# CSTR-Edinburgh/magphase

Measured on AMD Instinct MI355X. Metric: frames/sec analysis+synthesis @48kHz FFT=4096, higher is better.
Workload: dtype f32

## Files before the change

include/magphase_hip.h:

```cpp
#ifndef MAGPHASE_HIP_H
#define MAGPHASE_HIP_H

#include <stddef.h>
#include <stdint.h>

#ifdef __cplusplus
extern "C" {
#endif

#define MPX_ABI_VERSION 2

#define MPX_OK 0
#define MPX_ERR_ARG (-1)
#define MPX_ERR_HIP (-2)
#define MPX_ERR_HOST (-3)

int mpx_version(void);
const char* mpx_last_error(void);

size_t mpx_tables_bytes(int fft_len);
int mpx_tables_init(void* stream, int fft_len, void* tables);

int mpx_analysis_frames(void* stream, int fft_len, const void* tables, const float* sig,
                        const int64_t* frame_pos, const int32_t* frame_left, const int32_t* frame_right,
                        int64_t n_frames, float* out_mag, float* out_real, float* out_imag, int64_t ld);

size_t mpx_tables_f64_bytes(int fft_len);
int mpx_tables_f64_init(void* stream, int fft_len, void* tables);
int mpx_analysis_frames_f64(void* stream, int fft_len, const void* tables_f64, const float* sig,
                            const int64_t* frame_pos, const int32_t* frame_left, const int32_t* frame_right,
                            int64_t n_frames, float* out_mag, float* out_real, float* out_imag, int64_t ld,
                            const float* rows_in_use);

int mpx_analysis_frames_f64w(void* stream, int fft_len, const void* tables_f64, const float* sig,
                             const int64_t* frame_pos, const int32_t* frame_left, const int32_t* frame_right,
                             int64_t n_frames, float* out_mag, float* out_real, float* out_imag, int64_t ld,
                             const float* rows_in_use, const double* win_tab, int32_t win_cap);

int mpx_analysis_compressed_fused(void* stream, int fft_len, const void* tables_f64, const float* sig,
                                  const int64_t* frame_pos, const int32_t* frame_left, const int32_t* frame_right,
                                  int64_t n_frames, const double* win_tab, int32_t win_cap, const float* wpack,
                                  const float* whalf, int32_t mag_dim, int32_t phase_dim, const float* voiced,
                                  int32_t mag_fbank, float* out_mag, float* out_real, float* out_imag);
int mpx_analysis_compressed_fused_cr(void* stream, int fft_len, const void* tables_f64, const float* sig,
                                     const int64_t* frame_pos, const int32_t* frame_left, const int32_t* frame_right,
                                     int64_t n_frames, const double* win_tab, int32_t win_cap, const float* wpack,
                                     const float* whalf, int32_t mag_dim, int32_t phase_dim, const float* rows_in_use,
                                     const int32_t* row0, const int32_t* row1, const float* row_t, int64_t n_const,
                                     float* out_mag, float* tmp_real, float* tmp_imag, void* work);
int64_t mpx_analysis_compressed_fused_cr_work_bytes(int fft_len, int64_t n_frames);
int mpx_analysis_compressed_fused_tiles(int32_t mag_dim, int32_t phase_dim, int32_t* ntm, int32_t* ntp);
int mpx_analysis_compressed_fused_waves(void);
int mpx_analysis_compressed_fused_layout(void);
int mpx_analysis_compressed_fused_blocks_per_cu(int fft_len, int32_t phase_dim);

int64_t mpx_feat_ld(int fft_len);

int mpx_synthesis_lossless_frames(void* stream, int fft_len, const void* tables, const float* mag,
                                  const float* real, const float* imag, int64_t n_frames, float* frames_out,
                                  int64_t ld);

int mpx_ola_gather(void* stream, int fft_len, const float* frames, int32_t n_utts, const int32_t* utt_frame_off,
                   const int32_t* pm_rel, const int32_t* out_start, const int64_t* out_off, int64_t max_out_len,
                   float* pcm_out);

typedef struct mpx_ola_run {
    int32_t frame_begin, frame_end;
    int32_t x0;
    int32_t head_end;
    int32_t out_lo, out_hi;
    int32_t flush_end;
    int32_t fix_lo, fix_hi;
    int32_t pad;
    int64_t out_base;
    int64_t strip_off;
} mpx_ola_run;

int mpx_synth_ola_slots(void);
int mpx_synth_ola_slot_weights(float* weights_host, int32_t n_slots);
int64_t mpx_ola_strip_floats(int fft_len);
int mpx_synthesis_lossless_ola(void* stream, int fft_len, const void* tables, const float* mag, const float* real,
                               const float* imag, const mpx_ola_run* runs, int32_t n_runs, const int32_t* slot_off,
                               const int32_t* slot_runs, int32_t n_slots, const int32_t* pm_rel, float* strips,
                               float* pcm_out, int64_t ld );
int mpx_ola_fixup(void* stream, int fft_len, const mpx_ola_run* runs, int32_t n_runs, const float* strips,
                  float* pcm_out);
int mpx_ola_fixup_width(void* stream, int fft_len, const mpx_ola_run* runs, int32_t n_runs, const float* strips,
                        float* pcm_out, int32_t max_width);
int mpx_synthesis_lossless_ola_lerp(void* stream, int fft_len, const void* tables, const float* mag, const float* real,
                                    const float* imag, const int32_t* row0, const int32_t* row1, const float* row_t,
                                    const mpx_ola_run* runs, int32_t n_runs, const int32_t* slot_off,
                                    const int32_t* slot_runs, int32_t n_slots, const int32_t* pm_rel, float* strips,
                                    float* pcm_out, int64_t ld);

int mpx_rows_lerp(void* stream, int32_t n_bins, const float* src_mag, const float* src_real, const float* src_imag,
                  int64_t ld_src, const int32_t* row0, const int32_t* row1, const float* row_t, int64_t n_out,
                  float* dst_mag, float* dst_real, float* dst_imag, int64_t ld_dst);

int mpx_synthesis_lossless_backward(void* stream, int fft_len, const void* tables, const float* grad_out,
                                    int64_t total_out, const int64_t* grad_pos, const int32_t* grad_lo,
                                    const int32_t* grad_hi, int64_t n_frames, const float* mag, const float* real,
                                    const float* imag, int64_t ld, const int32_t* row0, const int32_t* row1,
                                    const float* row_t, float* grad_mag, float* grad_real, float* grad_imag,
                                    int64_t ld_grad);

int mpx_synthesis_compressed_backward(void* stream, int fft_len, const void* tables, const float* grad_out,
                                      int64_t total_out, const int64_t* grad_pos, const int32_t* grad_lo,
                                      const int32_t* grad_hi, int64_t n_frames, const float* mag, const float* real,
                                      const float* imag, int64_t ld, const float* noise, const int64_t* noise_pos,
                                      const int32_t* noise_left, const int32_t* noise_right, const int32_t* noise_wtype,
                                      const int32_t* voiced, const float* inv_gain, const int32_t* win_left,
                                      const int32_t* win_right, const float* per_v, const float* ap_v, const float* ap_u,
                                      int32_t n_per, float* grad_mag, float* grad_real, float* grad_imag,
                                      int64_t ld_grad);

int mpx_synthesis_compressed_type2_backward(void* stream, int fft_len, const void* tables, const float* grad_out,
                                            int64_t total_out, const int64_t* grad_pos, const int32_t* grad_lo,
                                            const int32_t* grad_hi, int64_t n_frames, const float* mag, const float* real,
                                            const float* imag, int64_t ld, const float* noise, const int64_t* noise_pos,
                                            const int32_t* noise_left, const int32_t* noise_right,
                                            const int32_t* noise_wtype, const int32_t* voiced, const float* inv_gain,
                                            const int32_t* win_left, const int32_t* win_right, const float* per_v,
                                            const float* ap_v, const float* ap_u, int32_t n_per, float* grad_mag,
                                            float* grad_real, float* grad_imag, int64_t ld_grad);

int mpx_rows_lerp_adjoint(void* stream, int32_t n_bins, const float* src_mag, const float* src_real,
                          const float* src_imag, int64_t ld_src, const int32_t* ranges, const float* row_t,
                          int64_t n_rows, float* dst_mag, float* dst_real, float* dst_imag, int64_t ld_dst);

int mpx_analysis_lossless_backward(void* stream, int fft_len, const void* tables, const float* mag, const float* real,
                                   const float* imag, int64_t ld, const float* grad_mag, const float* grad_real,
                                   const float* grad_imag, int64_t ld_grad, const int64_t* frame_pos,
                                   const int32_t* frame_left, const int32_t* frame_right, const int64_t* scratch_off,
                                   int64_t n_frames, float* scratch, int64_t scratch_floats, float* grad_sig,
                                   int64_t total_smpls);

int mpx_roundtrip_slot_weights(float* weights_host, int32_t n_slots);
int mpx_roundtrip_frame_terms(int fft_len, const int32_t* frame_left, const int32_t* frame_right, int64_t n_frames,
                              int32_t* terms_host);
int mpx_roundtrip_slot_costs(int32_t* coef_host, int32_t n_slots);
int mpx_roundtrip_lossless_ola(void* stream, int fft_len, const void* tables, const float* sig, const int64_t* frame_pos,
                               const int32_t* frame_left, const int32_t* frame_right, int64_t n_frames,
                               const mpx_ola_run* runs, int32_t n_runs, const int32_t* slot_off, const int32_t* slot_runs,
                               int32_t n_slots, const int32_t* pm_rel, float* out_mag, float* out_real, float* out_imag,
                               float* strips, float* pcm_out, int64_t ld);
#define MPX_RT_FULL_SUPPORT 1u
#define MPX_RT_STORE_ROWS 4u
#define MPX_RT_STORE_NT 8u
#define MPX_RT_INVERSE_TRANSFORM 32u
int mpx_roundtrip_store_map(int fft_len, int phase, int32_t* out);
int mpx_roundtrip_lossless_ola_flags(void* stream, int fft_len, const void* tables, const float* sig,
                                     const int64_t* frame_pos, const int32_t* frame_left, const int32_t* frame_right,
                                     int64_t n_frames, const mpx_ola_run* runs, int32_t n_runs, const int32_t* slot_off,
                                     const int32_t* slot_runs, int32_t n_slots, const int32_t* pm_rel, float* out_mag,
                                     float* out_real, float* out_imag, float* strips, float* pcm_out, int64_t ld,
                                     uint32_t flags);
int mpx_roundtrip_support_classes(int fft_len, const int32_t* frame_left, const int32_t* frame_right, int64_t n_frames,
                                  int32_t* class_host);
int mpx_roundtrip_frame_extents(int fft_len, const int32_t* frame_left, const int32_t* frame_right, int64_t n_frames,
                                uint32_t flags, int32_t* extents_host);

int mpx_griffin_lim_ola(void* stream, int fft_len, const void* tables, const float* sig_in, const int64_t* frame_pos,
                        const int32_t* frame_left, const int32_t* frame_right, int64_t n_frames, const float* target_mag,
                        const mpx_ola_run* runs, int32_t n_runs, const int32_t* slot_off, const int32_t* slot_runs,
                        int32_t n_slots, const int32_t* pm_rel, float* phase_out, float* strips, float* sig_out,
                        int64_t ld);


int mpx_mel_unwarp(void* stream, int64_t n_frames, int32_t n_bins, const float* a_mag, int32_t k_mag,
                   const float* u_mag, float* out_mag, const float* a_real, const float* a_imag, int32_t k_phase,
                   const float* u_phase, float* out_real, float* out_imag,
// ... 236 lines not shown
```

magphase_amd/_lib.py:

```python
import ctypes
import threading
import os

_HERE = os.path.dirname(os.path.abspath(__file__))
LIB_PATH = os.path.join(_HERE, "libmagphase_hip.so")

vp, i32, i64, sz, f64 = ctypes.c_void_p, ctypes.c_int32, ctypes.c_int64, ctypes.c_size_t, ctypes.c_double
u32 = ctypes.c_uint32

PROTOTYPES = {
    "mpx_version": (i32, []),
    "mpx_last_error": (ctypes.c_char_p, []),
    "mpx_tables_bytes": (sz, [i32]),
    "mpx_tables_init": (i32, [vp, i32, vp]),
    "mpx_feat_ld": (i64, [i32]),
    "mpx_analysis_frames": (i32, [vp, i32] + [vp] * 5 + [i64, vp, vp, vp, i64]),
    "mpx_tables_f64_bytes": (sz, [i32]),
    "mpx_tables_f64_init": (i32, [vp, i32, vp]),
    "mpx_analysis_frames_f64": (i32, [vp, i32] + [vp] * 5 + [i64, vp, vp, vp, i64, vp]),
    "mpx_analysis_frames_f64w": (i32, [vp, i32] + [vp] * 5 + [i64, vp, vp, vp, i64, vp, vp, i32]),
    "mpx_analysis_compressed_fused": (i32, [vp, i32] + [vp] * 5 + [i64, vp, i32, vp, vp, i32, i32, vp, i32, vp, vp,
                                       vp]),
    "mpx_analysis_compressed_fused_cr": (i32, [vp, i32] + [vp] * 5 + [i64, vp, i32, vp, vp, i32, i32] + [vp] * 4 +
                                          [i64] + [vp] * 4),
    "mpx_analysis_compressed_fused_cr_work_bytes": (i64, [i32, i64]),
    "mpx_analysis_compressed_fused_tiles": (i32, [i32, i32, ctypes.POINTER(i32), ctypes.POINTER(i32)]),
    "mpx_analysis_compressed_fused_waves": (i32, []),
    "mpx_analysis_compressed_fused_layout": (i32, []),
    "mpx_analysis_compressed_fused_blocks_per_cu": (i32, [i32, i32]),
    "mpx_synthesis_lossless_frames": (i32, [vp, i32] + [vp] * 4 + [i64, vp, i64]),
    "mpx_ola_gather": (i32, [vp, i32, vp, i32] + [vp] * 4 + [i64, vp]),
    "mpx_synth_ola_slots": (i32, []),
    "mpx_synth_ola_slot_weights": (i32, [vp, i32]),
    "mpx_ola_strip_floats": (i64, [i32]),
    "mpx_synthesis_lossless_ola": (i32, [vp, i32] + [vp] * 5 + [i32, vp, vp, i32, vp, vp, vp, i64]),
    "mpx_synthesis_lossless_ola_lerp": (i32, [vp, i32] + [vp] * 8 + [i32, vp, vp, i32, vp, vp, vp, i64]),
    "mpx_rows_lerp": (i32, [vp, i32, vp, vp, vp, i64, vp, vp, vp, i64, vp, vp, vp, i64]),
    "mpx_synthesis_lossless_backward": (i32, [vp, i32, vp, vp, i64, vp, vp, vp, i64, vp, vp, vp, i64] + [vp] * 6 + [i64]),
    "mpx_synthesis_compressed_backward": (i32, [vp, i32, vp, vp, i64, vp, vp, vp, i64, vp, vp, vp, i64] + [vp] * 12
                                          + [i32, vp, vp, vp, i64]),
    "mpx_synthesis_compressed_type2_backward": (i32, [vp, i32, vp, vp, i64, vp, vp, vp, i64, vp, vp, vp, i64] + [vp] * 12
                                                + [i32, vp, vp, vp, i64]),
    "mpx_rows_lerp_adjoint": (i32, [vp, i32, vp, vp, vp, i64, vp, vp, i64, vp, vp, vp, i64]),
    "mpx_analysis_lossless_backward": (i32, [vp, i32, vp, vp, vp, vp, i64, vp, vp, vp, i64, vp, vp, vp, vp, i64, vp, i64,
                                             vp, i64]),
    "mpx_ola_fixup": (i32, [vp, i32, vp, i32, vp, vp]),
    "mpx_ola_fixup_width": (i32, [vp, i32, vp, i32, vp, vp, i32]),
    "mpx_roundtrip_lossless_ola": (i32, [vp, i32] + [vp] * 5 + [i64, vp, i32, vp, vp, i32] + [vp] * 6 + [i64]),
    "mpx_roundtrip_lossless_ola_flags": (i32, [vp, i32] + [vp] * 5 + [i64, vp, i32, vp, vp, i32] + [vp] * 6 + [i64, u32]),
    "mpx_roundtrip_support_classes": (i32, [i32, vp, vp, i64, vp]),
    "mpx_roundtrip_frame_extents": (i32, [i32, vp, vp, i64, u32, vp]),
    "mpx_roundtrip_store_map": (i32, [i32, i32, vp]),
    "mpx_roundtrip_slot_weights": (i32, [vp, i32]),
    "mpx_roundtrip_frame_terms": (i32, [i32, vp, vp, i64, vp]),
    "mpx_roundtrip_slot_costs": (i32, [vp, i32]),
    "mpx_griffin_lim_ola": (i32, [vp, i32] + [vp] * 5 + [i64, vp, vp, i32, vp, vp, i32] + [vp] * 4 + [i64]),
    "mpx_mel_unwarp": (i32, [vp, i64, i32, vp, i32] + [vp] * 4 + [i32, vp, vp, vp, i64]),
    "mpx_mel_unwarp_rows": (i32, [vp, i64, i32, vp, i32] + [vp] * 4 + [i32, vp, vp, vp, i64, vp, vp, vp, i64, vp, vp,
                             i32]),
    "mpx_spec_ld": (i64, [i32]),
    "mpx_noise_uniform": (i32, [vp, i32, vp, vp, i64, vp]),
    "mpx_noise_numpy_mt19937": (i32, [vp, vp, i32, i64] + [vp] * 5),
    "mpx_noise_numpy_mt19937_work_words": (i64, []),
    "mpx_host_mt19937_jump_poly": (i32, [i64, i32, vp]),
    "mpx_host_mt19937_jump_polys": (i32, [vp, i32, vp, i32]),
    "mpx_noise_stats": (i32, [vp, i32] + [vp] * 6 + [i64, vp]),
    "mpx_noise_spectra_floats": (i64, [i32, i64]),
    "mpx_noise_stats_spectra": (i32, [vp, i32] + [vp] * 6 + [i64, vp, vp]),
    "mpx_synth_comp_slots": (i32, []),
    "mpx_synth_comp_slot_weights": (i32, [vp, i32]),
    "mpx_synthesis_compressed_ola": (i32, [vp, i32] + [vp] * 21 + [i32, vp, vp, i32, vp, vp, i64, i32]),
    "mpx_synthesis_compressed_type2_ola": (i32, [vp, i32] + [vp] * 21 + [i32, vp, vp, i32, vp, vp, i64, i32]),
    "mpx_synthesis_compressed_ola_spectra": (i32, [vp, i32] + [vp] * 21 + [i32, vp, vp, i32, vp, vp, i64, i32, vp]),
    "mpx_host_const_to_var_scan": (i64, [vp, vp, i64, vp, vp]),
    "mpx_host_const_to_var_scan_cap": (i64, [vp, vp, i64, vp, vp, i64]),
    "mpx_host_plan_analysis": (i64, [i32] + [vp] * 12),
    "mpx_host_plan_analysis_batch": (i64, [i32] + [vp] * 8 + [i32] + [vp] * 9 + [i32, vp, vp, i64, vp, i32]),
    "mpx_host_plan_synthesis": (i64, [i32, vp, vp, f64, i32, i32, i32, i64] + [vp] * 17),
    "mpx_host_plan_synthesis_batch": (i64, [i32] + [vp] * 5 + [i32, i32, vp, vp, f64] + [i32] * 4 + [vp, f64, i32, vp,
                                       i64] + [vp] * 9 + [i64, vp, i32]),
    "mpx_host_plan_lossless_synthesis": (i64, [i32, vp, vp, vp, i32] + [vp] * 4),
    "mpx_host_ola_runs": (i64, [i32] + [vp] * 5 + [i32, vp, i64, vp, i64]),
    "mpx_host_ola_runs_extents": (i64, [i32] + [vp] * 5 + [i32, vp, i64, vp, vp, i64]),
    "mpx_host_deal_cuts": (i64, [vp, i64, i32, vp, i32, vp, vp]),
    "mpx_host_widen_f32": (i32, [vp, vp, i64, i32]),
    "mpx_host_narrow_f64": (i32, [vp, vp, i64, i32]),
    "mpx_host_copy_many": (i32, [i32] + [vp] * 4 + [i32]),
    "mpx_host_file_sizes": (i32, [i32, vp, vp]),
    "mpx_host_read_est_batch": (i32, [i32, vp, i32] + [vp] * 4 + [i32]),
    "mpx_host_write_files": (i32, [i32] + [vp] * 6 + [i32]),
    "mpx_host_read_files": (i32, [i32] + [vp] * 4 + [i32]),
    "mpx_mel_warp": (i32, [vp, i64, i32] + [vp] * 7 + [i32, vp, i32] + [vp] * 4 + [i64]),
    "mpx_mel_warp_fbank": (i32, [vp, i64, i32] + [vp] * 7 + [i32, vp, i32] + [vp] * 4 + [i64]),
    "mpx_mel_warp_rows": (i32, [vp, i64, i32] + [vp] * 7 + [i32, vp, i32] + [vp] * 4 + [i64, i32, i64, vp, vp, vp]),
    "mpx_warp_phase_rows": (i32, [vp, i64, i32] + [vp] * 8),
    "mpx_mel_warp_backward": (i32, [vp, i32, vp, vp, i32, vp, i64] + [vp] * 7 + [i32, vp, vp, i64, vp, vp, vp, i64, i64]),
    "mpx_mel_unwarp_backward": (i32, [vp, i32, vp, i64, vp, i64, vp, i32, i64, vp, vp, vp, i64, i32, vp, i32, i64, vp, vp]),
    "mpx_phase_grad_mask": (i32, [vp, i64, i32] + [vp] * 7),
    "mpx_min_phase": (i32, [vp, i32] + [vp] * 5 + [i64, vp, vp, vp, i64]),
    "mpx_true_envelope": (i32, [vp, i32, vp, vp, vp, i64, i64, i32, f64, i32, vp, i64, vp, vp, vp]),
    "mpx_frame_gain": (i32, [vp, i32] + [vp] * 5 + [i64, vp, i32]),
    "mpx_noise_gains": (i32, [vp] * 4 + [i32, i32, vp, vp]),
    "mpx_noise_power": (i32, [vp, i32] + [vp] * 5 + [i64, vp]),
    "mpx_noise_rms": (i32, [vp, i32, vp, vp, i32, vp, vp]),
    "mpx_post_filter": (i32, [vp, vp, i64, i32, vp, i32, i32, vp, vp]),
    "mpx_epoch_f0_track": (i32, [vp, vp, vp, i32, i32, vp, i64, vp, vp, vp, i64] + [i32] * 4 + [f64, vp, vp, vp]),
    "mpx_epoch_zff": (i32, [vp, vp, vp, i32, i64, vp, i32, vp, vp, vp, i32] + [vp] * 5),
    "mpx_pcm16": (i32, [vp, vp, i32, vp, i32, i64, f64, vp, vp]),
    "mpx_pcm16_to_f32": (i32, [vp, vp, i64, vp]),
    "mpx_hpf_block": (i32, []),
    "mpx_output_hpf": (i32, [vp] * 4 + [i32, i64] + [vp] * 7),
    "mpx_bw_probe": (i32, [vp, i32, vp, vp, i64]),
    "mpx_bw_probe_shapes": (i32, []),
    "mpx_rows_pack": (i32, [vp, vp, vp, i32, i32] + [vp, i32, i64, i64] * 3),
    "mpx_post_filter_merlin": (i32, [vp, vp, i64, i32] + [vp] * 4 + [i32, f64, vp, f64] + [vp] * 5),
}
SYMBOLS = tuple(PROTOTYPES)
RT_STORE_FLAGS = {"rows": 4, "lines": 0, "lines_nt": 8}
RT_INVERSE_FLAGS = {"direct": 0, "transform": 32}
del vp, i32, i64, sz, f64

_lib = None


class MagphaseHipError(RuntimeError):
    pass


_load_lock = threading.Lock()


def load():
    global _lib
    if _lib is not None:
        return _lib
    with _load_lock:
        return _load_locked()


def _load_locked():
    global _lib
    if _lib is not None:
        return _lib
    import torch
    if not os.path.isfile(LIB_PATH):
        raise MagphaseHipError(
            "libmagphase_hip.so not found at %s -- build it with `python -m magphase_amd.build` "
            "(hipcc --offload-arch=gfx950). There is no CPU fallback." % LIB_PATH
        )
    lib = ctypes.CDLL(LIB_PATH)
    for name, (restype, argtypes) in PROTOTYPES.items():
        fn = getattr(lib, name)
        fn.restype, fn.argtypes = restype, argtypes
    _lib = lib
    return lib


def check(rc, what):
    if rc != 0:
        msg = load().mpx_last_error()
        raise MagphaseHipError("%s failed (%d): %s" % (what, rc, msg.decode("utf-8", "replace") if msg else ""))
```

magphase_amd/csrc/magphase_comp.hip:

```cpp
#include <type_traits>

#include "mpx_common.hpp"

#ifndef MPX_COMP_PAIR_WAVES
#define MPX_COMP_PAIR_WAVES 12
#endif
#ifndef MPX_COMP_DIT
#define MPX_COMP_DIT 0
#endif
#ifndef MPX_COMP_CH
#define MPX_COMP_CH 16
#endif

namespace mpx {

template <int P, bool PRESTAGED, bool COMPACT, int W>
__device__ __forceinline__ void noise_window_gather(const FrameGeom& g, int wtype, float* xbuf, unsigned xbuf_byte, int lane,
                                                    float (&re)[P], float (&im)[P]) {
    constexpr int M = 64 * P, N = 2 * M, kTile = noise_tile_len(P, COMPACT);
    MPX_MARK("zero_init");
#pragma unroll
    for (int j = 0; j < P; ++j)
        if (j < W || j >= P - W) re[(COMPACT && MPX_COMP_DIT) ? brev(j, ilog2(P)) : j] = im[(COMPACT && MPX_COMP_DIT) ? brev(j, ilog2(P)) : j] = 0.0f;
    const int ntiles = MPX_NOISE_TILES(g.len, kTile);
    for (int t = 0; t < ntiles; ++t) {
        MPX_MARK("window");
        const int tile0 = t * kTile;
        if (!PRESTAGED || t > 0) {
            stage_samples_async(g, tile0, kTile, xbuf_byte, lane);
            staged_wait<0>();
        }
        const int hi = min(g.len, tile0 + kTile);
        if (wtype == 0) {
            for (int k = tile0 + lane; k < hi; k += 64)
                xbuf[k - tile0] *= half_window(k, g.L, g.LR, g.kadd, g.invL, g.invR, 0);
        } else {
            for (int k = tile0 + lane; k < hi; k += 64)
                xbuf[k - tile0] *= half_window(k, g.L, g.LR, g.kadd, g.invL, g.invR, 1);
        }
        wave_sync();
        MPX_MARK("gather");
        {
            int n_lo = g.len - g.rot, n_hi = N - g.rot;
            asm volatile("" : "+s"(n_lo), "+s"(n_hi));
            const unsigned span = (unsigned)(hi - tile0);
            const unsigned b0 = (unsigned)(2 * lane + g.rot) - (unsigned)tile0;
#pragma unroll
            for (int j = 0; j < P; ++j) {
                constexpr int LBJ = ilog2(P);
                const int m0 = 128 * j;
                if ((j < W || j >= P - W) && MPX_NOISE_ROW_ACTIVE(m0, n_lo, n_hi)) {
                    const int rj = (COMPACT && MPX_COMP_DIT) ? brev(j, LBJ) : j;
                    const unsigned d0 = (b0 + (unsigned)m0) & (unsigned)(N - 1), d1 = (d0 + 1u) & (unsigned)(N - 1);
                    const float v0 = xbuf[min(d0, (unsigned)(kTile - 1))], v1 = xbuf[min(d1, (unsigned)(kTile - 1))];
                    re[rj] = (d0 < span) ? v0 : re[rj];
                    im[rj] = (d1 < span) ? v1 : im[rj];
                }
            }
        }
        wave_sync();
    }
}

struct NoiseFftNoHook {
    template <int P, typename B>
    __device__ __forceinline__ void gathered(float (&)[P], float (&)[P], B) const {}
    __device__ __forceinline__ void exchanged() const {}
};
template <typename GFn, typename XFn>
struct NoiseFftHook {
    GFn on_gathered;
    XFn on_exchanged;
    template <int P, typename B>
    __device__ __forceinline__ void gathered(float (&re)[P], float (&im)[P], B narrow_c) const { on_gathered(re, im, narrow_c); }
    __device__ __forceinline__ void exchanged() const { on_exchanged(); }
};
template <typename GFn, typename XFn>
__device__ __forceinline__ NoiseFftHook<GFn, XFn> noise_fft_hook(GFn g, XFn x) { return NoiseFftHook<GFn, XFn>{g, x}; }

template <int P, bool PRESTAGED = false, bool COMPACT = false, int NW = 0, typename Hook = NoiseFftNoHook>
__device__ __forceinline__ void noise_fft(const FrameGeom& g, int wtype, const float* tw, float* xbuf,
                                          unsigned xbuf_byte, int lane, float (&re)[P], float (&im)[P], float lc = 1.0f,
                                          float ls = 0.0f, bool narrow = false, Hook hook = Hook()) {
    static_assert(NW == 0 || (COMPACT && !MPX_COMP_DIT), "support classes: the compact DIF form only");
    if constexpr (NW > 0) {
        constexpr unsigned kZin = support_zero_rows<P>(NW);
        constexpr int S0 = zin_clear_stride<P>(kZin);
        static_assert(S0 >= 1 && S0 < P / 2, "a class prunes some, not all, stages of the first pass");
        if (narrow) {
            noise_window_gather<P, PRESTAGED, COMPACT, NW>(g, wtype, xbuf, xbuf_byte, lane, re, im);
            mpx_pin_live<~kZin>(re), mpx_pin_live<~kZin>(im);
            hook.gathered(re, im, std::true_type());
            MPX_MARK("fft_forward");
            fft_inreg_pruned_stage<P, -1, P / 2, kZin, kAllRegs, 2 * S0>(re, im);
            MPX_ARM_END_CLASS();
        } else {
            noise_window_gather<P, PRESTAGED, COMPACT, P / 2>(g, wtype, xbuf, xbuf_byte, lane, re, im);
            mpx_pin(re), mpx_pin(im);
            hook.gathered(re, im, std::false_type());
            MPX_MARK("fft_forward");
            fft_inreg_stages<P, -1, P / 2, 2 * S0>(re, im);
            MPX_ARM_END_FULL();
        }
        const float4 pk = tw_half_pad<P>(tw, lane);
        fft_inreg_stages<P, -1, S0>(re, im);
        wave_fft_front_compact_rest<P, -1>(re, im, tw, xbuf, lane, pk.z, pk.w);
        hook.exchanged();
        fft_inreg<P, -1>(re, im);
        (void)lc;
        (void)ls;
        return;
    }
    constexpr int M = 64 * P, N = 2 * M, kTile = noise_tile_len(P, COMPACT);
    MPX_MARK("zero_init");
#pragma unroll
    for (int j = 0; j < P; ++j) re[j] = im[j] = 0.0f;
    const int ntiles = MPX_NOISE_TILES(g.len, kTile);
    for (int t = 0; t < ntiles; ++t) {
        MPX_MARK("window");
        const int tile0 = t * kTile;
        if (!PRESTAGED || t > 0) {
            stage_samples_async(g, tile0, kTile, xbuf_byte, lane);
            staged_wait<0>();
        }
        const int hi = min(g.len, tile0 + kTile);
        if (wtype == 0) {
            for (int k = tile0 + lane; k < hi; k += 64)
                xbuf[k - tile0] *= half_window(k, g.L, g.LR, g.kadd, g.invL, g.invR, 0);
        } else {
            for (int k = tile0 + lane; k < hi; k += 64)
                xbuf[k - tile0] *= half_window(k, g.L, g.LR, g.kadd, g.invL, g.invR, 1);
        }
        wave_sync();
        MPX_MARK("gather");
        {
            int n_lo = g.len - g.rot, n_hi = N - g.rot;
            asm volatile("" : "+s"(n_lo), "+s"(n_hi));
            const unsigned span = (unsigned)(hi - tile0);
            const unsigned b0 = (unsigned)(2 * lane + g.rot) - (unsigned)tile0;
#pragma unroll
            for (int j = 0; j < P; ++j) {
                constexpr int LBJ = ilog2(P);
                const int m0 = 128 * j;
                if (MPX_NOISE_ROW_ACTIVE(m0, n_lo, n_hi)) {
                    const int rj = (COMPACT && MPX_COMP_DIT) ? brev(j, LBJ) : j;
                    const unsigned d0 = (b0 + (unsigned)m0) & (unsigned)(N - 1), d1 = (d0 + 1u) & (unsigned)(N - 1);
                    const float v0 = xbuf[min(d0, (unsigned)(kTile - 1))], v1 = xbuf[min(d1, (unsigned)(kTile - 1))];
                    re[rj] = (d0 < span) ? v0 : re[rj];
                    im[rj] = (d1 < span) ? v1 : im[rj];
                }
            }
        }
        wave_sync();
    }
    mpx_pin(re), mpx_pin(im);
    hook.gathered(re, im, std::false_type());
    MPX_MARK("fft_forward");
    if constexpr (COMPACT) {
        const float4 pk = tw_half_pad<P>(tw, lane);
#if MPX_COMP_DIT
        wave_fft_dit_compact<P, -1>(re, im, tw, xbuf, lane, pk.z, pk.w);
        hook.exchanged();
#else
        wave_fft_front_compact<P, -1>(re, im, tw, xbuf, lane, pk.z, pk.w);
        hook.exchanged();
        fft_inreg<P, -1>(re, im);
#endif
        (void)lc;
        (void)ls;
    } else {
        wave_fft_front<P, -1>(re, im, tw, xbuf, lane);
        hook.exchanged();
        fft_inreg<P, -1>(re, im);
    }
}

template <int P, bool PRESTAGED = false, bool COMPACT = false, int NW = 0, typename Hook = NoiseFftNoHook>
__device__ __forceinline__ void noise_spectrum_paired(const FrameGeom& g, int wtype, const float* tw, float* xbuf,
                                                      unsigned xbuf_byte, int lane, float wl_c, float wl_s,
                                                      float (&no_r)[P / 2], float (&no_i)[P / 2], float (&nm_r)[P / 2],
                                                      float (&nm_i)[P / 2], float& nh_r, float& nh_i, float lc = 1.0f,
                                                      float ls = 0.0f, bool narrow = false, Hook hook = Hook()) {
    constexpr int LB = ilog2(P);
    float re[P], im[P];
    noise_fft<P, PRESTAGED, COMPACT, NW>(g, wtype, tw, xbuf, xbuf_byte, lane, re, im, lc, ls, narrow, hook);
    mpx_pin(re), mpx_pin(im);
    MPX_MARK("split");
    if constexpr (COMPACT) {
        const float4 pk = tw_half_pad<P>(tw, lane);
        wl_c = pk.x;
        wl_s = pk.y;
    }
    const int kap = kappa<P>(lane);
    const int src_lane = kappa<P>((64 - kap) & 63);
    const bool lane0 = (kap == 0);
#ifndef MPX_NOISE_SPLIT_BATCH
#define MPX_NOISE_SPLIT_BATCH (MPX_COMP_PAIR_WAVES > 8 ? 8 : 16)
#endif
    constexpr int SB = (P / 2 < MPX_NOISE_SPLIT_BATCH) ? P / 2 : MPX_NOISE_SPLIT_BATCH;
#pragma unroll
    for (int qb = 0; qb < P / 2; qb += SB) {
        float zpr[SB], zpi[SB];
        constexpr bool NATR = COMPACT && MPX_COMP_DIT;
#pragma unroll
        for (int u = 0; u < SB; ++u) {
            const int i = NATR ? qb + u : brev(qb + u, LB);
            zpr[u] = __shfl(re[P - 1 - i], src_lane);
            zpi[u] = __shfl(im[P - 1 - i], src_lane);
        }
#pragma unroll
        for (int u = 0; u < SB; ++u) {
            const int q = qb + u;
            const int i = NATR ? q : brev(q, LB);
            const int i0 = NATR ? (P - q) % P : brev((P - q) % P, LB);
            const float pr = lane0 ? re[i0] : zpr[u];
            const float pi = lane0 ? im[i0] : zpi[u];
            const float er = 0.5f * (re[i] + pr), ei = 0.5f * (im[i] - pi);
            const float orr = 0.5f * (im[i] + pi), oi = -0.5f * (re[i] - pr);
            const float cq = cos2p<P>(q), sq = -sin2p<P>(q);
            const float wr = wl_c * cq - wl_s * sq, wi = wl_c * sq + wl_s * cq;
            const float tr = wr * orr - wi * oi, ti = wr * oi + wi * orr;
            no_r[q] = er + tr;
            no_i[q] = ei + ti;
            nm_r[q] = er - tr;
            nm_i[q] = ti - ei;
        }
    }
    constexpr int ih = (COMPACT && MPX_COMP_DIT) ? P / 2 : 1;
    nh_r = re[ih];
    nh_i = -im[ih];
}

template <int P, bool PRESTAGED = false, bool COMPACT = false>
__device__ __forceinline__ void noise_spectrum(const FrameGeom& g, int wtype, const float* tw, float* xbuf,
                                               unsigned xbuf_byte, int lane, float wl_c, float wl_s,
                                               float (&nr)[P], float (&ni)[P], float& nM, float lc = 1.0f, float ls = 0.0f) {
    constexpr int LB = ilog2(P);
    float re[P], im[P];
    noise_fft<P, PRESTAGED, COMPACT>(g, wtype, tw, xbuf, xbuf_byte, lane, re, im, lc, ls);
    if constexpr (COMPACT) {
        const float4 pk = tw_half_pad<P>(tw, lane);
        wl_c = pk.x;
        wl_s = pk.y;
    }
    const int kap = kappa<P>(lane);
    const int src_lane = kappa<P>((64 - kap) & 63);
    const bool lane0 = (kap == 0);
#pragma unroll
    for (int ib = 0; ib < P; ib += 8) {
        float prb[8], pib[8];
#pragma unroll
        for (int u = 0; u < 8; ++u) {
            prb[u] = __shfl(re[P - 1 - (ib + u)], src_lane);
            pib[u] = __shfl(im[P - 1 - (ib + u)], src_lane);
        }
#pragma unroll
        for (int u = 0; u < 8; ++u) {
            const int i = ib + u;
            constexpr bool NATR = COMPACT && MPX_COMP_DIT;
            const int q = NATR ? i : brev(i, LB);
            const int i0 = NATR ? (P - q) % P : brev((P - q) % P, LB);
            const float pr = lane0 ? re[i0] : prb[u];
            const float pi = lane0 ? im[i0] : pib[u];
            const float er = 0.5f * (re[i] + pr), ei = 0.5f * (im[i] - pi);
            const float orr = 0.5f * (im[i] + pi), oi = -0.5f * (re[i] - pr);
            const float cq = cos2p<P>(q), sq = -sin2p<P>(q);
            const float wr = wl_c * cq - wl_s * sq, wi = wl_c * sq + wl_s * cq;
            nr[q] = er + (wr * orr - wi * oi);
            ni[q] = ei + (wr * oi + wi * orr);
        }
    }
    nM = re[0] - im[0];
}

constexpr int kSpecFrameFloats = 17 * 64 * 4;
typedef float spec_f32x4 __attribute__((ext_vector_type(4)));

template <int P>
__global__ __launch_bounds__(kAnaThreads) void k_noise_stats(const float* __restrict__ noise,
                                                          const long long* __restrict__ npos,
                                                          const int* __restrict__ nleft,
                                                          const int* __restrict__ nright,
                                                          const int* __restrict__ wtype, long long nframes,
                                                          const float* __restrict__ tw_g,
                                                          float* __restrict__ out_sum,
                                                          float* __restrict__ spec_out) {
    constexpr int M = 64 * P, N = 2 * M;
    extern __shared__ __attribute__((aligned(16))) float smem[];
    float* tw = smem;
    const int lane_id = threadIdx.x & 63;
    const int wave = threadIdx.x >> 6;
    float* xbuf = smem + tw_floats<P>() + wave * (P * kXStride);
    const unsigned xbuf_byte = 4u * (unsigned)(tw_floats<P>() + rfl(wave) * (P * kXStride));
    for (int i = threadIdx.x; i < tw_floats<P>(); i += kAnaThreads) tw[i] = tw_g[i];
    unsigned* queue = reinterpret_cast<unsigned*>(smem + tw_floats<P>() + kAnaWaves * (P * kXStride));
    if (threadIdx.x == 0) *queue = 0u;
    __syncthreads();
    float wl_s0, wl_c0;
    sincospif(-2.0f * (float)kappa<P>(lane_id) / (float)N, &wl_s0, &wl_c0);
    long long fb, fe;
    block_frame_range(nframes, fb, fe);
    for (long long f = queue_pull(queue, fb); f < fe; f = queue_pull(queue, fb)) {
        int lane = lane_id;
        float wl_s = wl_s0, wl_c = wl_c0;
        asm volatile("" : "+v"(lane), "+v"(wl_s), "+v"(wl_c));
        const FrameGeom g = frame_geom(noise, npos[f], nleft[f], nright[f], N);
        float no_r[P / 2], no_i[P / 2], nm_r[P / 2], nm_i[P / 2], nh_r, nh_i;
        noise_spectrum_paired<P>(g, wtype[f], tw, xbuf, xbuf_byte, lane, wl_c, wl_s, no_r, no_i, nm_r, nm_i, nh_r, nh_i);
        if constexpr (P == 32) {
            if (spec_out) {
                spec_f32x4* d = reinterpret_cast<spec_f32x4*>(spec_out + f * (long long)kSpecFrameFloats) + lane_id;
#pragma unroll
                for (int s_ = 0; s_ < 4; ++s_) {
                    __builtin_nontemporal_store(spec_f32x4{no_r[4 * s_], no_r[4 * s_ + 1], no_r[4 * s_ + 2], no_r[4 * s_ + 3]}, d + 64 * s_);
                    __builtin_nontemporal_store(spec_f32x4{no_i[4 * s_], no_i[4 * s_ + 1], no_i[4 * s_ + 2], no_i[4 * s_ + 3]}, d + 64 * (4 + s_));
                    __builtin_nontemporal_store(spec_f32x4{nm_r[4 * s_], nm_r[4 * s_ + 1], nm_r[4 * s_ + 2], nm_r[4 * s_ + 3]}, d + 64 * (8 + s_));
                    __builtin_nontemporal_store(spec_f32x4{nm_i[4 * s_], nm_i[4 * s_ + 1], nm_i[4 * s_ + 2], nm_i[4 * s_ + 3]}, d + 64 * (12 + s_));
                }
                __builtin_nontemporal_store(spec_f32x4{nh_r, nh_i, 0.0f, 0.0f}, d + 64 * 16);
            }
        }
        const bool lane0 = (kappa<P>(lane) == 0);
        float so[P / 2], sm[P / 2];
        const float sh = nh_r * nh_r + nh_i * nh_i;
        float smin = lane0 ? sh : 1.0f;
#pragma unroll
        for (int q = 0; q < P / 2; ++q) {
            so[q] = no_r[q] * no_r[q] + no_i[q] * no_i[q];
            sm[q] = nm_r[q] * nm_r[q] + nm_i[q] * nm_i[q];
            smin = fminf(smin, fminf(so[q], sm[q]));
        }
        float acc;
        if (!__any(smin < 1.1754944e-38f)) {
            auto term = [](float s_) {
                const float lg = 0.34657359027997264f * __builtin_amdgcn_logf(s_);
                return lg * lg;
            };
            acc = lane0 ? term(sh) : 0.0f;
#pragma unroll
            for (int q = 0; q < P / 2; ++q) {
                const float tq = term(so[q]) + term(sm[q]);
                acc += (q == 0 && lane0) ? 0.0f : tq;
            }
        } else {
            auto term = [](float s_) {
                const float lg = (s_ > 0.0f) ? 0.5f * __logf(s_) : -1.0e10f;
                return lg * lg;
            };
            acc = lane0 ? term(sh) : 0.0f;
#pragma unroll
            for (int q = 0; q < P / 2; ++q) {
                const float tq = term(so[q]) + term(sm[q]);
                acc += (q == 0 && lane0) ? 0.0f : tq;
            }
        }
#pragma unroll
        for (int off = 32; off >= 1; off >>= 1) acc += __shfl_xor(acc, off);
        if (lane_id == 0) out_sum[f] = acc;
    }
}

__global__ __launch_bounds__(256) void k_noise_gains(const float* __restrict__ sums, const int* __restrict__ voiced,
                                                     const int* __restrict__ utt_frame_off, int bins_per_frame,
                                                     float* __restrict__ inv_gain, double* __restrict__ gains) {
    __shared__ double s_sum[2][256];
    __shared__ int s_cnt[2][256];
    const int u = blockIdx.x;
    const int f0 = utt_frame_off[u], f1 = utt_frame_off[u + 1];
    double acc[2] = {0.0, 0.0};
    int cnt[2] = {0, 0};
    for (int f = f0 + threadIdx.x; f < f1; f += 256) {
        const int c = voiced[f] ? 0 : 1;
        acc[c] += (double)sums[f];
        cnt[c] += 1;
    }
    for (int c = 0; c < 2; ++c) {
        s_sum[c][threadIdx.x] = acc[c];
        s_cnt[c][threadIdx.x] = cnt[c];
    }
    __syncthreads();
    for (int off = 128; off >= 1; off >>= 1) {
        if (threadIdx.x < off) {
            for (int c = 0; c < 2; ++c) {
                s_sum[c][threadIdx.x] += s_sum[c][threadIdx.x + off];
                s_cnt[c][threadIdx.x] += s_cnt[c][threadIdx.x + off];
            }
        }
        __syncthreads();
    }
    double g[2];
    for (int c = 0; c < 2; ++c)
        g[c] = (s_cnt[c][0] > 0) ? sqrt(exp(s_sum[c][0] / ((double)s_cnt[c][0] * (double)bins_per_frame))) : nan("");
    if (threadIdx.x == 0 && gains) {
        gains[2 * u + 0] = g[0];
        gains[2 * u + 1] = g[1];
    }
    for (int f = f0 + threadIdx.x; f < f1; f += 256) inv_gain[f] = (float)(1.0 / g[voiced[f] ? 0 : 1]);
}

template <int P>
__global__ __launch_bounds__(kThreads) void k_min_phase(const float* __restrict__ mag, const int* __restrict__ row0,
                                                        const int* __restrict__ row1,
                                                        const float* __restrict__ rowt, long long nframes,
                                                        const float* __restrict__ tw_g, float* __restrict__ omag,
                                                        float* __restrict__ oreal, float* __restrict__ oimag,
                                                        long long ld) {
    constexpr int M = 64 * P, N = 2 * M, H = M + 1, LB = ilog2(P);
    extern __shared__ __attribute__((aligned(16))) float smem[];
    float* tw = smem;
    const int lane_id = threadIdx.x & 63;
    const int wave = threadIdx.x >> 6;
    float* xbuf = smem + tw_floats<P>() + wave * (P * kXStride);
    for (int i = threadIdx.x; i < tw_floats<P>(); i += kThreads) tw[i] = tw_g[i];
    __syncthreads();
    float wa_s0, wa_c0, ws_s0, ws_c0;
    sincospif(-2.0f * (float)kappa<P>(lane_id) / (float)N, &wa_s0, &wa_c0);
    sincospif(2.0f * (float)lane_id / (float)N, &ws_s0, &ws_c0);
    const int wave_u = rfl(wave);
    for (long long f = (long long)blockIdx.x * kWavesPerBlock + wave_u; f < nframes;
         f += (long long)gridDim.x * kWavesPerBlock) {
        int lane = lane_id;
        float wa_s = wa_s0, wa_c = wa_c0, ws_s = ws_s0, ws_c = ws_c0;
        asm volatile("" : "+v"(lane), "+v"(wa_s), "+v"(wa_c), "+v"(ws_s), "+v"(ws_c));
        const int r0 = row0[f], r1 = row1[f];
        const float rt = rowt[f];
        const float* m0p = mag + (long long)r0 * ld;
        const float* m1p = mag + (long long)r1 * ld;
        float xr[P], xi[P], mv[P];
        const float scale = 0.5f / (float)M;
#pragma unroll
        for (int j = 0; j < P; ++j) {
            const float a = m0p[lane + 64 * j], b = m1p[lane + 64 * j];
            mv[j] = fmaf(b - a, rt, a);
        }
        float mM = 0.0f;
        if (lane == 0) {
            const float a = m0p[M], b = m1p[M];
            mM = fmaf(b - a, rt, a);
        }
#pragma unroll
        for (int j = 0; j < P; ++j) {
            xr[j] = ((mv[j] > 0.0f) ? logf(mv[j]) : -1.0e10f) * scale;
            xi[j] = 0.0f;
        }
        const float xm = ((mM > 0.0f) ? logf(mM) : -1.0e10f) * scale;
        hermitian_merge<P>(xr, xi, xm, lane, ws_c, ws_s);
        wave_fft<P, +1>(xr, xi, tw, xbuf, lane);
        const int kap = kappa<P>(lane);
#pragma unroll
        for (int i = 0; i < P; ++i) {
            const int n0 = 2 * (kap + 64 * brev(i, LB));
            const float w0 = (n0 == 0) ? 1.0f : ((n0 < M) ? 2.0f : ((n0 == M) ? 1.0f : 0.0f));
            const float w1 = (n0 + 1 < M) ? 2.0f : ((n0 + 1 == M) ? 1.0f : 0.0f);
            xr[i] *= w0;
            xi[i] *= w1;
        }
        float re[P], im[P];
#pragma unroll
        for (int i = 0; i < P; ++i) {
            re[brev(i, LB)] = xr[i];
            im[brev(i, LB)] = xi[i];
// ... 835 lines not shown
                              "the mirror tail's lanes: lane 0 and those that do not store this step's mirror");
                st_mask(mhi + row_mir_base(lane, cu_m, M) + row_mir_off(HP), lane0 ? mH : hm, ~k_cu_m | 1ull);
                st_mask(rhi + row_mir_base(lane, cu_r, M) + row_mir_off(HP), lane0 ? aH : ha, ~k_cu_r | 1ull);
                st_mask(ihi + row_mir_base(lane, cu_i, M) + row_mir_off(HP), lane0 ? bH : hb, ~k_cu_i | 1ull);
            }
            if constexpr (!DIRECT) merge_handover<P>(zr, zi, 2.0f * nh_r, -2.0f * nh_i, xr, xi, lane);
        }
        if constexpr (DIRECT) {
            g = g_next;
        } else {
            pair_inverse_fft_front<P>(w, xr, xi, lane);
            if (nxt.valid) {
                g = frame_geom(sig, fpos[nxt.fi], fleft[nxt.fi], fright[nxt.fi], N);
                pair_stage_next<P>(w, g, lane);
            }
            if constexpr (kCls) pair_inverse_fft_back_class<P, NW>(xr, xi, narrow);
            else pair_inverse_fft_back<P>(xr, xi);
            constexpr float kScale = 0.5f / (float)M;
            auto plain_add = [](float o, float v, int) { return fmaf(v, kScale, o); };
            auto all_rows = [](int) { return true; };
            pair_ordered_ola<P, true, NW>(w, cur, smem, runs, pm_rel, strips, pcm, xr, xi, lane, plain_add, all_rows, narrow);
        }
        cur = nxt;
#ifdef MPX_PROBE_ENDTIME
        ++probe_frames;
#endif
    }
#ifdef MPX_PROBE_ENDTIME
    if (w.lane_id == 0) {
        const int pw = (blockIdx.x * kCompPairWaves + (int)(threadIdx.x >> 6)) % 8192;
        g_rt_endprobe[4 * pw + 0] = probe_t0;
        g_rt_endprobe[4 * pw + 1] = wall_clock64();
        g_rt_endprobe[4 * pw + 2] = (unsigned long long)probe_frames;
        g_rt_endprobe[4 * pw + 3] = clock64() - probe_c0;
    }
#endif
}

template <int P, bool PHASE>
__global__ __launch_bounds__(kCompPairWaves * 64) void k_griffin_lim_pair(const float* __restrict__ sig,
                                                                         const long long* __restrict__ fpos,
                                                                         const int* __restrict__ fleft,
                                                                         const int* __restrict__ fright,
                                                                         const RunDesc* __restrict__ runs,
                                                                         const int* __restrict__ slot_off,
                                                                         const int* __restrict__ slot_runs, int nslots,
                                                                         const int* __restrict__ pm_rel,
                                                                         const float* __restrict__ tw_g,
                                                                         const float* __restrict__ tmag,
                                                                         float* __restrict__ phase_out,
                                                                         float* __restrict__ strips,
                                                                         float* __restrict__ pcm, long long ld) {
    constexpr int M = 64 * P, N = 2 * M, HP = P / 2;
    extern __shared__ __attribute__((aligned(16))) float smem[];
    PairWave w;
    if (!pair_wave_setup<P>(w, smem, tw_g, runs, slot_off, slot_runs, nslots)) return;
    PairCursor cur = w.cur;

    FrameGeom g = frame_geom(sig, fpos[cur.fi], fleft[cur.fi], fright[cur.fi], N);
    pair_stage_frame<P>(w, g, w.lane_id);

    while (cur.valid) {
        int lane;
        float wa_s, wa_c, ws_s, ws_c;
        pair_frame_lane<P>(w, lane, wa_s, wa_c, ws_s, ws_c);
        PairCursor nxt = cur;
        pair_cursor_advance(nxt, w.wi_end, w.half, runs, slot_runs);
        const int fi = cur.fi;

        float xr[P], xi[P];
        {
            float no_r[HP], no_i[HP], nm_r[HP], nm_i[HP], nh_r, nh_i;
            pair_analysis_spectrum<P>(w, g, lane, wa_c, wa_s, no_r, no_i, nm_r, nm_i, nh_r, nh_i);
            MPX_MARK("magnitude_merge");
            const bool lane0 = (lane == 0);
            const float sgn = (lane & 1) ? -1.0f : 1.0f;
            const float* trow = tmag + (long long)fi * ld;
            float* prow = PHASE ? phase_out + (long long)fi * ld : nullptr;
            if constexpr (PHASE) {
                auto ang = [](float x_r, float x_i, float s) {
                    return (x_r == 0.0f && x_i == 0.0f) ? 0.0f : atan2f(s * x_i, s * x_r);
                };
#pragma unroll
                for (int q = 0; q < HP; ++q) {
                    const int k = lane + 64 * q;
                    prow[k] = ang(no_r[q], no_i[q], sgn);
                    prow[M - k] = ang(nm_r[q], nm_i[q], sgn);
                    asm volatile("" ::: "memory");
                }
                if (lane0) prow[M / 2] = ang(nh_r, nh_i, 1.0f);
            }
            auto replace = [](float& x_r, float& x_i, float t, float s) {
                const bool z = (x_r == 0.0f) && (x_i == 0.0f);
                const float sc = (fmaxf(fabsf(x_r), fabsf(x_i)) < 0x1p-60f) ? 0x1p100f : 1.0f;
                const float u_r = x_r * sc, u_i = x_i * sc;
                const float r = __builtin_amdgcn_rsqf(fmaxf(u_r * u_r + u_i * u_i, 1.0e-37f));
                x_r = z ? t * s : t * (u_r * r);
                x_i = z ? 0.0f : t * (u_i * r);
            };
            if constexpr (comp_compact<P>()) {
                const float4 pk = tw_half_pad<P>(w.tw, lane);
                ws_c = pk.x;
                ws_s = -pk.y;
            }
            float zr[HP], zi[HP];
#pragma unroll
            for (int q = 0; q < HP; ++q) {
                const int k = lane + 64 * q;
                float x_r = no_r[q], x_i = no_i[q], p_r = nm_r[q], p_i = nm_i[q];
                replace(x_r, x_i, trow[k], sgn);
                replace(p_r, p_i, trow[M - k], sgn);
                if (q == 0) {
                    x_i = lane0 ? 0.0f : x_i;
                    p_i = lane0 ? 0.0f : p_i;
                }
                merge_pair_step<P>(q, x_r, x_i, p_r, p_i, ws_c, ws_s, xr[q], xi[q], zr[q], zi[q]);
            }
            replace(nh_r, nh_i, trow[M / 2], 1.0f);
            merge_handover<P>(zr, zi, 2.0f * nh_r, -2.0f * nh_i, xr, xi, lane);
        }
        pair_inverse_fft_front<P>(w, xr, xi, lane);
        if (nxt.valid) {
            g = frame_geom(sig, fpos[nxt.fi], fleft[nxt.fi], fright[nxt.fi], N);
            pair_stage_next<P>(w, g, lane);
        }
        pair_inverse_fft_back<P>(xr, xi);
        constexpr float kScale = 0.5f / (float)M;
        auto plain_add = [](float o, float v, int) { return fmaf(v, kScale, o); };
        auto all_rows = [](int) { return true; };
        pair_ordered_ola<P, true>(w, cur, smem, runs, pm_rel, strips, pcm, xr, xi, lane, plain_add, all_rows);
        cur = nxt;
    }
}

}

using namespace mpx;

extern "C" {

int64_t mpx_spec_ld(int32_t n_bins) { return n_bins <= 0 ? 0 : ((int64_t)n_bins + 31) / 32 * 32; }

static int noise_stats_impl(void* stream, int fft_len, const void* tables, const float* noise, const int64_t* frame_pos,
                            const int32_t* frame_left, const int32_t* frame_right, const int32_t* frame_wtype,
                            int64_t n_frames, float* out_sum, float* spectra) {
    const int P = p_of(fft_len);
    if (!P) return fail(MPX_ERR_ARG, "mpx_noise_stats: fft_len must be 1024, 2048 or 4096%s");
    if (n_frames < 0) return fail(MPX_ERR_ARG, "mpx_noise_stats: negative n_frames%s");
    if (n_frames == 0) return MPX_OK;
    if (!tables || !noise || !frame_pos || !frame_left || !frame_right || !frame_wtype || !out_sum)
        return fail(MPX_ERR_ARG, "mpx_noise_stats: null pointer%s");
    const dim3 grid(grid_for(n_frames, kAnaWaves)), block(kAnaThreads);
    hipStream_t s = (hipStream_t)stream;
    if (P == 32) {
        if (int rc = set_lds(k_noise_stats<32>, lds_bytes_ana<32>())) return rc;
        hipLaunchKernelGGL(k_noise_stats<32>, grid, block, lds_bytes_ana<32>(), s, noise, (const long long*)frame_pos,
                           frame_left, frame_right, frame_wtype, (long long)n_frames, (const float*)tables, out_sum, spectra);
    } else if (P == 16) {
        if (int rc = set_lds(k_noise_stats<16>, lds_bytes_ana<16>())) return rc;
        hipLaunchKernelGGL(k_noise_stats<16>, grid, block, lds_bytes_ana<16>(), s, noise, (const long long*)frame_pos,
                           frame_left, frame_right, frame_wtype, (long long)n_frames, (const float*)tables, out_sum, spectra);
    } else {
        if (int rc = set_lds(k_noise_stats<8>, lds_bytes_ana<8>())) return rc;
        hipLaunchKernelGGL(k_noise_stats<8>, grid, block, lds_bytes_ana<8>(), s, noise, (const long long*)frame_pos,
                           frame_left, frame_right, frame_wtype, (long long)n_frames, (const float*)tables, out_sum, spectra);
    }
    MPX_HIP_CHECK(hipGetLastError());
    return MPX_OK;
}

int mpx_noise_stats(void* stream, int fft_len, const void* tables, const float* noise, const int64_t* frame_pos,
                    const int32_t* frame_left, const int32_t* frame_right, const int32_t* frame_wtype,
                    int64_t n_frames, float* out_sum) {
    return noise_stats_impl(stream, fft_len, tables, noise, frame_pos, frame_left, frame_right, frame_wtype, n_frames,
                            out_sum, nullptr);
}

int64_t mpx_noise_spectra_floats(int fft_len, int64_t n_frames) {
    return (fft_len == 4096 && n_frames > 0) ? n_frames * (int64_t)kSpecFrameFloats : 0;
}

int mpx_noise_stats_spectra(void* stream, int fft_len, const void* tables, const float* noise, const int64_t* frame_pos,
                            const int32_t* frame_left, const int32_t* frame_right, const int32_t* frame_wtype,
                            int64_t n_frames, float* out_sum, float* spectra) {
    if (fft_len != 4096) return fail(MPX_ERR_ARG, "mpx_noise_stats_spectra: fft_len must be 4096%s");
    if (!spectra && n_frames > 0) return fail(MPX_ERR_ARG, "mpx_noise_stats_spectra: null pointer%s");
    return noise_stats_impl(stream, fft_len, tables, noise, frame_pos, frame_left, frame_right, frame_wtype, n_frames,
                            out_sum, spectra);
}

int mpx_synth_comp_slots(void) { return device_cus() * kCompPairs; }

#ifndef MPX_COMP_W0
#define MPX_COMP_W0 100
#endif
#ifndef MPX_COMP_W1
#define MPX_COMP_W1 (MPX_COMP_PAIR_WAVES > 8 ? 82 : 80)
#endif
#ifndef MPX_COMP_W2
#define MPX_COMP_W2 66
#endif
int mpx_synth_comp_slot_weights(float* weights_host, int32_t n_slots) {
    if (!weights_host || n_slots < 0) return fail(MPX_ERR_ARG, "mpx_synth_comp_slot_weights: bad arguments%s");
    for (int s = 0; s < n_slots; ++s) {
        const int age = ((s % kCompPairs) * 2) / 4;
        weights_host[s] = (age == 0) ? (float)MPX_COMP_W0 : ((age == 1) ? (float)MPX_COMP_W1 : (float)MPX_COMP_W2);
    }
    return MPX_OK;
}

extern "C++" {
template <bool T2>
static int synthesis_compressed_ola_impl(const char* who, void* stream, int fft_len, const void* tables, const float* mag, const float* real,
                                 const float* imag, const float* noise, const int64_t* noise_pos,
                                 const int32_t* noise_left, const int32_t* noise_right, const int32_t* noise_wtype,
                                 const int32_t* voiced, const float* inv_gain, const int32_t* row0,
                                 const int32_t* row1, const float* row_t, const int32_t* win_left,
                                 const int32_t* win_right, const int32_t* pm_rel, const float* per_v,
                                 const float* ap_v, const float* ap_u, const mpx_ola_run* runs, int32_t n_runs,
                                 const int32_t* slot_off, const int32_t* slot_runs, int32_t n_slots,
                                 float* strips, float* pcm_out, int64_t ld, int32_t n_per_bins,
                                 const float* spectra) {
    const int P = p_of(fft_len);
    if (!P) return fail(MPX_ERR_ARG, "%s: fft_len must be 1024, 2048 or 4096", who);
    const int n_per = (n_per_bins <= 0 || n_per_bins > fft_len / 2 + 1) ? fft_len / 2 + 1 : (int)n_per_bins;
    if (n_runs < 0 || n_slots < 0) return fail(MPX_ERR_ARG, "%s: negative count", who);
    if (n_runs == 0 || n_slots == 0) return MPX_OK;
    if (!tables || !mag || !real || !imag || !noise || !noise_pos || !noise_left || !noise_right || !noise_wtype ||
        !voiced || !inv_gain || !win_left || !win_right || !pm_rel || !per_v || !ap_v ||
        !ap_u || !runs || !slot_off || !slot_runs || !strips || !pcm_out)
        return fail(MPX_ERR_ARG, "%s: null pointer", who);
    const bool lerp = row0 || row1 || row_t;
    if (lerp && (!row0 || !row1 || !row_t))
        return fail(MPX_ERR_ARG, "%s: row0 / row1 / row_t must be given together", who);
    CompFrameTabs tb{(const long long*)noise_pos, noise_left, noise_right, noise_wtype, voiced, inv_gain,
                     row0, row1, row_t, win_left, win_right, pm_rel, spectra};
    hipStream_t s = (hipStream_t)stream;
    const dim3 pgrid((n_slots + kCompPairs - 1) / kCompPairs), pblock(kCompPairWaves * 64);
    if (spectra) {
        if (P != 32 || lerp)
            return fail(MPX_ERR_ARG, "mpx_synthesis_compressed_ola_spectra: fft_len 4096 and one row per frame only%s");
        if (n_per <= 512) {
            if (int rc = set_lds(k_synth_comp_pair<32, false, 8, true>, lds_bytes_comp_pair<32>())) return rc;
            hipLaunchKernelGGL((k_synth_comp_pair<32, false, 8, true>), pgrid, pblock, lds_bytes_comp_pair<32>(),
                               s, mag, real, imag, noise, tb, per_v, ap_v, ap_u, (const RunDesc*)runs, slot_off, slot_runs,
                               (int)n_slots, (const float*)tables, strips, pcm_out, (long long)ld, n_per);
        } else {
            if (int rc = set_lds(k_synth_comp_pair<32, false, -1, true>, lds_bytes_comp_pair<32>())) return rc;
            hipLaunchKernelGGL((k_synth_comp_pair<32, false, -1, true>), pgrid, pblock, lds_bytes_comp_pair<32>(),
                               s, mag, real, imag, noise, tb, per_v, ap_v, ap_u, (const RunDesc*)runs, slot_off, slot_runs,
                               (int)n_slots, (const float*)tables, strips, pcm_out, (long long)ld, n_per);
        }
        MPX_HIP_CHECK(hipGetLastError());
        return MPX_OK;
    }
#define MPX_LAUNCH_COMP(PP, LL)                                                                                        \
    do {                                                                                                             \
        if (int rc = set_lds(k_synth_comp_pair<PP, LL, -1, false, T2>, lds_bytes_comp_pair<PP>())) return rc;        \
        hipLaunchKernelGGL((k_synth_comp_pair<PP, LL, -1, false, T2>), pgrid, pblock, lds_bytes_comp_pair<PP>(), s,  \
                           mag, real, imag,                                                                          \
                           noise, tb, per_v, ap_v, ap_u, (const RunDesc*)runs, slot_off, slot_runs, (int)n_slots,    \
                           (const float*)tables, strips, pcm_out, (long long)ld, n_per);                 \
    } while (0)
    if (lerp) {
        if (P == 32) MPX_LAUNCH_COMP(32, true);
        else if (P == 16) MPX_LAUNCH_COMP(16, true);
        else MPX_LAUNCH_COMP(8, true);
    } else {
        if (P == 32 && n_per <= 512) {
            if (int rc = set_lds(k_synth_comp_pair<32, false, 8, false, T2>, lds_bytes_comp_pair<32>())) return rc;
            hipLaunchKernelGGL((k_synth_comp_pair<32, false, 8, false, T2>), pgrid, pblock, lds_bytes_comp_pair<32>(), s, mag, real, imag,
                               noise, tb, per_v, ap_v, ap_u, (const RunDesc*)runs, slot_off, slot_runs, (int)n_slots,
                               (const float*)tables, strips, pcm_out, (long long)ld, n_per);
        } else if (P == 32) MPX_LAUNCH_COMP(32, false);
        else if (P == 16) MPX_LAUNCH_COMP(16, false);
        else MPX_LAUNCH_COMP(8, false);
    }
#undef MPX_LAUNCH_COMP
    MPX_HIP_CHECK(hipGetLastError());
    return MPX_OK;
}
}

int mpx_synthesis_compressed_ola(void* stream, int fft_len, const void* tables, const float* mag, const float* real,
                                 const float* imag, const float* noise, const int64_t* noise_pos,
                                 const int32_t* noise_left, const int32_t* noise_right, const int32_t* noise_wtype,
                                 const int32_t* voiced, const float* inv_gain, const int32_t* row0,
                                 const int32_t* row1, const float* row_t, const int32_t* win_left,
                                 const int32_t* win_right, const int32_t* pm_rel, const float* per_v,
                                 const float* ap_v, const float* ap_u, const mpx_ola_run* runs, int32_t n_runs,
                                 const int32_t* slot_off, const int32_t* slot_runs, int32_t n_slots,
                                 float* strips, float* pcm_out, int64_t ld, int32_t n_per_bins) {
    return synthesis_compressed_ola_impl<false>("mpx_synthesis_compressed_ola", stream, fft_len, tables, mag, real, imag, noise,
                                                noise_pos, noise_left, noise_right, noise_wtype, voiced, inv_gain, row0, row1,
                                                row_t, win_left, win_right, pm_rel, per_v, ap_v, ap_u, runs, n_runs, slot_off,
                                                slot_runs, n_slots, strips, pcm_out, ld, n_per_bins, nullptr);
}

int mpx_synthesis_compressed_type2_ola(void* stream, int fft_len, const void* tables, const float* mag, const float* real,
                                       const float* imag, const float* noise, const int64_t* noise_pos,
                                       const int32_t* noise_left, const int32_t* noise_right, const int32_t* noise_wtype,
                                       const int32_t* voiced, const float* inv_gain, const int32_t* row0,
                                       const int32_t* row1, const float* row_t, const int32_t* win_left,
                                       const int32_t* win_right, const int32_t* pm_rel, const float* per_v,
                                       const float* ap_v, const float* ap_u, const mpx_ola_run* runs, int32_t n_runs,
                                       const int32_t* slot_off, const int32_t* slot_runs, int32_t n_slots,
                                       float* strips, float* pcm_out, int64_t ld, int32_t n_per_bins) {
// ... 283 lines not shown
```

magphase_amd/csrc/magphase_f64.hip:

```cpp
#include <type_traits>

#include "mpx_common.hpp"
#include "wave_fft_f64.hpp"

namespace mpx {

constexpr int kAna64Waves = 8;
template <int P>
constexpr int f64_win_floats() { return 58 * P; }
#ifndef MPX_F64_DIT
#define MPX_F64_DIT 1
#endif
constexpr bool kF64Dit = MPX_F64_DIT != 0;
template <int P>
constexpr size_t lds_bytes_ana64() {
    return sizeof(double) * (size_t)tw64_doubles<P>() +
           sizeof(float) * (size_t)(kAna64Waves * P * kXStride + 4 + kAna64Waves * f64_win_floats<P>());
}

__device__ __forceinline__ double sin_halfpi_range(double x) {
    const double x2 = x * x;
    double p = 1.0 / 355687428096000.0;
    p = fma(x2, p, -1.0 / 1307674368000.0);
    p = fma(x2, p, 1.0 / 6227020800.0);
    p = fma(x2, p, -1.0 / 39916800.0);
    p = fma(x2, p, 1.0 / 362880.0);
    p = fma(x2, p, -1.0 / 5040.0);
    p = fma(x2, p, 1.0 / 120.0);
    p = fma(x2, p, -1.0 / 6.0);
    return fma(x * x2, p, x);
}

__device__ __forceinline__ double hann_half_f64(int k, int L, int LR, int kadd, double invL, double invR) {
    const bool rising = k <= L;
    const int num = rising ? k + kadd : LR - k;
    const double t = (double)num * (rising ? invL : invR);
    return fma(0.5, sin_halfpi_range(3.14159265358979323846 * (t - 0.5)), 0.5);
}

__device__ __forceinline__ double rsqrt_f64(double s) {
    const double r = (double)__builtin_amdgcn_rsqf((float)s);
    return r * fma(-0.5 * s, r * r, 1.5);
}

template <bool PH>
__device__ __forceinline__ void feat_store(double xr, double xi, double zero2, float mag_scale, float* pm, float* pr, float* pi) {
    const double s = xr * xr + xi * xi;
    const bool nz = s > zero2;
    const double r = nz ? rsqrt_f64(s) : 0.0;
    *pm = (float)(s * r) * mag_scale;
    if (PH) {
        *pr = (float)(xr * r);
        *pi = (float)(xi * r);
    }
}

template <int P>
__device__ __forceinline__ constexpr int f64_in_reg(int j) { return kF64Dit ? brev(j, ilog2(P)) : j; }
template <int P>
__device__ __forceinline__ constexpr int f64_out_reg(int q) { return kF64Dit ? q : brev(q, ilog2(P)); }

template <int P>
__device__ __forceinline__ void f64_frame_transform(const float* __restrict__ sig, long long pos, int Lf, int Rf,
                                                    const double* __restrict__ win_tab, int win_cap, const double* tw,
                                                    float* xbuf, unsigned xbuf_byte, float* wbuf, unsigned wbuf_byte,
                                                    int lane, double (&re)[P], double (&im)[P], double& zero2_out,
                                                    float& mag_scale_out) {
    constexpr int N = 128 * P, kTile = 64 * P;
    const FrameGeom g = frame_geom(sig, pos, Lf, Rf, N);
    const double invL = (g.L > 0) ? 1.0 / (double)g.L : 1.0;
    const double invR = (g.LR > g.L) ? 1.0 / (double)(g.LR - g.L) : 0.0;
    const int gR = g.LR - g.L;
    const bool tabw = rfl((int)(win_tab != nullptr && g.L <= win_cap && gR <= win_cap)) != 0;
    const double* tl = win_tab + ((long long)g.L * (g.L + 1) >> 1);
    const double* tr = win_tab + ((long long)gR * (gR + 1) >> 1);
    const float in_scale = tabw ? 1073741824.0f : 1.0f;
    const float mag_scale = tabw ? 9.313225746154785e-10f : 1.0f;

    double s_abs = 0.0;
#pragma unroll
    for (int j = 0; j < P; ++j) re[j] = im[j] = 0.0;
    constexpr int capD = f64_win_floats<P>() / 2;
    double* wl = reinterpret_cast<double*>(wbuf);
    const int nidx = g.LR + 2;
    const int ntiles = (g.len + kTile - 1) / kTile;
    for (int t = 0; t < ntiles; ++t) {
        const int tile0 = t * kTile;
        const int hi = min(g.len, tile0 + kTile);
        stage_samples_async(g, tile0, kTile, xbuf_byte, lane);
        for (int seg0 = 0; seg0 < nidx; seg0 += capD) {
            const int seg1 = min(seg0 + capD, nidx);
            if (tabw) {
                const int a0 = seg0, a1 = min(g.L + 1, seg1), b0 = max(g.L + 1, seg0), b1 = seg1;
                const float* srcl = reinterpret_cast<const float*>(tl + a0);
                const float* srcr = reinterpret_cast<const float*>(tr + (b0 - (g.L + 1)));
                const int nl = 2 * max(a1 - a0, 0), nr = 2 * max(b1 - b0, 0);
                for (int c = 0; c < (nl + 63) >> 6; ++c) {
                    const unsigned m0v = __builtin_amdgcn_readfirstlane(wbuf_byte + 256u * (unsigned)c);
                    if (64 * c + lane < nl) {
                        const float* src = srcl + 64 * c + lane;
                        asm volatile("s_mov_b32 m0, %1\n\ts_nop 0\n\tglobal_load_lds_dword %0, off" ::"v"(src), "s"(m0v) : "m0", "memory");
                    }
                }
                for (int c = 0; c < (nr + 63) >> 6; ++c) {
                    const unsigned m0v = __builtin_amdgcn_readfirstlane(wbuf_byte + 8u * (unsigned)(b0 - seg0) + 256u * (unsigned)c);
                    if (64 * c + lane < nr) {
                        const float* src = srcr + 64 * c + lane;
                        asm volatile("s_mov_b32 m0, %1\n\ts_nop 0\n\tglobal_load_lds_dword %0, off" ::"v"(src), "s"(m0v) : "m0", "memory");
                    }
                }
            } else {
                for (int i = seg0 + lane; i < seg1; i += 64) {
                    const int k = (i <= g.L) ? i : g.LR - (i - (g.L + 1));
                    wl[i - seg0] = hann_half_f64(k, g.L, g.LR, g.kadd, invL, invR);
                }
            }
            staged_wait<0>();
            wave_sync();
            int lane_g = lane;
            asm volatile("" : "+v"(lane_g));
#pragma unroll
            for (int j = 0; j < P; ++j) {
                const int m0 = 128 * j;
                const bool any = (m0 < g.len - g.rot) || (m0 + 127 >= N - g.rot);
                if (any) {
                    const int m = m0 + 2 * lane_g;
                    int k0 = m + g.rot;
                    k0 = (k0 >= N) ? k0 - N : k0;
                    int k1 = m + 1 + g.rot;
                    k1 = (k1 >= N) ? k1 - N : k1;
                    const int i0 = ((k0 <= g.L) ? k0 : g.L + 1 + (g.LR - k0)) - seg0;
                    const int i1 = ((k1 <= g.L) ? k1 : g.L + 1 + (g.LR - k1)) - seg0;
                    if (k0 >= tile0 && k0 < hi && i0 >= 0 && i0 < capD) {
                        const double v = (double)(xbuf[k0 - tile0] * in_scale) * wl[i0];
                        re[f64_in_reg<P>(j)] = v;
                        s_abs += fabs(v);
                    }
                    if (k1 >= tile0 && k1 < hi && i1 >= 0 && i1 < capD) {
                        const double v = (double)(xbuf[k1 - tile0] * in_scale) * wl[i1];
                        im[f64_in_reg<P>(j)] = v;
                        s_abs += fabs(v);
                    }
                }
            }
            wave_sync();
        }
    }
    float s_all = (float)s_abs;
#pragma unroll
    for (int d = 32; d >= 1; d >>= 1) s_all += __shfl_xor(s_all, d);
    const double zt = 2.842170943040401e-14 * (double)s_all;
#ifdef MPX_F64_NOFLUSH
    const double zero2 = 1.0e-36 + 0.0 * zt;
#else
    const double zero2 = tabw ? 1.0e-36 : fmax(zt * zt, 1.0e-36);
#endif

    if constexpr (kF64Dit) wave_fft_dit_f64<P, -1>(re, im, tw, xbuf, lane);
    else wave_fft_f64<P, -1>(re, im, tw, xbuf, lane);
#pragma unroll
    for (int j = 0; j < P; j += 4)
        asm volatile("" : "+v"(re[j]), "+v"(re[j + 1]), "+v"(re[j + 2]), "+v"(re[j + 3]), "+v"(im[j]), "+v"(im[j + 1]),
                          "+v"(im[j + 2]), "+v"(im[j + 3]));

    zero2_out = zero2;
    mag_scale_out = mag_scale;
}

template <int P>
__global__ __launch_bounds__(kAna64Waves * 64) void k_analysis_f64(const float* __restrict__ sig,
                                                                  const long long* __restrict__ fpos,
                                                                  const int* __restrict__ fleft,
                                                                  const int* __restrict__ fright, long long nframes,
                                                                  const double* __restrict__ tw_g,
                                                                  float* __restrict__ omag, float* __restrict__ oreal,
                                                                  float* __restrict__ oimag, long long ld,
                                                                  const float* __restrict__ rows_in_use,
                                                                  const double* __restrict__ win_tab, int win_cap) {
    constexpr int M = 64 * P, N = 2 * M, LB = ilog2(P), kTile = 64 * P;
    extern __shared__ __attribute__((aligned(16))) double smem64[];
    double* tw = smem64;
    float* xbase = reinterpret_cast<float*>(smem64 + tw64_doubles<P>());
    const int lane_id = threadIdx.x & 63;
    const int wave = rfl((int)(threadIdx.x >> 6));
    float* xbuf = xbase + wave * (P * kXStride);
    const unsigned xbuf_byte = 8u * (unsigned)tw64_doubles<P>() + 4u * (unsigned)(wave * (P * kXStride));
    for (int i = threadIdx.x; i < tw64_doubles<P>(); i += kAna64Waves * 64) {
        const int l = i / tw64_stride<P>(), c = i - l * tw64_stride<P>();
        const int src = (kF64Dit && c < 2 * P) ? l * tw64_stride<P>() + 2 * brev(c >> 1, LB) + (c & 1) : i;
        tw[i] = tw_g[src];
    }
    unsigned* queue = reinterpret_cast<unsigned*>(xbase + kAna64Waves * (P * kXStride));
    float* wbuf = xbase + kAna64Waves * (P * kXStride) + 4 + wave * f64_win_floats<P>();
    const unsigned wbuf_byte = 8u * (unsigned)tw64_doubles<P>() + 4u * (unsigned)(kAna64Waves * (P * kXStride) + 4 + wave * f64_win_floats<P>());
    if (threadIdx.x == 0) *queue = 0u;
    __syncthreads();

    double wl_s0, wl_c0;
    sincospi(-2.0 * (double)kappa<P>(lane_id) / (double)N, &wl_s0, &wl_c0);

    long long fb, fe;
    block_frame_range(nframes, fb, fe);
    for (long long f = queue_pull(queue, fb); f < fe; f = queue_pull(queue, fb)) {
        int lane = lane_id;
        double wl_s = wl_s0, wl_c = wl_c0;
        asm volatile("" : "+v"(lane), "+v"(wl_s), "+v"(wl_c));
        const int kap = kappa<P>(lane);
        const int src_lane = kappa<P>((64 - kap) & 63);
        const bool lane0 = (kap == 0);
        double re[P], im[P];
        double zero2;
        float mag_scale;
        f64_frame_transform<P>(sig, fpos[f], fleft[f], fright[f], win_tab, win_cap, tw, xbuf, xbuf_byte, wbuf, wbuf_byte, lane, re,
                               im, zero2, mag_scale);

        float* row_m = omag + f * ld;
        float* row_r = oreal + f * ld;
        float* row_i = oimag + f * ld;
#ifndef MPX_F64_EPI_BATCH
#define MPX_F64_EPI_BATCH 4
#endif
        constexpr int EB = MPX_F64_EPI_BATCH;
        auto epilogue = [&](auto ph_tag) {
            constexpr bool PH = decltype(ph_tag)::value;
#pragma unroll
            for (int qb = 0; qb < P / 2; qb += EB) {
                double zpr[EB], zpi[EB];
#pragma unroll
                for (int u = 0; u < EB; ++u) {
                    const int i = f64_out_reg<P>(qb + u);
                    unsigned a, b, c, d;
                    split64(re[P - 1 - i], a, b);
// ... 14 lines not shown
                    const double cq = dc64(q * kq), sq = -ds64(q * kq);
                    const double wr = wl_c * cq - wl_s * sq, wi = wl_c * sq + wl_s * cq;
                    const double tr = wr * orr - wi * oi, ti = wr * oi + wi * orr;
                    const int k = kap + 64 * q;
                    feat_store<PH>(er + tr, ei + ti, zero2, mag_scale, row_m + k, row_r + k, row_i + k);
                    const int km = M - k;
                    feat_store<PH>(er - tr, ti - ei, zero2, mag_scale, row_m + km, row_r + km, row_i + km);
                }
            }
            constexpr int ih = f64_out_reg<P>(P / 2);
            if (lane0) feat_store<PH>(re[ih], -im[ih], zero2, mag_scale, row_m + M / 2, row_r + M / 2, row_i + M / 2);
        };
        if (rows_in_use == nullptr || rfl((int)(rows_in_use[f] != 0.0f))) epilogue(std::true_type{});
        else epilogue(std::false_type{});
    }
}

typedef float f32x4_t __attribute__((ext_vector_type(4)));
#ifndef MPX_FUSED_WAVES
#define MPX_FUSED_WAVES 8
#endif
constexpr int kFusedWaves = MPX_FUSED_WAVES;
static_assert(kFusedWaves == 4 || kFusedWaves == 8, "4 or 8 waves per fused workgroup");
constexpr int kFusedCols = 128 / kFusedWaves;
constexpr int kFusedKH = kFusedCols / 16;
#ifndef MPX_FUSED_ASTRIDE
#define MPX_FUSED_ASTRIDE 136
#endif
constexpr int kFusedAStride = MPX_FUSED_ASTRIDE;
static_assert(kFusedAStride % 4 == 0 && kFusedAStride >= 128, "published rows: 128 columns, 16-byte aligned");

constexpr int kFusedRedStride = 68;
#ifndef MPX_FUSED_PAIR
#define MPX_FUSED_PAIR 1
#endif
#ifndef MPX_FUSED_VOIBRANCH
#define MPX_FUSED_VOIBRANCH 1
#endif
#ifndef MPX_FUSED_F32NORM
#define MPX_FUSED_F32NORM 1
#endif
#ifndef MPX_FUSED_M4
#define MPX_FUSED_M4 1
#endif

__device__ __forceinline__ float fused_prologue_mag(int mode, float x) {
    if (mode == 0) return __builtin_amdgcn_logf(fmaf(x, x, 1.0e-8f)) * 0.69314718055994531f;
    return (x > 0.0f) ? __logf(x) : -1.0e10f;
}
#ifndef MPX_FUSED_EXPFIT
#define MPX_FUSED_EXPFIT 1
#endif
__device__ __forceinline__ float fused_prologue_phase(float x) {
#if MPX_FUSED_EXPFIT
    const float t = fmaf(x, fmaf(x, 2.75579379e-8f, -3.18127371e-8f), 0.90168841e-8f);
    return fmaf(2.0f, x, t);
#else
    return fmaf(1.0e-8f, __expf(-2.0f * x), 2.0f * x);
#endif
}

template <int MAGMODE, bool RAW>
__device__ __forceinline__ void fused_operand(double xr, double xi, double zero2, float mag_scale, bool voi, float& a_m, float& a_r,
                                              float& a_i) {
    const double s2 = xr * xr + xi * xi;
    const bool nz = s2 > zero2;
#if MPX_FUSED_F32NORM
    const float s2f = (float)s2;
    const float rf = nz ? __builtin_amdgcn_rsqf(s2f) : 0.0f;
    a_m = RAW ? (s2f * rf) * mag_scale : fused_prologue_mag(MAGMODE, (s2f * rf) * mag_scale);
    if (RAW) asm volatile("" : "+v"(a_m));
    if (voi) {
        a_r = fused_prologue_phase((float)xr * rf);
        a_i = fused_prologue_phase((float)xi * rf);
    } else {
        a_r = a_i = 0.0f;
    }
    return;
#endif
    const double rr = nz ? rsqrt_f64(s2) : 0.0;
    a_m = RAW ? (float)(s2 * rr) * mag_scale : fused_prologue_mag(MAGMODE, (float)(s2 * rr) * mag_scale);
    if (RAW) asm volatile("" : "+v"(a_m));
#if MPX_FUSED_VOIBRANCH
    if (voi) {
        a_r = fused_prologue_phase((float)(xr * rr));
        a_i = fused_prologue_phase((float)(xi * rr));
    } else {
        a_r = a_i = 0.0f;
    }
#else
    a_r = voi ? fused_prologue_phase((float)(xr * rr)) : 0.0f;
    a_i = voi ? fused_prologue_phase((float)(xi * rr)) : 0.0f;
#endif
}

#ifndef MPX_FUSED_EB
#define MPX_FUSED_EB 2
#endif
template <int P, int MAGMODE, bool RAW>
__device__ __forceinline__ void fused_split_operands(double (&re)[P], double (&im)[P], double zero2, float mag_scale, bool voi,
                                                     bool lane0, int src_lane, double wl_c, double wl_s, float (&vm)[P],
                                                     float (&vr)[P], float (&vi)[P], float& m0, float& m1, float& m2) {
    constexpr int EB = MPX_FUSED_EB;
#pragma unroll
    for (int qb = 0; qb < P / 2; qb += EB) {
        asm volatile("" : "+v"(re[f64_out_reg<P>(qb)]), "+v"(im[f64_out_reg<P>(qb)]));
        double zpr[EB], zpi[EB];
#pragma unroll
        for (int u = 0; u < EB; ++u) {
            const int i = f64_out_reg<P>(qb + u);
            unsigned a, b, c, d;
            split64(re[P - 1 - i], a, b);
            split64(im[P - 1 - i], c, d);
            zpr[u] = join64((unsigned)__shfl((int)a, src_lane), (unsigned)__shfl((int)b, src_lane));
            zpi[u] = join64((unsigned)__shfl((int)c, src_lane), (unsigned)__shfl((int)d, src_lane));
        }
#pragma unroll
        for (int u = 0; u < EB; ++u) {
            const int q = qb + u;
            const int i = f64_out_reg<P>(q);
            const int i0 = f64_out_reg<P>((P - q) % P);
            const double pr_ = lane0 ? re[i0] : zpr[u];
            const double pi_ = lane0 ? im[i0] : zpi[u];
            const double er = 0.5 * (re[i] + pr_), ei = 0.5 * (im[i] - pi_);
            const double orr = 0.5 * (im[i] + pi_), oi = -0.5 * (re[i] - pr_);
            constexpr int kq = 64 / (2 * P);
            const double cq = dc64(q * kq), sq = -ds64(q * kq);
            const double wr = wl_c * cq - wl_s * sq, wi = wl_c * sq + wl_s * cq;
            const double tr = wr * orr - wi * oi, ti = wr * oi + wi * orr;
            fused_operand<MAGMODE, RAW>(er + tr, ei + ti, zero2, mag_scale, voi, vm[2 * q], vr[2 * q], vi[2 * q]);
            fused_operand<MAGMODE, RAW>(er - tr, ti - ei, zero2, mag_scale, voi, vm[2 * q + 1], vr[2 * q + 1], vi[2 * q + 1]);
        }
    }
    constexpr int ih = f64_out_reg<P>(P / 2);
    fused_operand<MAGMODE, RAW>(re[ih], -im[ih], zero2, mag_scale, voi, m0, m1, m2);
}

template <int P, int NTP>
constexpr bool fused_pair() {
    return MPX_FUSED_PAIR != 0 && NTP >= 3 && kFusedWaves == 8 &&
           kFusedWaves * f64_win_floats<P>() >= 4 * 3 * kFusedWaves * kFusedAStride;
}

template <int P, int NTM, int NTP>
constexpr size_t lds_bytes_fused() {
    static_assert(kFusedWaves * f64_win_floats<P>() >= 2 * 3 * kFusedWaves * kFusedAStride, "the tiles live inside the window regions");
    constexpr size_t tiles = NTM + NTP;
    constexpr size_t work = sizeof(float) * (size_t)(kFusedWaves * P * kXStride + kFusedWaves * f64_win_floats<P>());
    constexpr size_t red = sizeof(float) * (size_t)(kFusedWaves * tiles * 4 * kFusedRedStride);
    static_assert(work >= red, "the reduction buffer must fit the regions it aliases");
    return sizeof(double) * (size_t)tw64_doubles<P>() + work + sizeof(float) * 32;
}

template <int P, int NTM, int NTP, int MAGMODE>
__attribute__((amdgpu_waves_per_eu(2, 2)))
__global__ __launch_bounds__(kFusedWaves * 64) void k_analysis_warp_fused(
    const float* __restrict__ sig, const long long* __restrict__ fpos, const int* __restrict__ fleft,
    const int* __restrict__ fright, long long nframes, const double* __restrict__ tw_g,
    const double* __restrict__ win_tab, int win_cap, const float* __restrict__ wpack, const float* __restrict__ whalf,
    const float* __restrict__ voiced, int mag_dim, int phase_dim, float* __restrict__ omag, float* __restrict__ oreal,
    float* __restrict__ oimag) {
    constexpr int M = 64 * P, N = 2 * M, LB = ilog2(P), T = NTM + NTP;
    extern __shared__ __attribute__((aligned(16))) double smem64[];
    double* tw = smem64;
    float* xbase = reinterpret_cast<float*>(smem64 + tw64_doubles<P>());
    const int lane_id = threadIdx.x & 63;
    const int wave = rfl((int)(threadIdx.x >> 6));
    float* xbuf = xbase + wave * (P * kXStride);
    const unsigned xbuf_byte = 8u * (unsigned)tw64_doubles<P>() + 4u * (unsigned)(wave * (P * kXStride));
    float* As = xbase + kFusedWaves * (P * kXStride);
    float* wbuf = As + wave * f64_win_floats<P>();
    const unsigned wbuf_byte = 8u * (unsigned)tw64_doubles<P>() + 4u * (unsigned)(kFusedWaves * (P * kXStride) + wave * f64_win_floats<P>());
    float* red = xbase;
    float* mid = xbase + kFusedWaves * (P * kXStride) + kFusedWaves * f64_win_floats<P>();
    for (int i = threadIdx.x; i < tw64_doubles<P>(); i += kFusedWaves * 64) {
        const int l = i / tw64_stride<P>(), c = i - l * tw64_stride<P>();
        const int src = (kF64Dit && c < 2 * P) ? l * tw64_stride<P>() + 2 * brev(c >> 1, LB) + (c & 1) : i;
        tw[i] = tw_g[src];
    }
    __syncthreads();

    double wl_s0, wl_c0;
    sincospi(-2.0 * (double)kappa<P>(lane_id) / (double)N, &wl_s0, &wl_c0);
    const long long nrounds = (nframes + kFusedWaves - 1) / kFusedWaves;
    const int li = lane_id & 15, g = lane_id >> 4;
    const f32x4_t* wp_wave = reinterpret_cast<const f32x4_t*>(wpack) + ((long long)wave * kFusedKH * T) * 64;

    for (long long rnd = blockIdx.x; rnd < nrounds; rnd += gridDim.x) {
        int lane = lane_id;
        double wl_s = wl_s0, wl_c = wl_c0;
        asm volatile("" : "+v"(lane), "+v"(wl_s), "+v"(wl_c));
        const int kap = kappa<P>(lane);
        const int src_lane = kappa<P>((64 - kap) & 63);
        const bool lane0 = (kap == 0);
        const long long f = rnd * kFusedWaves + wave;
        const bool has = f < nframes;
        double re[P], im[P];
        double zero2 = 1.0e-36;
        float mag_scale = 1.0f;
        bool voi = false;
        if (has) {
            f64_frame_transform<P>(sig, fpos[f], fleft[f], fright[f], win_tab, win_cap, tw, xbuf, xbuf_byte, wbuf, wbuf_byte, lane,
                                   re, im, zero2, mag_scale);
            voi = rfl((int)(voiced[f] != 0.0f)) != 0;
        } else {
#pragma unroll
            for (int j = 0; j < P; ++j) re[j] = im[j] = 0.0;
        }

        float vm[P], vr[P], vi[P];
        {
            float m0, m1, m2;
            fused_split_operands<P, MAGMODE, false>(re, im, zero2, mag_scale, voi, lane0, src_lane, wl_c, wl_s, vm, vr, vi, m0, m1, m2);
            if (lane0) {
                mid[0 * kFusedWaves + wave] = m0;
                mid[1 * kFusedWaves + wave] = m1;
                mid[2 * kFusedWaves + wave] = m2;
            }
        }
        constexpr bool M4 = kFusedKH == 1 && MPX_FUSED_M4 != 0;
        constexpr int TR = M4 ? 2 + NTP : T;
        f32x4_t acc[TR];
#pragma unroll
        for (int t = 0; t < TR; ++t) acc[t] = f32x4_t{0.0f, 0.0f, 0.0f, 0.0f};
        __syncthreads();
#ifdef MPX_FUSED_PRIO
        __builtin_amdgcn_s_setprio(MPX_FUSED_PRIO);
#endif
        if constexpr (M4) {
            constexpr int FR = 8 + NTP;
            const f32x4_t* wp4 = reinterpret_cast<const f32x4_t*>(wpack) + ((long long)wave * FR) * 64;
            f32x4_t bm[4][2], bp[NTP];
            {
                int wo = 0;
                asm volatile("" : "+s"(wo));
#pragma unroll
                for (int f = 0; f < 8; ++f) bm[f >> 1][f & 1] = wp4[wo + f * 64 + lane_id];
#pragma unroll
                for (int t = 0; t < NTP; ++t) bp[t] = wp4[wo + (8 + t) * 64 + lane_id];
            }
            const int arow4 = (4 * (lane_id >> 5) + (lane_id & 3)) * kFusedAStride + kFusedCols * wave;
            constexpr bool PAIR = fused_pair<P, NTP>();
            constexpr int NB = PAIR ? 4 : 2;
            auto publish = [&](int q) {
                float* row = As + (q & (NB - 1)) * (3 * kFusedWaves * kFusedAStride) + wave * kFusedAStride;
                row[kap] = vm[2 * q];
                row[64 + kap] = vm[2 * q + 1];
                row += kFusedWaves * kFusedAStride;
                row[kap] = vr[2 * q];
                row[64 + kap] = vr[2 * q + 1];
                row += kFusedWaves * kFusedAStride;
                row[kap] = vi[2 * q];
                row[64 + kap] = vi[2 * q + 1];
            };
#pragma unroll
            for (int q = 0; q < P / 2; ++q) {
                const float* tile = As + (q & (NB - 1)) * (3 * kFusedWaves * kFusedAStride);
                if (!PAIR) {
                    publish(q);
                    __syncthreads();
                } else if ((q & 1) == 0) {
                    publish(q);
                    publish(q + 1);
                    __syncthreads();
                }
                f32x4_t a4[4];
#pragma unroll
                for (int kg = 0; kg < 4; ++kg) a4[kg] = *reinterpret_cast<const f32x4_t*>(tile + arow4 + 4 * kg);
                const f32x4_t ap = *reinterpret_cast<const f32x4_t*>(
                    tile + ((li < 8 ? 1 : 2) * kFusedWaves + (li & (kFusedWaves - 1))) * kFusedAStride + kFusedCols * wave + 4 * g);
                int wo = (q + 1 < P / 2 ? q + 1 : q) * (kFusedWaves * FR * 64);
                asm volatile("" : "+s"(wo));
                f32x4_t cm[2][2];
#pragma unroll
                for (int i = 0; i < 4; ++i) cm[i >> 1][i & 1] = f32x4_t{0.0f, 0.0f, 0.0f, 0.0f};
#pragma unroll
                for (int kg = 0; kg < 4; ++kg) {
#pragma unroll
                    for (int e = 0; e < 4; ++e) {
#pragma unroll
                        for (int hf = 0; hf < 2; ++hf) {
#ifdef MPX_PROBE_FUSEDA_NOMFMA
                            cm[hf][e & 1][e] = fmaf(a4[kg][e], bm[kg][hf][e], cm[hf][e & 1][e]);
#else
                            cm[hf][e & 1] = __builtin_amdgcn_mfma_f32_4x4x1f32(a4[kg][e], bm[kg][hf][e], cm[hf][e & 1], 0, 0, 0);
#endif
                        }
                    }
                    if (q + 1 < P / 2) {
                        bm[kg][0] = wp4[wo + (2 * kg) * 64 + lane_id];
                        bm[kg][1] = wp4[wo + (2 * kg + 1) * 64 + lane_id];
                    }
                }
#pragma unroll
                for (int t = 0; t < NTP; ++t) {
                    f32x4_t ca = f32x4_t{0.0f, 0.0f, 0.0f, 0.0f};
#pragma unroll
                    for (int e = 0; e < 4; ++e) {
#ifdef MPX_PROBE_FUSEDA_NOMFMA
                        ca[e] = fmaf(ap[e], bp[t][e], ca[e]);
#else
                        ca = __builtin_amdgcn_mfma_f32_16x16x4f32(ap[e], bp[t][e], ca, 0, 0, 0);
#endif
                    }
                    if (q + 1 < P / 2) bp[t] = wp4[wo + (8 + t) * 64 + lane_id];
                    acc[2 + t] += ca;
                }
                acc[0] += cm[0][0] + cm[0][1];
                acc[1] += cm[1][0] + cm[1][1];
            }
        } else
#pragma unroll
        for (int q = 0; q < P / 2; ++q) {
            float* tile = As + (q & 1) * (3 * kFusedWaves * kFusedAStride);
            {
                float* row = tile + wave * kFusedAStride;
                row[kap] = vm[2 * q];
                row[64 + kap] = vm[2 * q + 1];
                row += kFusedWaves * kFusedAStride;
                row[kap] = vr[2 * q];
                row[64 + kap] = vr[2 * q + 1];
                row += kFusedWaves * kFusedAStride;
                row[kap] = vi[2 * q];
                row[64 + kap] = vi[2 * q + 1];
            }
            int wo = q * (kFusedWaves * kFusedKH * T * 64);
            asm volatile("" : "+s"(wo));
            const f32x4_t* wq = wp_wave + wo;
            f32x4_t bw[T];
#pragma unroll
            for (int t = 0; t < T; ++t) bw[t] = wq[t * 64 + lane_id];
            __syncthreads();
            f32x4_t ca[T];
#pragma unroll
            for (int t = 0; t < T; ++t) ca[t] = f32x4_t{0.0f, 0.0f, 0.0f, 0.0f};
#pragma unroll
            for (int h = 0; h < kFusedKH; ++h) {
                const int col = kFusedCols * wave + 16 * h + 4 * g;
                const f32x4_t am = *reinterpret_cast<const f32x4_t*>(tile + (li & (kFusedWaves - 1)) * kFusedAStride + col);
                const f32x4_t ap = *reinterpret_cast<const f32x4_t*>(
                    tile + ((li < 8 ? 1 : 2) * kFusedWaves + (li & (kFusedWaves - 1))) * kFusedAStride + col);
                if (h > 0) {
                    int who = h * (T * 64);
                    asm volatile("" : "+s"(who));
                    const f32x4_t* wh = wq + who;
#pragma unroll
                    for (int t = 0; t < T; ++t) bw[t] = wh[t * 64 + lane_id];
                }
#pragma unroll
                for (int e = 0; e < 4; ++e) {
#ifdef MPX_PROBE_FUSEDA_NOMFMA
#pragma unroll
                    for (int t = 0; t < NTM; ++t) ca[t][e] = fmaf(am[e], bw[t][e], ca[t][e]);
#pragma unroll
                    for (int t = NTM; t < T; ++t) ca[t][e] = fmaf(ap[e], bw[t][e], ca[t][e]);
#else
#pragma unroll
                    for (int t = 0; t < NTM; ++t) ca[t] = __builtin_amdgcn_mfma_f32_16x16x4f32(am[e], bw[t][e], ca[t], 0, 0, 0);
#pragma unroll
                    for (int t = NTM; t < T; ++t) ca[t] = __builtin_amdgcn_mfma_f32_16x16x4f32(ap[e], bw[t][e], ca[t], 0, 0, 0);
#endif
                }
            }
#pragma unroll
            for (int t = 0; t < T; ++t) acc[t] += ca[t];
        }
#ifdef MPX_FUSED_PRIO
        __builtin_amdgcn_s_setprio(0);
#endif
        __syncthreads();
#pragma unroll
        for (int t = 0; t < TR; ++t)
#pragma unroll
            for (int r = 0; r < 4; ++r) red[((wave * TR + t) * 4 + r) * kFusedRedStride + lane_id] = acc[t][r];
        __syncthreads();
        constexpr int kOuts = NTM + 2 * NTP;
        for (int idx = threadIdx.x; idx < kFusedWaves * kOuts * 16; idx += kFusedWaves * 64) {
            const int c = idx & 15, to = (idx >> 4) % kOuts, fr = idx / (16 * kOuts);
            const long long fo = rnd * kFusedWaves + fr;
            if (fo >= nframes) continue;
            const int sa = (to < NTM) ? 0 : ((to < NTM + NTP) ? 1 : 2);
            const int t = (sa == 2) ? to - NTP : to;
            const int row = (sa == 2) ? 8 + fr : fr;
            const int gg = row >> 2, r = row & 3;
            float y = 0.0f;
            if (M4 && sa == 0) {
                const int n = 16 * to + c;
#pragma unroll
                for (int w = 0; w < kFusedWaves; ++w)
                    y += red[((w * TR + (n >> 5)) * 4 + (fr & 3)) * kFusedRedStride + (n & 31) + 32 * (fr >> 2)];
            } else {
                const int tr = M4 ? t - NTM + 2 : t;
#pragma unroll
                for (int w = 0; w < kFusedWaves; ++w) y += red[((w * TR + tr) * 4 + r) * kFusedRedStride + c + 16 * gg];
            }
            y = fmaf(mid[sa * kFusedWaves + fr], whalf[t * 16 + c], y);
            if (sa == 0) {
                const int n = 16 * t + c;
                if (n >= mag_dim) continue;
                if (MAGMODE == 2) y = (y < -745.13321f) ? -1.0e10f : y;
                omag[fo * mag_dim + n] = y;
            } else {
                const int n = 16 * (t - NTM) + c;
                if (n >= phase_dim) continue;
                const float vo = voiced[fo];
                y = (vo == 0.0f) ? 0.0f : fminf(fmaxf(y * vo, -1.0f), 1.0f);
                (sa == 1 ? oreal : oimag)[fo * phase_dim + n] = y;
            }
        }
        __syncthreads();
    }
}

constexpr int kCrRows = 16;
constexpr int kCrRawRows = 9;
constexpr int kCrPhRows = 2 * 2 * 2 * kFusedWaves;
template <int P>
constexpr int cr_tile_floats() {
    constexpr int mag_rows = 3 * kCrRawRows + 2 * kCrRows;
    constexpr int win = kFusedWaves * f64_win_floats<P>(), tiles = (mag_rows > kCrPhRows ? mag_rows : kCrPhRows) * kFusedAStride;
    return win > tiles ? win : tiles;
}
template <int P>
constexpr int cr_halo_floats() { return 64 * P + 64; }
template <int P, int NTP>
constexpr size_t lds_bytes_fused_cr() {
    constexpr size_t work = sizeof(float) * (size_t)(kFusedWaves * P * kXStride + cr_tile_floats<P>());
    constexpr size_t red = sizeof(float) * (size_t)(kFusedWaves * (4 + NTP) * 4 * kFusedRedStride);
    static_assert(work >= red, "the reduction buffer must fit the regions it aliases");
    return sizeof(double) * (size_t)tw64_doubles<P>() + work + sizeof(float) * (48 + 3 * kCrRows);
}

__global__ __launch_bounds__(256) void k_cr_index(const int* __restrict__ row1, int n_const, long long nframes,
                                                  int* __restrict__ cstart) {
    const long long f = (long long)blockIdx.x * 256 + threadIdx.x;
    if (f > nframes) return;
    int lo = 0, hi = n_const;
    while (lo < hi) {
        const int m = (lo + hi) >> 1;
        if ((long long)row1[m] < f) lo = m + 1; else hi = m;
    }
    cstart[f] = lo;
}

template <int P, int NTP>
__attribute__((amdgpu_waves_per_eu(2, 2)))
__global__ __launch_bounds__(kFusedWaves * 64) void k_analysis_warp_fused_cr(
    const float* __restrict__ sig, const long long* __restrict__ fpos, const int* __restrict__ fleft,
    const int* __restrict__ fright, long long nframes, const double* __restrict__ tw_g,
    const double* __restrict__ win_tab, int win_cap, const float* __restrict__ wpack, const float* __restrict__ whalf,
    const float* __restrict__ rows_in_use, const int* __restrict__ row0, const int* __restrict__ row1,
    const float* __restrict__ rowt, const int* __restrict__ cstart, int frames_per_wg, int mag_dim, int phase_dim,
    float* __restrict__ omag, float* __restrict__ tr_out, float* __restrict__ ti_out, float* halo) {
    static_assert(kFusedWaves == 8 && kFusedKH == 1 && MPX_FUSED_M4 != 0, "the constant-rate form is written for 8 waves and the 4 x 4 magnitude product");
    constexpr int M = 64 * P, N = 2 * M, LB = ilog2(P), NC = P / 2, AS = kFusedAStride;
    constexpr int TR = 4 + NTP;
    constexpr int FR = 8 + NTP;
    extern __shared__ __attribute__((aligned(16))) double smem64[];
    double* tw = smem64;
    float* xbase = reinterpret_cast<float*>(smem64 + tw64_doubles<P>());
    const int lane_id = threadIdx.x & 63;
    const int wave = rfl((int)(threadIdx.x >> 6));
    float* xbuf = xbase + wave * (P * kXStride);
    const unsigned xbuf_byte = 8u * (unsigned)tw64_doubles<P>() + 4u * (unsigned)(wave * (P * kXStride));
    float* rawb = xbase + kFusedWaves * (P * kXStride);
    float* abuf = rawb + 3 * kCrRawRows * AS;
    float* wbuf = rawb + wave * f64_win_floats<P>();
    const unsigned wbuf_byte = 8u * (unsigned)tw64_doubles<P>() + 4u * (unsigned)(kFusedWaves * (P * kXStride) + wave * f64_win_floats<P>());
    float* red = xbase;
    float* mid = rawb + cr_tile_floats<P>();
    float* prm = mid + 48;
    for (int i = threadIdx.x; i < tw64_doubles<P>(); i += kFusedWaves * 64) {
        const int l = i / tw64_stride<P>(), c = i - l * tw64_stride<P>();
        const int src = (kF64Dit && c < 2 * P) ? l * tw64_stride<P>() + 2 * brev(c >> 1, LB) + (c & 1) : i;
        tw[i] = tw_g[src];
    }
    __syncthreads();

    double wl_s0, wl_c0;
    sincospi(-2.0 * (double)kappa<P>(lane_id) / (double)N, &wl_s0, &wl_c0);
    const int li = lane_id & 15, g = lane_id >> 4;
    const f32x4_t* wp4 = reinterpret_cast<const f32x4_t*>(wpack) + ((long long)wave * FR) * 64;
    float* hs = halo + (long long)blockIdx.x * (2 * cr_halo_floats<P>());
    const long long own_lo = (long long)blockIdx.x * frames_per_wg;
    const long long own_end = (own_lo + frames_per_wg < nframes) ? own_lo + frames_per_wg : nframes;
    const int arow4 = (4 * (lane_id >> 5) + (lane_id & 3)) * AS + kFusedCols * wave;
    const int jr = (int)(threadIdx.x >> 5), col4 = 4 * (int)(threadIdx.x & 31);

    int c_next0 = 0, c_next1 = 0;
    bool prm_ready = false;
    for (int r = 0;; ++r) {
        const long long a = own_lo - 1 + 8ll * r;
        const long long hi_lo = (r == 0) ? a + 1 : a;
        if (hi_lo >= own_end) break;
        const long long hi_hi = (a + 8 < own_end) ? a + 8 : own_end;
        const int c0 = (r == 0) ? cstart[hi_lo] : c_next0;
        const int c1 = (r == 0) ? cstart[hi_hi] : c_next1;
        const bool more = a + 8 < own_end;
        c_next0 = c1;
        c_next1 = more ? cstart[(a + 16 < own_end) ? a + 16 : own_end] : c1;
        int lane = lane_id;
        double wl_s = wl_s0, wl_c = wl_c0;
        asm volatile("" : "+v"(lane), "+v"(wl_s), "+v"(wl_c));
        const int kap = kappa<P>(lane);
        const int src_lane = kappa<P>((64 - kap) & 63);
        const bool lane0 = (kap == 0);
        const long long f = a + wave;
        const bool has = f >= 0 && f < own_end;
        double re[P], im[P];
        double zero2 = 1.0e-36;
        float mag_scale = 1.0f;
        bool voi = false;
        if (has) {
            f64_frame_transform<P>(sig, fpos[f], fleft[f], fright[f], win_tab, win_cap, tw, xbuf, xbuf_byte, wbuf, wbuf_byte, lane,
                                   re, im, zero2, mag_scale);
            voi = rfl((int)(rows_in_use[f] != 0.0f)) != 0;
        } else {
#pragma unroll
            for (int j = 0; j < P; ++j) re[j] = im[j] = 0.0;
        }
        float vm[P], vr[P], vi[P];
        const bool halo_on = r >= 1;
        const float* hp = hs + ((r + 1) & 1) * cr_halo_floats<P>();
        {
            float m0, m1, m2;
            fused_split_operands<P, 0, true>(re, im, zero2, mag_scale, voi, lane0, src_lane, wl_c, wl_s, vm, vr, vi, m0, m1, m2);
            if (lane0) {
                mid[wave] = m0;
                mid[9 + wave] = m1;
                mid[17 + wave] = m2;
            }
            if (wave == kFusedWaves - 1) {
                float* hw = hs + (r & 1) * cr_halo_floats<P>();
#pragma unroll
                for (int j = 0; j < P; ++j) hw[j * 64 + lane_id] = vm[j];
                if (lane0) {
                    hw[64 * P] = m0;
                    if (halo_on) mid[8] = hp[64 * P];
                }
            }
        }
        if (lane_id == 0) mid[32 + wave] = voi ? 1.0f : 0.0f;
        __syncthreads();
        bool any_ph = false;
#pragma unroll
        for (int w = 0; w < kFusedWaves; ++w) any_ph |= mid[32 + w] != 0.0f;
        any_ph = rfl((int)any_ph) != 0;

        constexpr int kHaloAhead = 4;
        const bool halo_w = halo_on && wave == kFusedWaves - 1;
        float hq[kHaloAhead][2];
#pragma unroll
        for (int u = 0; u < kHaloAhead; ++u) hq[u][0] = hq[u][1] = 0.0f;
        if (halo_w && c1 > c0) {
#pragma unroll
            for (int u = 0; u < kHaloAhead; ++u) {
                hq[u][0] = hp[(2 * u) * 64 + lane_id];
                hq[u][1] = hp[(2 * u + 1) * 64 + lane_id];
            }
        }

        f32x4_t accp[NTP];
#pragma unroll
        for (int t = 0; t < NTP; ++t) accp[t] = f32x4_t{0.0f, 0.0f, 0.0f, 0.0f};
        if (any_ph) {
            f32x4_t bp[2][NTP];
#pragma unroll
            for (int u = 0; u < 2; ++u) {
                int wo = u * (kFusedWaves * FR * 64);
                asm volatile("" : "+s"(wo));
#pragma unroll
                for (int t = 0; t < NTP; ++t) bp[u][t] = wp4[wo + (8 + t) * 64 + lane_id];
            }
#pragma unroll
            for (int q = 0; q < NC; ++q) {
                float* tile = rawb + (((q >> 1) & 1) * 2 + (q & 1)) * (2 * kFusedWaves * AS);
                if ((q & 1) == 0) {
#pragma unroll
                    for (int u = 0; u < 2; ++u) {
                        float* row = tile + u * (2 * kFusedWaves * AS) + wave * AS;
                        row[kap] = vr[2 * (q + u)];
                        row[64 + kap] = vr[2 * (q + u) + 1];
                        row += kFusedWaves * AS;
                        row[kap] = vi[2 * (q + u)];
                        row[64 + kap] = vi[2 * (q + u) + 1];
                    }
                    __syncthreads();
                }
                const f32x4_t ap = *reinterpret_cast<const f32x4_t*>(tile + li * AS + kFusedCols * wave + 4 * g);
                int wo = (q + 2 < NC ? q + 2 : q) * (kFusedWaves * FR * 64);
                asm volatile("" : "+s"(wo));
#pragma unroll
                for (int t = 0; t < NTP; ++t) {
                    f32x4_t ca = f32x4_t{0.0f, 0.0f, 0.0f, 0.0f};
#pragma unroll
                    for (int e = 0; e < 4; ++e) ca = __builtin_amdgcn_mfma_f32_16x16x4f32(ap[e], bp[q & 1][t][e], ca, 0, 0, 0);
                    if (q + 2 < NC) bp[q & 1][t] = wp4[wo + (8 + t) * 64 + lane_id];
                    accp[t] += ca;
                }
            }
            __syncthreads();
        }

        for (int cb = c0, sweep = 0; sweep == 0 || cb < c1; cb += kCrRows, ++sweep) {
            const bool ph = sweep == 0 && any_ph;
            const int nrows = (c1 - cb < kCrRows) ? c1 - cb : kCrRows;
            const int npass = nrows > 8 ? 2 : (nrows > 0 ? 1 : 0);
            if (!(sweep == 0 && prm_ready)) {
                if (threadIdx.x < kCrRows && (int)threadIdx.x < nrows) {
                    prm[3 * threadIdx.x] = __int_as_float(row0[cb + threadIdx.x]);
                    prm[3 * threadIdx.x + 1] = __int_as_float(row1[cb + threadIdx.x]);
                    prm[3 * threadIdx.x + 2] = rowt[cb + threadIdx.x];
                }
                __syncthreads();
            }
            int lo_rel = 0, hi_rel = 0;
            float tt = 0.0f;
            if (jr < nrows) {
                lo_rel = __float_as_int(prm[3 * jr]) - (int)a;
                hi_rel = __float_as_int(prm[3 * jr + 1]) - (int)a;
                tt = prm[3 * jr + 2];
                if (lo_rel < 0) lo_rel = 8;
            }
            f32x4_t acc[4];
#pragma unroll
            for (int t = 0; t < 4; ++t) acc[t] = f32x4_t{0.0f, 0.0f, 0.0f, 0.0f};
            auto chunks = [&](auto np_tag) {
                constexpr int NP = decltype(np_tag)::value;
                f32x4_t bm[2][4][2];
#pragma unroll
                for (int u = 0; u < 2; ++u) {
                    int wo = u * (kFusedWaves * FR * 64);
                    asm volatile("" : "+s"(wo));
#pragma unroll
                    for (int fi = 0; fi < 8; ++fi) bm[u][fi >> 1][fi & 1] = wp4[wo + fi * 64 + lane_id];
                }
                const bool builder = NP == 2 || wave < kFusedWaves / 2;
                if (sweep > 0 && halo_w) {
#pragma unroll
                    for (int u = 0; u < kHaloAhead; ++u) {
                        hq[u][0] = hp[(2 * u) * 64 + lane_id];
                        hq[u][1] = hp[(2 * u + 1) * 64 + lane_id];
                    }
                }
                auto publish = [&](int q) {
                    float* row = rawb + (q % 3) * (kCrRawRows * AS) + wave * AS;
                    row[kap] = vm[2 * q];
                    row[64 + kap] = vm[2 * q + 1];
                    if (halo_w) {
                        float* hr = rawb + (q % 3) * (kCrRawRows * AS) + 8 * AS;
                        hr[kap] = hq[q % kHaloAhead][0];
                        hr[64 + kap] = hq[q % kHaloAhead][1];
                        if (q + kHaloAhead < NC) {
                            hq[q % kHaloAhead][0] = hp[(2 * (q + kHaloAhead)) * 64 + lane_id];
                            hq[q % kHaloAhead][1] = hp[(2 * (q + kHaloAhead) + 1) * 64 + lane_id];
                        }
                    }
                };
                auto build = [&](int q) {
                    const float* rb = rawb + (q % 3) * (kCrRawRows * AS);
                    const f32x4_t x0 = *reinterpret_cast<const f32x4_t*>(rb + lo_rel * AS + col4);
                    const f32x4_t x1 = *reinterpret_cast<const f32x4_t*>(rb + hi_rel * AS + col4);
                    f32x4_t av;
#pragma unroll
                    for (int e = 0; e < 4; ++e) av[e] = fused_prologue_mag(0, fmaf(x1[e] - x0[e], tt, x0[e]));
                    *reinterpret_cast<f32x4_t*>(abuf + (q & 1) * (kCrRows * AS) + jr * AS + col4) = av;
                };
                publish(0);
// ... 46 lines not shown
            }
            __syncthreads();
#pragma unroll
            for (int t = 0; t < 4; ++t)
#pragma unroll
                for (int rr = 0; rr < 4; ++rr) red[((wave * TR + t) * 4 + rr) * kFusedRedStride + lane_id] = acc[t][rr];
            if (ph) {
#pragma unroll
                for (int t = 0; t < NTP; ++t)
#pragma unroll
                    for (int rr = 0; rr < 4; ++rr) red[((wave * TR + 4 + t) * 4 + rr) * kFusedRedStride + lane_id] = accp[t][rr];
            }
            __syncthreads();
            for (int idx = threadIdx.x; idx < kCrRows * 64; idx += kFusedWaves * 64) {
                const int jo = idx >> 6, n = idx & 63;
                if (jo >= nrows || n >= mag_dim) continue;
                const int p = jo >> 3, fr = jo & 7;
                float y = 0.0f;
#pragma unroll
                for (int w = 0; w < kFusedWaves; ++w)
                    y += red[((w * TR + 2 * p + (n >> 5)) * 4 + (fr & 3)) * kFusedRedStride + (n & 31) + 32 * (fr >> 2)];
                int lo = __float_as_int(prm[3 * jo]) - (int)a;
                const int hi = __float_as_int(prm[3 * jo + 1]) - (int)a;
                if (lo < 0) lo = 8;
                const float xm = fmaf(mid[hi] - mid[lo], prm[3 * jo + 2], mid[lo]);
                omag[(long long)(cb + jo) * mag_dim + n] = fmaf(fused_prologue_mag(0, xm), whalf[n], y);
            }
            if (ph) {
                for (int idx = threadIdx.x; idx < kFusedWaves * 2 * NTP * 16; idx += kFusedWaves * 64) {
                    const int c = idx & 15, to = (idx >> 4) % (2 * NTP), fr = idx / (16 * 2 * NTP);
                    const long long fo = a + fr;
                    if (fo < 0 || fo >= own_end) continue;
                    const int sa = (to < NTP) ? 1 : 2;
                    const int tp = (sa == 2) ? to - NTP : to;
                    const int row = (sa == 2) ? 8 + fr : fr;
                    const int n = 16 * tp + c;
                    if (n >= phase_dim || mid[32 + fr] == 0.0f) continue;
                    float y = 0.0f;
#pragma unroll
                    for (int w = 0; w < kFusedWaves; ++w)
                        y += red[((w * TR + 4 + tp) * 4 + (row & 3)) * kFusedRedStride + c + 16 * (row >> 2)];
                    y = fmaf(mid[(sa == 1 ? 9 : 17) + fr], whalf[(4 + tp) * 16 + c], y);
                    (sa == 1 ? tr_out : ti_out)[fo * phase_dim + n] = y;
                }
            }
            __syncthreads();
            if (fetch) {
                prm[3 * threadIdx.x] = __int_as_float(n_lo);
                prm[3 * threadIdx.x + 1] = __int_as_float(n_hi);
                prm[3 * threadIdx.x + 2] = n_t;
            }
            prm_ready = last_sweep && more;
        }
    }
}

__global__ void k_tables_init_f64(int P, double* __restrict__ tab) {
    const int l = blockIdx.x, i = threadIdx.x;
    const int M = 64 * P, stride = 2 * P + 2;
    int lb = 0;
    while ((1 << lb) < P) ++lb;
    if (i < P) {
        int k1 = 0;
        for (int b = 0; b < lb; ++b) k1 |= ((i >> b) & 1) << (lb - 1 - b);
        const int r = (int)(((long long)l * k1) % M);
        double sn, cs;
        sincospi(2.0 * (double)r / (double)M, &sn, &cs);
        tab[l * stride + 2 * i + 0] = cs;
        tab[l * stride + 2 * i + 1] = sn;
    } else if (i == P) {
        tab[l * stride + 2 * i + 0] = 0.0;
        tab[l * stride + 2 * i + 1] = 0.0;
    }
}

}

using namespace mpx;

extern "C" {

size_t mpx_tables_f64_bytes(int fft_len) {
    const int P = p_of(fft_len);
    return P ? sizeof(double) * 64 * (size_t)(2 * P + 2) : 0;
}

int mpx_tables_f64_init(void* stream, int fft_len, void* tables) {
    const int P = p_of(fft_len);
    if (!P) return fail(MPX_ERR_ARG, "mpx_tables_f64_init: fft_len must be 1024, 2048 or 4096%s");
    if (!tables) return fail(MPX_ERR_ARG, "mpx_tables_f64_init: null tables%s");
    hipLaunchKernelGGL(k_tables_init_f64, dim3(64), dim3(64), 0, (hipStream_t)stream, P, (double*)tables);
    MPX_HIP_CHECK(hipGetLastError());
    return MPX_OK;
}

int mpx_analysis_frames_f64(void* stream, int fft_len, const void* tables_f64, const float* sig, const int64_t* frame_pos,
                            const int32_t* frame_left, const int32_t* frame_right, int64_t n_frames, float* out_mag,
                            float* out_real, float* out_imag, int64_t ld, const float* rows_in_use) {
    return mpx_analysis_frames_f64w(stream, fft_len, tables_f64, sig, frame_pos, frame_left, frame_right, n_frames, out_mag,
                                    out_real, out_imag, ld, rows_in_use, nullptr, 0);
}

int mpx_analysis_frames_f64w(void* stream, int fft_len, const void* tables_f64, const float* sig, const int64_t* frame_pos,
                             const int32_t* frame_left, const int32_t* frame_right, int64_t n_frames, float* out_mag,
                             float* out_real, float* out_imag, int64_t ld, const float* rows_in_use, const double* win_tab,
                             int32_t win_cap) {
    const int P = p_of(fft_len);
    if (!P) return fail(MPX_ERR_ARG, "mpx_analysis_frames_f64: fft_len must be 1024, 2048 or 4096%s");
    if (n_frames < 0) return fail(MPX_ERR_ARG, "mpx_analysis_frames_f64: negative n_frames%s");
    if (ld < fft_len / 2 + 1) return fail(MPX_ERR_ARG, "mpx_analysis_frames_f64: ld < fft_len/2 + 1%s");
    if (win_tab && win_cap < 0) return fail(MPX_ERR_ARG, "mpx_analysis_frames_f64w: negative win_cap%s");
    if (n_frames == 0) return MPX_OK;
    if (!tables_f64 || !sig || !frame_pos || !frame_left || !frame_right || !out_mag || !out_real || !out_imag)
        return fail(MPX_ERR_ARG, "mpx_analysis_frames_f64: null pointer%s");
    const dim3 grid(grid_for(n_frames, kAna64Waves)), block(kAna64Waves * 64);
    hipStream_t s = (hipStream_t)stream;
#define MPX_LAUNCH_A64(PP)                                                                                        \
    do {                                                                                                          \
        if (int rc = set_lds(k_analysis_f64<PP>, lds_bytes_ana64<PP>())) return rc;                               \
        hipLaunchKernelGGL(k_analysis_f64<PP>, grid, block, lds_bytes_ana64<PP>(), s, sig,                        \
                           (const long long*)frame_pos, frame_left, frame_right, (long long)n_frames,             \
                           (const double*)tables_f64, out_mag, out_real, out_imag, (long long)ld, rows_in_use,    \
                           win_tab, (int)win_cap);                                                                \
    } while (0)
    if (P == 32) MPX_LAUNCH_A64(32);
    else if (P == 16) MPX_LAUNCH_A64(16);
    else MPX_LAUNCH_A64(8);
#undef MPX_LAUNCH_A64
    MPX_HIP_CHECK(hipGetLastError());
    return MPX_OK;
}


int mpx_analysis_compressed_fused(void* stream, int fft_len, const void* tables_f64, const float* sig,
                                  const int64_t* frame_pos, const int32_t* frame_left, const int32_t* frame_right,
                                  int64_t n_frames, const double* win_tab, int32_t win_cap, const float* wpack,
                                  const float* whalf, int32_t mag_dim, int32_t phase_dim, const float* voiced,
                                  int32_t mag_fbank, float* out_mag, float* out_real, float* out_imag) {
    const int P = p_of(fft_len);
    if (P != 32 && P != 16) return fail(MPX_ERR_ARG, "mpx_analysis_compressed_fused: fft_len must be 2048 or 4096%s");
    if (n_frames < 0) return fail(MPX_ERR_ARG, "mpx_analysis_compressed_fused: negative n_frames%s");
    if (mag_dim <= 0 || mag_dim > 64 || phase_dim <= 0 || phase_dim > 48)
        return fail(MPX_ERR_ARG, "mpx_analysis_compressed_fused: mag_dim must be in 1..64 and phase_dim in 1..48%s");
    if (win_tab && win_cap < 0) return fail(MPX_ERR_ARG, "mpx_analysis_compressed_fused: negative win_cap%s");
    if (n_frames == 0) return MPX_OK;
    if (!tables_f64 || !sig || !frame_pos || !frame_left || !frame_right || !wpack || !whalf || !voiced || !out_mag ||
        !out_real || !out_imag)
        return fail(MPX_ERR_ARG, "mpx_analysis_compressed_fused: null pointer%s");
    const long long nrounds = (n_frames + kFusedWaves - 1) / kFusedWaves;
    const long long slots = (long long)device_cus() * (8 / kFusedWaves);
    const dim3 grid((unsigned)(nrounds < slots ? nrounds : slots)), block(kFusedWaves * 64);
    hipStream_t s = (hipStream_t)stream;
    const int ntp = (phase_dim + 15) / 16;
#define MPX_FUSED_GO(PP, NTP_, MM)                                                                                        \
    do {                                                                                                                  \
        if (int rc = set_lds(k_analysis_warp_fused<PP, 4, NTP_, MM>, (lds_bytes_fused<PP, 4, NTP_>()))) return rc;        \
        hipLaunchKernelGGL((k_analysis_warp_fused<PP, 4, NTP_, MM>), grid, block, (lds_bytes_fused<PP, 4, NTP_>()), s, sig, \
                           (const long long*)frame_pos, frame_left, frame_right, (long long)n_frames,                     \
                           (const double*)tables_f64, win_tab, (int)win_cap, wpack, whalf, voiced, (int)mag_dim,          \
                           (int)phase_dim, out_mag, out_real, out_imag);                                                  \
    } while (0)
#define MPX_FUSED_P(PP)                                                     \
    do {                                                                    \
        if (ntp == 1 && !mag_fbank) MPX_FUSED_GO(PP, 1, 0);                 \
        else if (ntp == 1) MPX_FUSED_GO(PP, 1, 2);                          \
        else if (ntp == 2 && !mag_fbank) MPX_FUSED_GO(PP, 2, 0);            \
        else if (ntp == 2) MPX_FUSED_GO(PP, 2, 2);                          \
        else if (!mag_fbank) MPX_FUSED_GO(PP, 3, 0);                        \
        else MPX_FUSED_GO(PP, 3, 2);                                        \
    } while (0)
    if (P == 32) MPX_FUSED_P(32);
    else MPX_FUSED_P(16);
#undef MPX_FUSED_P
#undef MPX_FUSED_GO
    MPX_HIP_CHECK(hipGetLastError());
    return MPX_OK;
}

int64_t mpx_analysis_compressed_fused_cr_work_bytes(int fft_len, int64_t n_frames) {
    const int P = p_of(fft_len);
    if ((P != 32 && P != 16) || n_frames < 0) return MPX_ERR_ARG;
    const int64_t idx = ((int64_t)sizeof(int32_t) * (n_frames + 1) + 255) / 256 * 256;
    return idx + (int64_t)sizeof(float) * device_cus() * 2 * (64 * P + 64);
}

int mpx_analysis_compressed_fused_cr(void* stream, int fft_len, const void* tables_f64, const float* sig,
                                     const int64_t* frame_pos, const int32_t* frame_left, const int32_t* frame_right,
                                     int64_t n_frames, const double* win_tab, int32_t win_cap, const float* wpack,
                                     const float* whalf, int32_t mag_dim, int32_t phase_dim, const float* rows_in_use,
                                     const int32_t* row0, const int32_t* row1, const float* row_t, int64_t n_const,
                                     float* out_mag, float* tmp_real, float* tmp_imag, void* work) {
    const int P = p_of(fft_len);
    if (P != 32 && P != 16) return fail(MPX_ERR_ARG, "mpx_analysis_compressed_fused_cr: fft_len must be 2048 or 4096%s");
    if (n_frames < 0 || n_const < 0 || n_const > 2147483647ll || n_frames > 2147483647ll)
        return fail(MPX_ERR_ARG, "mpx_analysis_compressed_fused_cr: bad frame count%s");
    if (mag_dim <= 0 || mag_dim > 64 || phase_dim <= 0 || phase_dim > 48)
        return fail(MPX_ERR_ARG, "mpx_analysis_compressed_fused_cr: mag_dim must be in 1..64 and phase_dim in 1..48%s");
    if (win_tab && win_cap < 0) return fail(MPX_ERR_ARG, "mpx_analysis_compressed_fused_cr: negative win_cap%s");
    if (kFusedWaves != 8 || kFusedKH != 1 || MPX_FUSED_M4 == 0)
        return fail(MPX_ERR_ARG, "mpx_analysis_compressed_fused_cr: this build's fused kernel has another tile shape%s");
    if (n_frames == 0) return MPX_OK;
    if (!tables_f64 || !sig || !frame_pos || !frame_left || !frame_right || !wpack || !whalf || !rows_in_use || !work ||
        !tmp_real || !tmp_imag || (n_const > 0 && (!row0 || !row1 || !row_t || !out_mag)))
        return fail(MPX_ERR_ARG, "mpx_analysis_compressed_fused_cr: null pointer%s");
    hipStream_t s = (hipStream_t)stream;
    int* cstart = (int*)work;
    float* halo = (float*)((char*)work + ((int64_t)sizeof(int32_t) * (n_frames + 1) + 255) / 256 * 256);
    hipLaunchKernelGGL(k_cr_index, dim3((unsigned)((n_frames + 1 + 255) / 256)), dim3(256), 0, s, row1, (int)n_const,
                       (long long)n_frames, cstart);
    const long long slots = device_cus();
    const long long per = (n_frames + slots - 1) / slots;
    const long long fw = 8 * ((per + 1 + 7) / 8) - 1;
    const dim3 grid((unsigned)((n_frames + fw - 1) / fw)), block(kFusedWaves * 64);
    const int ntp = (phase_dim + 15) / 16;
#define MPX_FUSED_CR_GO(PP, NTP_)                                                                                       \
    do {                                                                                                                \
        if (int rc = set_lds(k_analysis_warp_fused_cr<PP, NTP_>, (lds_bytes_fused_cr<PP, NTP_>()))) return rc;          \
        hipLaunchKernelGGL((k_analysis_warp_fused_cr<PP, NTP_>), grid, block, (lds_bytes_fused_cr<PP, NTP_>()), s, sig, \
                           (const long long*)frame_pos, frame_left, frame_right, (long long)n_frames,                   \
                           (const double*)tables_f64, win_tab, (int)win_cap, wpack, whalf, rows_in_use, row0, row1,     \
                           row_t, (const int*)cstart, (int)fw, (int)mag_dim, (int)phase_dim, out_mag, tmp_real,         \
                           tmp_imag, halo);                                                                             \
    } while (0)
#define MPX_FUSED_CR_P(PP)                       \
    do {                                         \
        if (ntp == 1) MPX_FUSED_CR_GO(PP, 1);    \
        else if (ntp == 2) MPX_FUSED_CR_GO(PP, 2); \
        else MPX_FUSED_CR_GO(PP, 3);             \
    } while (0)
    if (P == 32) MPX_FUSED_CR_P(32);
    else MPX_FUSED_CR_P(16);
#undef MPX_FUSED_CR_P
#undef MPX_FUSED_CR_GO
    MPX_HIP_CHECK(hipGetLastError());
    return MPX_OK;
}

int mpx_analysis_compressed_fused_tiles(int32_t mag_dim, int32_t phase_dim, int32_t* ntm, int32_t* ntp) {
    if (mag_dim <= 0 || mag_dim > 64 || phase_dim <= 0 || phase_dim > 48 || !ntm || !ntp)
        return fail(MPX_ERR_ARG, "mpx_analysis_compressed_fused_tiles: bad arguments%s");
    *ntm = 4;
    *ntp = (phase_dim + 15) / 16;
    return MPX_OK;
}

int mpx_analysis_compressed_fused_waves(void) { return kFusedWaves; }

int mpx_analysis_compressed_fused_layout(void) { return (kFusedKH == 1 && MPX_FUSED_M4 != 0) ? 1 : 0; }

int mpx_analysis_compressed_fused_blocks_per_cu(int fft_len, int32_t phase_dim) {
    const int P = p_of(fft_len);
    if ((P != 32 && P != 16) || phase_dim <= 0 || phase_dim > 48) return MPX_ERR_ARG;
    const int ntp = (phase_dim + 15) / 16;
    int nb = -1;
#define MPX_FUSED_OCC(PP, NTP_)                                                                                       \
    do {                                                                                                              \
        if (set_lds(k_analysis_warp_fused<PP, 4, NTP_, 0>, (lds_bytes_fused<PP, 4, NTP_>()))) return -1;              \
        if (hipOccupancyMaxActiveBlocksPerMultiprocessor(&nb, k_analysis_warp_fused<PP, 4, NTP_, 0>, kFusedWaves * 64, \
                                                         (lds_bytes_fused<PP, 4, NTP_>())) != hipSuccess)             \
            return -1;                                                                                                \
    } while (0)
    if (P == 32) {
        if (ntp == 1) MPX_FUSED_OCC(32, 1); else if (ntp == 2) MPX_FUSED_OCC(32, 2); else MPX_FUSED_OCC(32, 3);
    } else {
        if (ntp == 1) MPX_FUSED_OCC(16, 1); else if (ntp == 2) MPX_FUSED_OCC(16, 2); else MPX_FUSED_OCC(16, 3);
    }
#undef MPX_FUSED_OCC
    return nb;
}

}
```

magphase_amd/csrc/magphase_hip.hip:

```cpp
#include "mpx_common.hpp"

namespace mpx {

#ifdef MPX_ANA_NT
#define MPX_ST(dst, val) __builtin_nontemporal_store((val), &(dst))
#else
#define MPX_ST(dst, val) ((dst) = (val))
#endif

#ifndef MPX_ANA_QUEUE
#define MPX_ANA_QUEUE 0
#endif
template <int P>
__global__ __launch_bounds__(kAnaThreads) void k_analysis(const float* __restrict__ sig,
                                                          const long long* __restrict__ fpos,
                                                          const int* __restrict__ fleft,
                                                          const int* __restrict__ fright, long long nframes,
                                                          const float* __restrict__ tw_g, float* __restrict__ omag,
                                                          float* __restrict__ oreal, float* __restrict__ oimag,
                                                          long long ld) {
    constexpr int M = 64 * P, N = 2 * M, LB = ilog2(P), kTile = 64 * P;
    extern __shared__ __attribute__((aligned(16))) float smem[];
    float* tw = smem;
    const int lane_id = threadIdx.x & 63;
// ... 570 lines not shown
        }
        asm volatile("s_waitcnt lgkmcnt(0)" ::: "memory");
        MPX_PHASE(6);
        __hip_atomic_store(turn, ticket + 1, __ATOMIC_RELAXED, __HIP_MEMORY_SCOPE_WORKGROUP);
        if constexpr (JB < P / 2) {
            asm volatile("" ::: "memory");
            MPX_FEAT_LOAD(JB, P / 2, false);
        }
        cur = nxt;
        MPX_PHASE(7);
#ifdef MPX_PROBE_ENDTIME
        ++probe_frames;
#endif
    }
#ifdef MPX_PROBE_ENDTIME
    if (lane_id == 0) {
        const int w = (blockIdx.x * kPairWaves + wave) % 8192;
        g_endprobe[4 * w + 0] = probe_t0;
        g_endprobe[4 * w + 1] = wall_clock64();
        g_endprobe[4 * w + 2] = (unsigned long long)probe_frames;
        g_endprobe[4 * w + 3] = clock64() - probe_c0;
#ifdef MPX_PROBE_PHASES
        asm volatile("s_waitcnt lgkmcnt(0)" ::: "memory");
        for (int i = 0; i < 8; ++i) g_phaseprobe[8 * w + i] = probe_ph[i];
#endif
    }
#endif
}

__global__ __launch_bounds__(256) void k_ola_fixup(const RunDesc* __restrict__ runs, const float* __restrict__ strips,
                                                   float* __restrict__ pcm) {
    const RunDesc rd = runs[blockIdx.x];
    const int e0 = (rd.fix_lo & ~63) + (int)blockIdx.y * 1024;
    if (e0 >= rd.fix_hi) return;
    const float* strip = strips + rd.strip_off;
    float* out = pcm + rd.out_base;
#pragma unroll
    for (int r = 0; r < 4; ++r) {
        const int e = e0 + 256 * r + (int)threadIdx.x;
        if (e >= rd.fix_lo && e < rd.fix_hi) out[e] += strip[e];
    }
}

__global__ __launch_bounds__(256) void k_ola_gather(const float* __restrict__ frames, int N,
                                                    const int* __restrict__ utt_frame_off,
                                                    const int* __restrict__ pm_rel,
                                                    const int* __restrict__ out_start,
                                                    const long long* __restrict__ out_off,
                                                    float* __restrict__ pcm) {
    const int u = blockIdx.y;
    const long long o0 = out_off[u];
    const long long len = out_off[u + 1] - o0;
    const long long t = (long long)blockIdx.x * blockDim.x + threadIdx.x;
    if (t >= len) return;
    const int f0 = utt_frame_off[u], f1 = utt_frame_off[u + 1];
    const long long b = t + out_start[u];
    int lo = f0, hi = f1;
    const long long thr = b - N;
    while (lo < hi) {
        const int mid = (lo + hi) >> 1;
        if ((long long)pm_rel[mid] > thr) hi = mid; else lo = mid + 1;
    }
    float acc = 0.0f;
    for (int i = lo; i < f1; ++i) {
        const long long off = b - pm_rel[i];
        if (off < 0) break;
        acc += frames[(long long)i * N + off];
    }
    pcm[o0 + t] = acc;
}

typedef float f4a4 __attribute__((ext_vector_type(4), aligned(4)));
constexpr int kLerpWaves = 4;

__global__ __launch_bounds__(kLerpWaves * 64) void k_rows_lerp(int H, const float* __restrict__ sm,
                                                               const float* __restrict__ sr, const float* __restrict__ si,
                                                               long long lds, const int* __restrict__ row0,
                                                               const int* __restrict__ row1,
                                                               const float* __restrict__ rowt, long long n_out,
                                                               float* __restrict__ dm, float* __restrict__ dr,
                                                               float* __restrict__ di, long long ldd) {
    const long long c = (long long)blockIdx.x * kLerpWaves + (threadIdx.x >> 6);
    if (c >= n_out) return;
    const int lane = threadIdx.x & 63;
    const long long a = row0[c], b = row1[c];
    const float t = rowt[c];
    const long long oa = a * lds, ob = b * lds, od = c * ldd;
    const int nv = H >> 2;
    if (a == b) {
        for (int v = lane; v < nv; v += 64) {
            const f4a4 x = *reinterpret_cast<const f4a4*>(sm + oa + 4 * v);
            const f4a4 y = *reinterpret_cast<const f4a4*>(sr + oa + 4 * v);
            const f4a4 z = *reinterpret_cast<const f4a4*>(si + oa + 4 * v);
            *reinterpret_cast<f4a4*>(dm + od + 4 * v) = x;
            *reinterpret_cast<f4a4*>(dr + od + 4 * v) = y;
            *reinterpret_cast<f4a4*>(di + od + 4 * v) = z;
        }
    } else {
        for (int v = lane; v < nv; v += 64) {
            const f4a4 x0 = *reinterpret_cast<const f4a4*>(sm + oa + 4 * v);
            const f4a4 y0 = *reinterpret_cast<const f4a4*>(sr + oa + 4 * v);
            const f4a4 z0 = *reinterpret_cast<const f4a4*>(si + oa + 4 * v);
            const f4a4 x1 = *reinterpret_cast<const f4a4*>(sm + ob + 4 * v);
            const f4a4 y1 = *reinterpret_cast<const f4a4*>(sr + ob + 4 * v);
            const f4a4 z1 = *reinterpret_cast<const f4a4*>(si + ob + 4 * v);
            f4a4 x, y, z;
#pragma unroll
            for (int e = 0; e < 4; ++e) {
                x[e] = fmaf(x1[e] - x0[e], t, x0[e]);
                y[e] = fmaf(y1[e] - y0[e], t, y0[e]);
                z[e] = fmaf(z1[e] - z0[e], t, z0[e]);
            }
            *reinterpret_cast<f4a4*>(dm + od + 4 * v) = x;
            *reinterpret_cast<f4a4*>(dr + od + 4 * v) = y;
            *reinterpret_cast<f4a4*>(di + od + 4 * v) = z;
        }
    }
    const int k = 4 * nv + lane;
    if (k < H) {
        dm[od + k] = fmaf(sm[ob + k] - sm[oa + k], t, sm[oa + k]);
        dr[od + k] = fmaf(sr[ob + k] - sr[oa + k], t, sr[oa + k]);
        di[od + k] = fmaf(si[ob + k] - si[oa + k], t, si[oa + k]);
    }
}

__global__ void k_tables_init(int P, float* __restrict__ tab) {
    const int l = blockIdx.x, i = threadIdx.x;
    const int M = 64 * P, stride = 2 * P + 4;
    int lb = 0;
    while ((1 << lb) < P) ++lb;
    if (i < P) {
        int k1 = 0;
        for (int b = 0; b < lb; ++b) k1 |= ((i >> b) & 1) << (lb - 1 - b);
        const int r = (int)(((long long)l * k1) % M);
        double sn, cs;
        sincospi(2.0 * (double)r / (double)M, &sn, &cs);
        tab[l * stride + 2 * i + 0] = (float)cs;
        tab[l * stride + 2 * i + 1] = (float)sn;
    } else if (i < P + 2) {
        tab[l * stride + 2 * i + 0] = 0.0f;
        tab[l * stride + 2 * i + 1] = 0.0f;
    }
}

}

using namespace mpx;

extern "C" {

int mpx_version(void) { return MPX_ABI_VERSION; }

const char* mpx_last_error(void) { return g_err; }

size_t mpx_tables_bytes(int fft_len) {
    const int P = p_of(fft_len);
    return P ? sizeof(float) * 64 * (size_t)(2 * P + 4) : 0;
}

int mpx_tables_init(void* stream, int fft_len, void* tables) {
    const int P = p_of(fft_len);
    if (!P) return fail(MPX_ERR_ARG, "mpx_tables_init: fft_len must be 1024, 2048 or 4096%s");
    if (!tables) return fail(MPX_ERR_ARG, "mpx_tables_init: null tables%s");
    hipLaunchKernelGGL(k_tables_init, dim3(64), dim3(64), 0, (hipStream_t)stream, P, (float*)tables);
    MPX_HIP_CHECK(hipGetLastError());
    return MPX_OK;
}

int64_t mpx_feat_ld(int fft_len) {
    if (!p_of(fft_len)) return 0;
    return (int64_t)(fft_len / 2 + 1);
}

int mpx_analysis_frames(void* stream, int fft_len, const void* tables, const float* sig, const int64_t* frame_pos,
                        const int32_t* frame_left, const int32_t* frame_right, int64_t n_frames, float* out_mag,
                        float* out_real, float* out_imag, int64_t ld) {
    const int P = p_of(fft_len);
    if (!P) return fail(MPX_ERR_ARG, "mpx_analysis_frames: fft_len must be 1024, 2048 or 4096%s");
    if (n_frames < 0) return fail(MPX_ERR_ARG, "mpx_analysis_frames: negative n_frames%s");
    if (ld < fft_len / 2 + 1) return fail(MPX_ERR_ARG, "mpx_analysis_frames: ld < fft_len/2 + 1%s");
    if (n_frames == 0) return MPX_OK;
    if (!tables || !sig || !frame_pos || !frame_left || !frame_right || !out_mag || !out_real || !out_imag)
        return fail(MPX_ERR_ARG, "mpx_analysis_frames: null pointer%s");
    const dim3 grid(grid_for(n_frames, kAnaWaves)), block(kAnaThreads);
    hipStream_t s = (hipStream_t)stream;
    if (P == 32) {
        if (int rc = set_lds(k_analysis<32>, lds_bytes_ana<32>())) return rc;
        hipLaunchKernelGGL(k_analysis<32>, grid, block, lds_bytes_ana<32>(), s, sig, (const long long*)frame_pos,
                           frame_left, frame_right, (long long)n_frames, (const float*)tables, out_mag, out_real,
                           out_imag, (long long)ld);
    } else if (P == 16) {
        if (int rc = set_lds(k_analysis<16>, lds_bytes_ana<16>())) return rc;
        hipLaunchKernelGGL(k_analysis<16>, grid, block, lds_bytes_ana<16>(), s, sig, (const long long*)frame_pos,
                           frame_left, frame_right, (long long)n_frames, (const float*)tables, out_mag, out_real,
                           out_imag, (long long)ld);
    } else {
        if (int rc = set_lds(k_analysis<8>, lds_bytes_ana<8>())) return rc;
        hipLaunchKernelGGL(k_analysis<8>, grid, block, lds_bytes_ana<8>(), s, sig, (const long long*)frame_pos,
                           frame_left, frame_right, (long long)n_frames, (const float*)tables, out_mag, out_real,
                           out_imag, (long long)ld);
    }
    MPX_HIP_CHECK(hipGetLastError());
    return MPX_OK;
}

int mpx_synthesis_lossless_frames(void* stream, int fft_len, const void* tables, const float* mag, const float* real,
                                  const float* imag, int64_t n_frames, float* frames_out, int64_t ld) {
    const int P = p_of(fft_len);
    if (!P) return fail(MPX_ERR_ARG, "mpx_synthesis_lossless_frames: fft_len must be 1024, 2048 or 4096%s");
    if (n_frames < 0) return fail(MPX_ERR_ARG, "mpx_synthesis_lossless_frames: negative n_frames%s");
    if (ld < fft_len / 2 + 1) return fail(MPX_ERR_ARG, "mpx_synthesis_lossless_frames: ld < fft_len/2 + 1%s");
    if (n_frames == 0) return MPX_OK;
    if (!tables || !mag || !real || !imag || !frames_out)
        return fail(MPX_ERR_ARG, "mpx_synthesis_lossless_frames: null pointer%s");
    const dim3 grid(grid_for(n_frames)), block(kThreads);
    hipStream_t s = (hipStream_t)stream;
    if (P == 32) {
        if (int rc = set_lds(k_synth_lossless<32>, lds_bytes<32>())) return rc;
        hipLaunchKernelGGL(k_synth_lossless<32>, grid, block, lds_bytes<32>(), s, mag, real, imag,
                           (long long)n_frames, (const float*)tables, frames_out, (long long)ld);
    } else if (P == 16) {
        if (int rc = set_lds(k_synth_lossless<16>, lds_bytes<16>())) return rc;
        hipLaunchKernelGGL(k_synth_lossless<16>, grid, block, lds_bytes<16>(), s, mag, real, imag,
                           (long long)n_frames, (const float*)tables, frames_out, (long long)ld);
    } else {
        if (int rc = set_lds(k_synth_lossless<8>, lds_bytes<8>())) return rc;
        hipLaunchKernelGGL(k_synth_lossless<8>, grid, block, lds_bytes<8>(), s, mag, real, imag,
                           (long long)n_frames, (const float*)tables, frames_out, (long long)ld);
    }
    MPX_HIP_CHECK(hipGetLastError());
    return MPX_OK;
}

int mpx_ola_gather(void* stream, int fft_len, const float* frames, int32_t n_utts, const int32_t* utt_frame_off,
                   const int32_t* pm_rel, const int32_t* out_start, const int64_t* out_off, int64_t max_out_len,
                   float* pcm_out) {
    if (!p_of(fft_len)) return fail(MPX_ERR_ARG, "mpx_ola_gather: fft_len must be 1024, 2048 or 4096%s");
    if (n_utts < 0 || max_out_len < 0) return fail(MPX_ERR_ARG, "mpx_ola_gather: negative size%s");
    if (n_utts == 0 || max_out_len == 0) return MPX_OK;
    if (!frames || !utt_frame_off || !pm_rel || !out_start || !out_off || !pcm_out)
        return fail(MPX_ERR_ARG, "mpx_ola_gather: null pointer%s");
    if (n_utts > 65535) return fail(MPX_ERR_ARG, "mpx_ola_gather: at most 65535 utterances per call%s");
    const dim3 block(256), grid((unsigned)((max_out_len + 255) / 256), (unsigned)n_utts);
    hipLaunchKernelGGL(k_ola_gather, grid, block, 0, (hipStream_t)stream, frames, fft_len, utt_frame_off, pm_rel,
                       out_start, (const long long*)out_off, pcm_out);
    MPX_HIP_CHECK(hipGetLastError());
    return MPX_OK;
}

int64_t mpx_host_const_to_var_scan(const double* centres, const double* shift_c, int64_t n, double* shifts_out,
                                   double* locs_out) {
#pragma clang fp contract(off)
    if (!centres || !shift_c || !shifts_out || !locs_out || n < 2) return -1;
    for (int64_t i = 0; i < 2 * n; ++i) shifts_out[i] = locs_out[i] = 0.0;
    double pos = centres[n - 1];
    for (int64_t i = 2 * n - 1; i >= 1; --i) {
        locs_out[i] = pos;
        if (!(pos >= centres[0] && pos <= centres[n - 1])) return i + 1;
        int64_t lo = 0, hi = n;
        while (lo < hi) {
            const int64_t mid = (lo + hi) >> 1;
            if (centres[mid] < pos) lo = mid + 1; else hi = mid;
        }
        int64_t idx = lo < 1 ? 1 : (lo > n - 1 ? n - 1 : lo);
        const double x_lo = centres[idx - 1], x_hi = centres[idx], y_lo = shift_c[idx - 1], y_hi = shift_c[idx];
        const double slope = (y_hi - y_lo) / (x_hi - x_lo);
        const double prod = slope * (pos - x_lo);
        const double y = prod + y_lo;
        shifts_out[i] = y;
        pos = pos - y;
    }
    return 0;
}

int64_t mpx_host_const_to_var_scan_cap(const double* centres, const double* shift_c, int64_t n, double* shifts_out,
                                       double* locs_out, int64_t cap) {
#pragma clang fp contract(off)
    if (!centres || !shift_c || !shifts_out || !locs_out || n < 1 || cap < 1) return -1;
    double pos = centres[n - 1];
    for (int64_t i = cap - 1; i >= 0; --i) {
        if (!(pos >= centres[0] && pos <= centres[n - 1])) return i + 1;
        locs_out[i] = pos;
        double y;
        if (n == 1) {
            y = shift_c[0];
        } else {
            int64_t lo = 0, hi = n;
            while (lo < hi) {
                const int64_t mid = (lo + hi) >> 1;
                if (centres[mid] < pos) lo = mid + 1; else hi = mid;
            }
            const int64_t idx = lo < 1 ? 1 : (lo > n - 1 ? n - 1 : lo);
            const double x_lo = centres[idx - 1], x_hi = centres[idx], y_lo = shift_c[idx - 1], y_hi = shift_c[idx];
            const double slope = (y_hi - y_lo) / (x_hi - x_lo);
            const double prod = slope * (pos - x_lo);
            y = prod + y_lo;
        }
        shifts_out[i] = y;
        pos = pos - y;
    }
    return (pos >= centres[0] && pos <= centres[n - 1]) ? -2 : 0;
}


#ifdef MPX_PROBE_ENDTIME
int mpx_probe_endtimes(unsigned long long* host, int n_words) {
// ... 140 lines not shown
```

magphase_amd/csrc/mpx_common.hpp:

```cpp
#pragma once
#include <hip/hip_runtime.h>
#include <cmath>
#include <cstdint>
#include <cstdio>
#include <cstring>
#include <mutex>
#include <vector>

#include "../../include/magphase_hip.h"
#include "wave_fft.hpp"

namespace mpx {

inline thread_local char g_err[512] = "";

inline int fail(int code, const char* fmt, const char* detail = "") {
    snprintf(g_err, sizeof(g_err), fmt, detail);
    return code;
}

#define MPX_HIP_CHECK(expr)                                                       \
    do {                                                                          \
        hipError_t e__ = (expr);                                                  \
        if (e__ != hipSuccess) return fail(MPX_ERR_HIP, #expr ": %s", hipGetErrorString(e__)); \
    } while (0)

#ifndef MPX_WAVES_PER_BLOCK
#define MPX_WAVES_PER_BLOCK 8
#endif
constexpr int kWavesPerBlock = MPX_WAVES_PER_BLOCK;
constexpr int kThreads = kWavesPerBlock * 64;

template <int P>
constexpr size_t lds_bytes() {
    return sizeof(float) * (size_t)(tw_floats<P>() + kWavesPerBlock * P * kXStride);
}

#ifndef MPX_ANA_WAVES
#define MPX_ANA_WAVES 12
#endif
constexpr int kAnaWaves = MPX_ANA_WAVES;
constexpr int kAnaThreads = kAnaWaves * 64;
template <int P>
constexpr size_t lds_bytes_ana() {
    return sizeof(float) * (size_t)(tw_floats<P>() + kAnaWaves * P * kXStride + 4);
}

__device__ __forceinline__ int rfl(int v) { return __builtin_amdgcn_readfirstlane(v); }

#ifdef MPX_PHASE_MARKS
#define MPX_MARK(name) asm volatile("; MPX_MARK " name ::: "memory")
#else
#define MPX_MARK(name) do { } while (0)
#endif
template <unsigned LIVE, int K>
__device__ __forceinline__ void mpx_pin_live(float (&a)[K]) {
#ifdef MPX_PHASE_MARKS
#pragma unroll
    for (int i = 0; i < K; ++i)
        if ((LIVE >> i) & 1u) asm volatile("" : "+v"(a[i]));
#else
    (void)a;
#endif
}
template <int K>
__device__ __forceinline__ void mpx_pin(float (&a)[K]) {
#ifdef MPX_PHASE_MARKS
    static_assert(K % 4 == 0, "pinned in groups of four");
#pragma unroll
    for (int i = 0; i < K; i += 4) asm volatile("" : "+v"(a[i]), "+v"(a[i + 1]), "+v"(a[i + 2]), "+v"(a[i + 3]));
#else
    (void)a;
#endif
}

__device__ __forceinline__ long long queue_pull(unsigned* ctr, long long begin) {
    unsigned v = 0u;
    if ((threadIdx.x & 63) == 0) v = atomicAdd(ctr, 1u);
    return begin + (long long)(unsigned)__builtin_amdgcn_readfirstlane((int)v);
}
__device__ __forceinline__ void block_frame_range(long long nframes, long long& fb, long long& fe) {
    fb = (long long)blockIdx.x * nframes / (long long)gridDim.x;
    fe = (long long)(blockIdx.x + 1) * nframes / (long long)gridDim.x;
}

__device__ __forceinline__ float sin2_halfpi(float t) {
    const float u = t - 0.5f;
    const float u2 = u * u;
    float p = fmaf(u2, 7.721838616e-02f, -5.980441939e-01f);
    p = fmaf(u2, p, 2.550031194e+00f);
    p = fmaf(u2, p, -5.167706866e+00f);
    p = fmaf(u2, p, 3.141592580e+00f);
    return fmaf(0.5f * u, p, 0.5f);
}

__device__ __forceinline__ float half_window(int k, int L, int LR, int kadd, float invL, float invR, int wtype) {
    const bool rising = k <= L;
    const int num = rising ? k + kadd : LR - k;
    const float inv = rising ? invL : invR;
    const float t = (float)num * inv;
    return (wtype == 0) ? sin2_halfpi(t) : t * t * __builtin_amdgcn_sqrtf(t);
}

__device__ __forceinline__ float hann_half(int k, int L, int LR, int kadd, float invL, float invR) {
    return half_window(k, L, LR, kadd, invL, invR, 0);
}

struct FrameGeom {
    const float* base;
    int L, LR, len, rot, kadd;
    float invL, invR;
};

__host__ __device__ __forceinline__ int frame_len(int L, int R, int N) { return (L + R + 1 < N) ? L + R + 1 : N; }
__host__ __device__ __forceinline__ int frame_rot(int L, int N) { return (L < N) ? L : 0; }

__host__ __device__ constexpr int noise_tile_len(int P, bool compact) { return compact ? 32 * P : 64 * P; }
#define MPX_NOISE_TILES(len, tile_len) (((len) + (tile_len) - 1) / (tile_len))
#define MPX_NOISE_ROW_ACTIVE(m0, n_lo, n_hi) (((m0) < (n_lo)) || ((m0) + 127 >= (n_hi)))
__host__ __device__ inline void frame_cost_terms(int L, int R, int N, int P, bool compact, int (&terms)[3]) {
    const int len = frame_len(L, R, N), rot = frame_rot(L, N);
    const int tile_len = noise_tile_len(P, compact), ntiles = MPX_NOISE_TILES(len, tile_len);
    int rows = 0;
    for (int j = 0; j < P; ++j) rows += MPX_NOISE_ROW_ACTIVE(128 * j, len - rot, N - rot) ? 1 : 0;
    terms[0] = 1;
    terms[1] = rows * ntiles;
    terms[2] = ntiles - 1;
}

constexpr int kSupportNarrow = 4;
__host__ __device__ inline int frame_support_class(int L, int R, int N) {
    const int P = N / 128;
    if (P == 32 && L >= 0 && R >= 0 && L <= 128 * kSupportNarrow && R <= 128 * kSupportNarrow - 1) return kSupportNarrow;
    return P / 2;
}
#define MPX_ARM_END_CLASS() asm volatile("; end of the class arm")
#define MPX_ARM_END_FULL() asm volatile("; end of the full arm")
template <int P>
__host__ __device__ constexpr unsigned support_zero_rows(int W) {
    unsigned z = 0u;
    for (int j = 0; j < P; ++j)
        if (!(j < W || j >= P - W)) z |= 1u << j;
    return z;
}
__host__ __device__ constexpr bool support_row_live(int q, int W, int P) { return q >= P / 2 - W && q < P / 2 + W; }

__host__ __device__ inline int row_store_phase(const float* row) { return (int)(((unsigned long long)row >> 2) & 31u); }
__host__ __device__ constexpr int row_store_count(int P) { return 2 * (P / 2) + 2; }
__host__ __device__ constexpr bool row_asc_prev(int lane, int s) { return lane >= 64 - s; }
__host__ __device__ constexpr int row_asc_base(int lane, bool prev) { return prev ? lane - 64 : lane; }
__host__ __device__ constexpr int row_asc_off(int q) { return 64 * q; }
__host__ __device__ constexpr bool row_mir_cur(int lane, int s) { return lane <= s; }
__host__ __device__ constexpr int row_mir_base(int lane, bool cur, int M) { return cur ? M - 64 - lane : M - lane; }
__host__ __device__ constexpr int row_mir_off(int q) { return -64 * (q - 1); }
__host__ __device__ constexpr bool row_mir_tail_live(int lane, bool cur) { return lane == 0 || !cur; }
__host__ __device__ constexpr int row_store_index(int st, int lane, int s, int P) {
    const int HP = P / 2, M = 64 * P, q = st >> 1;
    const bool prev = row_asc_prev(lane, s), cur = row_mir_cur(lane, s);
    if (st == 2 * HP) return prev ? row_asc_base(lane, true) + row_asc_off(HP) : -1;
    if (st == 2 * HP + 1) return row_mir_tail_live(lane, cur) ? row_mir_base(lane, cur, M) + row_mir_off(HP) : -1;
    if (!(st & 1)) return (q == 0 && prev) ? -1 : row_asc_base(lane, prev) + row_asc_off(q);
    return (q == 0 && !cur) ? -1 : row_mir_base(lane, cur, M) + row_mir_off(q);
}

__device__ __forceinline__ FrameGeom frame_geom(const float* __restrict__ sig, long long pos, int L, int R, int N) {
    FrameGeom g;
    g.L = L;
    g.LR = L + R;
    g.len = min(g.LR + 1, N);
    g.rot = (L < N) ? L : 0;
    g.kadd = (L == 0) ? 1 : 0;
    g.invL = (L > 0) ? 1.0f / (float)L : 1.0f;
// ... 517 lines not shown
```

magphase_amd/csrc/wave_fft.hpp:

```cpp
#pragma once
#include <hip/hip_runtime.h>

namespace mpx {

constexpr int kXStride = 68;

template <int P>
__host__ __device__ constexpr int tw_stride() { return 2 * P + 4; }
template <int P>
__host__ __device__ constexpr int tw_floats() { return 64 * tw_stride<P>(); }

__host__ __device__ constexpr int ilog2(int v) { return v <= 1 ? 0 : 1 + ilog2(v >> 1); }

__host__ __device__ constexpr int brev(int i, int bits) {
    int r = 0;
    for (int b = 0; b < bits; ++b) r |= ((i >> b) & 1) << (bits - 1 - b);
    return r;
}

__device__ __forceinline__ constexpr float c32(int k) {
    constexpr float t[16] = {1.000000000e+00f, 9.807852507e-01f, 9.238795042e-01f, 8.314695954e-01f,
                             7.071067691e-01f, 5.555702448e-01f, 3.826834261e-01f, 1.950903237e-01f,
                             0.0f,             -1.950903237e-01f, -3.826834261e-01f, -5.555702448e-01f,
                             -7.071067691e-01f, -8.314695954e-01f, -9.238795042e-01f, -9.807852507e-01f};
// ... 162 lines not shown
template <int P, int SIGN, int S_HI, int S_LO = 1>
__device__ __forceinline__ void fft_inreg_stages(float (&re)[P], float (&im)[P]) {
    fft_inreg_pruned_stage<P, SIGN, S_HI, 0u, kAllRegs, S_LO>(re, im);
}

template <int P, int SIGN>
__device__ __forceinline__ void fft_inreg_dit(float (&re)[P], float (&im)[P]) {
#pragma unroll
    for (int s = 1; s < P; s <<= 1) {
#pragma unroll
        for (int g = 0; g < P; g += 2 * s) {
#pragma unroll
            for (int k = 0; k < s; ++k) {
                const int i0 = g + k, i1 = g + k + s;
                const int t = k * (16 / s);
                const float ar = re[i0], ai = im[i0], br = re[i1], bi = im[i1];
                if (t == 0) {
                    re[i0] = ar + br;
                    im[i0] = ai + bi;
                    re[i1] = ar - br;
                    im[i1] = ai - bi;
                } else if (t == 8) {
                    re[i0] = (SIGN < 0) ? ar + bi : ar - bi;
                    im[i0] = (SIGN < 0) ? ai - br : ai + br;
                    re[i1] = (SIGN < 0) ? ar - bi : ar + bi;
                    im[i1] = (SIGN < 0) ? ai + br : ai - br;
                } else {
                    const float c = c32(t), sn = (SIGN < 0) ? -s32(t) : s32(t);
                    const float o0r = fmaf(br, c, fmaf(-bi, sn, ar));
                    const float o0i = fmaf(br, sn, fmaf(bi, c, ai));
                    re[i0] = o0r;
                    im[i0] = o0i;
                    re[i1] = fmaf(2.0f, ar, -o0r);
                    im[i1] = fmaf(2.0f, ai, -o0i);
                }
            }
        }
    }
}

template <int P, bool NAT = false>
__device__ __forceinline__ void lds_transpose(float (&x)[P], float* xbuf, int lane) {
    constexpr int LB = ilog2(P);
#pragma unroll
    for (int i = 0; i < P; ++i) xbuf[(NAT ? i : brev(i, LB)) * kXStride + lane] = x[i];
    wave_sync();
    const float4* src = reinterpret_cast<const float4*>(xbuf + (lane % P) * kXStride + (lane / P) * P);
#pragma unroll
    for (int q = 0; q < P / 4; ++q) {
        const float4 v = src[q];
        x[4 * q + 0] = v.x;
        x[4 * q + 1] = v.y;
        x[4 * q + 2] = v.z;
        x[4 * q + 3] = v.w;
    }
    wave_sync();
}

typedef unsigned u32x2 __attribute__((ext_vector_type(2)));
__device__ __forceinline__ void swap32(float& a, float& b) {
    const u32x2 r = __builtin_amdgcn_permlane32_swap(__builtin_bit_cast(unsigned, a), __builtin_bit_cast(unsigned, b),
                                                     false, false);
    const unsigned r0 = r.x, r1 = r.y;
    a = __builtin_bit_cast(float, r0);
    b = __builtin_bit_cast(float, r1);
}
__device__ __forceinline__ void swap16(float& a, float& b) {
    const u32x2 r = __builtin_amdgcn_permlane16_swap(__builtin_bit_cast(unsigned, a), __builtin_bit_cast(unsigned, b),
                                                     false, false);
    const unsigned r0 = r.x, r1 = r.y;
    a = __builtin_bit_cast(float, r0);
    b = __builtin_bit_cast(float, r1);
}

template <int P, int SIGN, int PARTNER, int TWN>
__device__ __forceinline__ void cross_lane_stage(float (&re)[P], float (&im)[P], bool upper, bool rot, int lane) {
    if (PARTNER >= 16) {
#pragma unroll
        for (int lp = 0; lp < P; lp += 2) {
            if (PARTNER == 32) { swap32(re[lp], re[lp + 1]); swap32(im[lp], im[lp + 1]); }
            else { swap16(re[lp], re[lp + 1]); swap16(im[lp], im[lp + 1]); }
        }
#pragma unroll
        for (int lp = 0; lp < P; lp += 2) {
            const float a = re[lp], b = re[lp + 1], c = im[lp], d = im[lp + 1];
            re[lp] = a + b;
            re[lp + 1] = a - b;
            im[lp] = c + d;
            im[lp + 1] = c - d;
        }
#pragma unroll
        for (int lp = 0; lp < P; lp += 2) {
            if (PARTNER == 32) { swap32(re[lp], re[lp + 1]); swap32(im[lp], im[lp + 1]); }
            else { swap16(re[lp], re[lp + 1]); swap16(im[lp], im[lp + 1]); }
        }
    } else {
        const float sg = upper ? -1.0f : 1.0f;
#pragma unroll
        for (int lp = 0; lp < P; ++lp) {
            const float orr = __builtin_bit_cast(float, __builtin_amdgcn_update_dpp(0, __builtin_bit_cast(int, re[lp]), 0x128, 0xf, 0xf, false));
            const float oii = __builtin_bit_cast(float, __builtin_amdgcn_update_dpp(0, __builtin_bit_cast(int, im[lp]), 0x128, 0xf, 0xf, false));
            re[lp] = fmaf(re[lp], sg, orr);
            im[lp] = fmaf(im[lp], sg, oii);
        }
    }
    if (upper) {
#pragma unroll
        for (int lp = 1; lp < P; ++lp) {
            const float cw = (TWN == 64) ? c64(lp) : ((TWN == 32) ? c32(lp) : c32(2 * lp));
            const float sw0 = (TWN == 64) ? s64(lp) : ((TWN == 32) ? s32(lp) : s32(2 * lp));
            const float sw = (SIGN < 0) ? -sw0 : sw0;
            const float xr = re[lp] * cw - im[lp] * sw;
            const float xi = re[lp] * sw + im[lp] * cw;
            re[lp] = xr;
            im[lp] = xi;
        }
    }
    if (PARTNER == 4 * P) {
        const int e = (lane >> 3) & 3;
        constexpr float kR2 = 7.071067691e-01f;
        const float fc = (e == 0) ? 1.0f : ((e == 1) ? kR2 : ((e == 2) ? 0.0f : -kR2));
        const float fs0 = (e == 0) ? 0.0f : ((e == 1) ? kR2 : ((e == 2) ? 1.0f : kR2));
        const float fs = (SIGN < 0) ? -fs0 : fs0;
        if (upper) {
#pragma unroll
            for (int lp = 0; lp < P; ++lp) {
                const float xr = re[lp] * fc - im[lp] * fs;
                const float xi = re[lp] * fs + im[lp] * fc;
                re[lp] = xr;
                im[lp] = xi;
            }
        }
    }
    if (PARTNER == 2 * P) {
        if (rot) {
#pragma unroll
            for (int lp = 0; lp < P; ++lp) {
                const float xr = re[lp], xi = im[lp];
                re[lp] = (SIGN < 0) ? xi : -xi;
                im[lp] = (SIGN < 0) ? -xr : xr;
            }
        }
    }
}

template <int P>
__device__ __forceinline__ int kappa(int lane) {
    if (P == 32) return lane;
    if (P == 16) return (lane & 15) | (((lane >> 5) & 1) << 4) | (((lane >> 4) & 1) << 5);
    return (lane & 7) | (((lane >> 5) & 1) << 3) | (lane & 16) | (((lane >> 3) & 1) << 5);
}

template <int P, int SIGN>
__device__ __forceinline__ void wave_fft_front(float (&re)[P], float (&im)[P], const float* tw, float* xbuf, int lane) {
    fft_inreg<P, SIGN>(re, im);
    const float4* trow = reinterpret_cast<const float4*>(tw + lane * tw_stride<P>());
#pragma unroll
    for (int q = 0; q < P / 2; ++q) {
        const float4 w = trow[q];
#pragma unroll
        for (int e = 0; e < 2; ++e) {
            const int i = 2 * q + e;
            const float wc = e ? w.z : w.x;
            const float ws = (SIGN < 0) ? -(e ? w.w : w.y) : (e ? w.w : w.y);
            const float xr = re[i] * wc - im[i] * ws;
            const float xi = re[i] * ws + im[i] * wc;
            re[i] = xr;
            im[i] = xi;
        }
    }
    lds_transpose<P>(re, xbuf, lane);
    lds_transpose<P>(im, xbuf, lane);
    if (P == 32) {
        cross_lane_stage<P, SIGN, 32, 64>(re, im, (lane & 32) != 0, false, lane);
    } else if (P == 16) {
        cross_lane_stage<P, SIGN, 32, 64>(re, im, (lane & 32) != 0, (lane & 48) == 48, lane);
        cross_lane_stage<P, SIGN, 16, 32>(re, im, (lane & 16) != 0, false, lane);
    } else {
        cross_lane_stage<P, SIGN, 32, 64>(re, im, (lane & 32) != 0, false, lane);
        cross_lane_stage<P, SIGN, 16, 32>(re, im, (lane & 16) != 0, (lane & 24) == 24, lane);
        cross_lane_stage<P, SIGN, 8, 16>(re, im, (lane & 8) != 0, false, lane);
    }
}

template <int P, int SIGN>
__device__ __forceinline__ void wave_fft(float (&re)[P], float (&im)[P], const float* tw, float* xbuf, int lane) {
    wave_fft_front<P, SIGN>(re, im, tw, xbuf, lane);
    fft_inreg<P, SIGN>(re, im);
}

template <int P>
__device__ __forceinline__ int tw_nat_index(int i) {
    constexpr int LB = ilog2(P);
    const int l = i / tw_stride<P>(), c = i - l * tw_stride<P>();
    return (c < 2 * P) ? l * tw_stride<P>() + 2 * brev(c >> 1, LB) + (c & 1) : i;
}

template <int P, int SIGN>
__device__ __forceinline__ void wave_fft_dit_front(float (&re)[P], float (&im)[P], const float* twn, float* xbuf, int lane) {
    fft_inreg_dit<P, SIGN>(re, im);
    const float4* trow = reinterpret_cast<const float4*>(twn + lane * tw_stride<P>());
#pragma unroll
    for (int q = 0; q < P / 2; ++q) {
        const float4 w = trow[q];
#pragma unroll
        for (int e = 0; e < 2; ++e) {
            const int i = 2 * q + e;
            const float wc = e ? w.z : w.x;
            const float ws = (SIGN < 0) ? -(e ? w.w : w.y) : (e ? w.w : w.y);
            const float xr = re[i] * wc - im[i] * ws;
            const float xi = re[i] * ws + im[i] * wc;
            re[i] = xr;
            im[i] = xi;
        }
    }
    lds_transpose<P, true>(re, xbuf, lane);
    lds_transpose<P, true>(im, xbuf, lane);
    if (P == 32) {
        cross_lane_stage<P, SIGN, 32, 64>(re, im, (lane & 32) != 0, false, lane);
    } else if (P == 16) {
        cross_lane_stage<P, SIGN, 32, 64>(re, im, (lane & 32) != 0, (lane & 48) == 48, lane);
        cross_lane_stage<P, SIGN, 16, 32>(re, im, (lane & 16) != 0, false, lane);
    } else {
        cross_lane_stage<P, SIGN, 32, 64>(re, im, (lane & 32) != 0, false, lane);
        cross_lane_stage<P, SIGN, 16, 32>(re, im, (lane & 16) != 0, (lane & 24) == 24, lane);
        cross_lane_stage<P, SIGN, 8, 16>(re, im, (lane & 8) != 0, false, lane);
    }
}

template <int P, int SIGN>
__device__ __forceinline__ void wave_fft_dit_back(float (&re)[P], float (&im)[P]) {
    constexpr int LB = ilog2(P);
    float tr[P], ti[P];
#pragma unroll
    for (int r = 0; r < P; ++r) {
        tr[brev(r, LB)] = re[r];
        ti[brev(r, LB)] = im[r];
    }
    fft_inreg_dit<P, SIGN>(tr, ti);
#pragma unroll
    for (int r = 0; r < P; ++r) {
        re[r] = tr[r];
        im[r] = ti[r];
    }
}

template <int P, int SIGN>
__device__ __forceinline__ void wave_fft_dit(float (&re)[P], float (&im)[P], const float* twn, float* xbuf, int lane) {
    wave_fft_dit_front<P, SIGN>(re, im, twn, xbuf, lane);
    wave_fft_dit_back<P, SIGN>(re, im);
}

template <int P>
__host__ __device__ constexpr int tw_half_stride() { return P + 4; }
template <int P>
__host__ __device__ constexpr int tw_half_floats() { return 64 * tw_half_stride<P>(); }

template <int P>
__device__ __forceinline__ float4 tw_half_pad(const float* twh, int lane) {
    return *reinterpret_cast<const float4*>(twh + lane * tw_half_stride<P>() + P);
}

template <int P, bool NAT = false>
__device__ __forceinline__ void lds_transpose_half(float (&x)[P], float* xbuf, int lane) {
    static_assert(P == 32, "the half-height transpose pairs lanes lam, lam ^ 16: P == 32 only");
    constexpr int LB = ilog2(P), HP = P / 2;
    float t[P];
    const int row = lane & (HP - 1);
    const int swz = ((row + 4) >> 3) & 1;
    const float4* src = reinterpret_cast<const float4*>(xbuf + row * kXStride + (lane / P) * P +
                                                        (((lane >> (LB - 1)) & 1) ^ swz) * HP);
    const int lane_s = lane ^ HP;
#pragma unroll
    for (int h = 0; h < 2; ++h) {
#pragma unroll
        for (int i = 0; i < P; ++i) {
            const int k1 = NAT ? i : brev(i, LB);
            const int r = k1 & (HP - 1);
            if ((k1 >> (LB - 1)) == h) xbuf[r * kXStride + ((((r + 4) >> 3) & 1) ? lane_s : lane)] = x[i];
        }
        wave_sync();
#pragma unroll
        for (int q = 0; q < HP / 4; ++q) {
            const float4 v = src[q];
            t[h * HP + 4 * q + 0] = v.x;
            t[h * HP + 4 * q + 1] = v.y;
            t[h * HP + 4 * q + 2] = v.z;
            t[h * HP + 4 * q + 3] = v.w;
        }
        wave_sync();
    }
#pragma unroll
    for (int j = 0; j < HP; ++j) swap16(t[j], t[HP + j]);
#pragma unroll
    for (int j = 0; j < P; ++j) x[j] = t[j];
}

template <int P, int SIGN>
__device__ __forceinline__ void wave_fft_front_compact_rest(float (&re)[P], float (&im)[P], const float* twh, float* xbuf,
                                                            int lane, float lc, float ls);
template <int P, int SIGN>
__device__ __forceinline__ void wave_fft_front_compact(float (&re)[P], float (&im)[P], const float* twh, float* xbuf,
                                                       int lane, float lc, float ls) {
    static_assert(P == 32, "compact form: P == 32 only");
    fft_inreg<P, SIGN>(re, im);
    wave_fft_front_compact_rest<P, SIGN>(re, im, twh, xbuf, lane, lc, ls);
}
template <int P, int SIGN>
// ... 78 lines not shown
```

magphase_amd/csrc/wave_fft_f64.hpp:

```cpp
#pragma once
#include "wave_fft.hpp"

namespace mpx {

__device__ __forceinline__ constexpr double dc64(int k) {
    constexpr double t[32] = {1.00000000000000000e+00, 9.95184726672196929e-01, 9.80785280403230431e-01, 9.56940335732208824e-01, 9.23879532511286738e-01, 8.81921264348355050e-01, 8.31469612302545236e-01, 7.73010453362736993e-01, 7.07106781186547573e-01, 6.34393284163645488e-01, 5.55570233019602289e-01, 4.71396736825997809e-01, 3.82683432365089837e-01, 2.90284677254462331e-01, 1.95090322016128331e-01, 9.80171403295607702e-02, 6.12323399573676604e-17, -9.80171403295606453e-02, -1.95090322016128193e-01, -2.90284677254462165e-01, -3.82683432365089726e-01, -4.71396736825997698e-01, -5.55570233019601956e-01, -6.34393284163645377e-01, -7.07106781186547462e-01, -7.73010453362736993e-01, -8.31469612302545347e-01, -8.81921264348354939e-01, -9.23879532511286738e-01, -9.56940335732208824e-01, -9.80785280403230431e-01, -9.95184726672196818e-01};
    return t[k];
}
__device__ __forceinline__ constexpr double ds64(int k) {
    constexpr double t[32] = {0.00000000000000000e+00, 9.80171403295606036e-02, 1.95090322016128248e-01, 2.90284677254462331e-01, 3.82683432365089782e-01, 4.71396736825997642e-01, 5.55570233019602178e-01, 6.34393284163645488e-01, 7.07106781186547462e-01, 7.73010453362736993e-01, 8.31469612302545236e-01, 8.81921264348354939e-01, 9.23879532511286738e-01, 9.56940335732208935e-01, 9.80785280403230431e-01, 9.95184726672196818e-01, 1.00000000000000000e+00, 9.95184726672196929e-01, 9.80785280403230431e-01, 9.56940335732208935e-01, 9.23879532511286738e-01, 8.81921264348355050e-01, 8.31469612302545458e-01, 7.73010453362737104e-01, 7.07106781186547573e-01, 6.34393284163645488e-01, 5.55570233019602178e-01, 4.71396736825997864e-01, 3.82683432365089893e-01, 2.90284677254462387e-01, 1.95090322016128609e-01, 9.80171403295608257e-02};
    return t[k];
}

template <int P>
__host__ __device__ constexpr int tw64_stride() { return 2 * P + 2; }
template <int P>
__host__ __device__ constexpr int tw64_doubles() { return 64 * tw64_stride<P>(); }

__device__ __forceinline__ void split64(double v, unsigned& lo, unsigned& hi) {
    const unsigned long long b = __builtin_bit_cast(unsigned long long, v);
    lo = (unsigned)b;
    hi = (unsigned)(b >> 32);
}
__device__ __forceinline__ double join64(unsigned lo, unsigned hi) {
    return __builtin_bit_cast(double, ((unsigned long long)hi << 32) | lo);
}

template <int P, int SIGN>
__device__ __forceinline__ void fft_inreg_f64(double (&re)[P], double (&im)[P]) {
#pragma unroll
    for (int s = P / 2; s >= 1; s >>= 1) {
#pragma unroll
        for (int g = 0; g < P; g += 2 * s) {
#pragma unroll
            for (int k = 0; k < s; ++k) {
                const int i0 = g + k, i1 = g + k + s;
                const int t = k * (16 / s);
                const double ar = re[i0], ai = im[i0], br = re[i1], bi = im[i1];
                re[i0] = ar + br;
                im[i0] = ai + bi;
                const double tr = ar - br, ti = ai - bi;
                if (t == 0) {
                    re[i1] = tr;
                    im[i1] = ti;
                } else if (t == 8) {
                    re[i1] = (SIGN < 0) ? ti : -ti;
                    im[i1] = (SIGN < 0) ? -tr : tr;
                } else {
                    const double c = dc64(2 * t), sn = (SIGN < 0) ? -ds64(2 * t) : ds64(2 * t);
                    re[i1] = tr * c - ti * sn;
                    im[i1] = tr * sn + ti * c;
                }
            }
        }
    }
}

template <int P, int SIGN>
__device__ __forceinline__ void fft_inreg_dit_f64(double (&re)[P], double (&im)[P]) {
#pragma unroll
    for (int s = 1; s < P; s <<= 1) {
#pragma unroll
        for (int g = 0; g < P; g += 2 * s) {
#pragma unroll
            for (int k = 0; k < s; ++k) {
                const int i0 = g + k, i1 = g + k + s;
                const int t = k * (16 / s);
                const double ar = re[i0], ai = im[i0], br = re[i1], bi = im[i1];
                if (t == 0) {
                    re[i0] = ar + br;
                    im[i0] = ai + bi;
                    re[i1] = ar - br;
                    im[i1] = ai - bi;
                } else if (t == 8) {
                    re[i0] = (SIGN < 0) ? ar + bi : ar - bi;
                    im[i0] = (SIGN < 0) ? ai - br : ai + br;
                    re[i1] = (SIGN < 0) ? ar - bi : ar + bi;
                    im[i1] = (SIGN < 0) ? ai + br : ai - br;
                } else {
                    const double c = dc64(2 * t), sn = (SIGN < 0) ? -ds64(2 * t) : ds64(2 * t);
                    const double o0r = fma(br, c, fma(-bi, sn, ar));
                    const double o0i = fma(br, sn, fma(bi, c, ai));
                    re[i0] = o0r;
                    im[i0] = o0i;
                    re[i1] = fma(2.0, ar, -o0r);
                    im[i1] = fma(2.0, ai, -o0i);
                }
            }
        }
    }
}

template <int P, bool NAT = false>
__device__ __forceinline__ void lds_transpose_f64(double (&x)[P], float* xbuf, int lane) {
    float lo[P], hi[P];
#pragma unroll
    for (int i = 0; i < P; ++i) {
        unsigned a, b;
        split64(x[i], a, b);
        lo[i] = __builtin_bit_cast(float, a);
        hi[i] = __builtin_bit_cast(float, b);
    }
    lds_transpose<P, NAT>(lo, xbuf, lane);
    lds_transpose<P, NAT>(hi, xbuf, lane);
#pragma unroll
    for (int i = 0; i < P; ++i) x[i] = join64(__builtin_bit_cast(unsigned, lo[i]), __builtin_bit_cast(unsigned, hi[i]));
}

template <int PARTNER>
__device__ __forceinline__ double lane_xor_f64(double v) {
    unsigned lo, hi;
    split64(v, lo, hi);
    if (PARTNER == 8) {
        lo = (unsigned)__builtin_amdgcn_update_dpp(0, (int)lo, 0x128, 0xf, 0xf, false);
        hi = (unsigned)__builtin_amdgcn_update_dpp(0, (int)hi, 0x128, 0xf, 0xf, false);
    } else {
        lo = (unsigned)__shfl_xor((int)lo, PARTNER);
        hi = (unsigned)__shfl_xor((int)hi, PARTNER);
    }
    return join64(lo, hi);
}

template <int P, int SIGN, int PARTNER, int TWN>
__device__ __forceinline__ void cross_lane_stage_f64(double (&re)[P], double (&im)[P], bool upper, bool rot, int lane) {
    if (PARTNER >= 16) {
        auto swp = [](double& a, double& b) {
            unsigned al, ah, bl, bh;
            split64(a, al, ah);
            split64(b, bl, bh);
            float fal = __builtin_bit_cast(float, al), fah = __builtin_bit_cast(float, ah);
            float fbl = __builtin_bit_cast(float, bl), fbh = __builtin_bit_cast(float, bh);
            if (PARTNER == 32) { swap32(fal, fbl); swap32(fah, fbh); } else { swap16(fal, fbl); swap16(fah, fbh); }
            a = join64(__builtin_bit_cast(unsigned, fal), __builtin_bit_cast(unsigned, fah));
            b = join64(__builtin_bit_cast(unsigned, fbl), __builtin_bit_cast(unsigned, fbh));
        };
#pragma unroll
        for (int lp = 0; lp < P; lp += 2) {
            swp(re[lp], re[lp + 1]);
            swp(im[lp], im[lp + 1]);
        }
#pragma unroll
        for (int lp = 0; lp < P; lp += 2) {
            const double a = re[lp], b = re[lp + 1], c = im[lp], d = im[lp + 1];
            re[lp] = a + b;
            re[lp + 1] = a - b;
            im[lp] = c + d;
            im[lp + 1] = c - d;
        }
#pragma unroll
        for (int lp = 0; lp < P; lp += 2) {
            swp(re[lp], re[lp + 1]);
            swp(im[lp], im[lp + 1]);
        }
    } else {
        const double sg = upper ? -1.0 : 1.0;
#pragma unroll
        for (int lp = 0; lp < P; ++lp) {
            const double orr = lane_xor_f64<PARTNER>(re[lp]);
            const double oii = lane_xor_f64<PARTNER>(im[lp]);
            re[lp] = fma(re[lp], sg, orr);
            im[lp] = fma(im[lp], sg, oii);
        }
    }
    if (upper) {
#pragma unroll
        for (int lp = 1; lp < P; ++lp) {
            const int k = (TWN == 64) ? lp : ((TWN == 32) ? 2 * lp : 4 * lp);
            const double cw = dc64(k), sw = (SIGN < 0) ? -ds64(k) : ds64(k);
            const double xr = re[lp] * cw - im[lp] * sw;
            const double xi = re[lp] * sw + im[lp] * cw;
            re[lp] = xr;
            im[lp] = xi;
        }
    }
    if (PARTNER == 4 * P) {
        const int e = (lane >> 3) & 3;
        constexpr double kR2 = 7.07106781186547524e-01;
        const double fc = (e == 0) ? 1.0 : ((e == 1) ? kR2 : ((e == 2) ? 0.0 : -kR2));
        const double fs0 = (e == 0) ? 0.0 : ((e == 1) ? kR2 : ((e == 2) ? 1.0 : kR2));
        const double fs = (SIGN < 0) ? -fs0 : fs0;
        if (upper) {
#pragma unroll
            for (int lp = 0; lp < P; ++lp) {
                const double xr = re[lp] * fc - im[lp] * fs;
                const double xi = re[lp] * fs + im[lp] * fc;
                re[lp] = xr;
                im[lp] = xi;
            }
        }
    }
    if (PARTNER == 2 * P) {
        if (rot) {
#pragma unroll
            for (int lp = 0; lp < P; ++lp) {
                const double xr = re[lp], xi = im[lp];
                re[lp] = (SIGN < 0) ? xi : -xi;
                im[lp] = (SIGN < 0) ? -xr : xr;
            }
        }
    }
}

template <int P, int SIGN>
__device__ __forceinline__ void wave_fft_f64(double (&re)[P], double (&im)[P], const double* tw, float* xbuf, int lane) {
    fft_inreg_f64<P, SIGN>(re, im);
    const double2* trow = reinterpret_cast<const double2*>(tw + lane * tw64_stride<P>());
#pragma unroll
    for (int i = 0; i < P; ++i) {
        if ((i & 7) == 0) asm volatile("" ::: "memory");
        const double2 w = trow[i];
        const double ws = (SIGN < 0) ? -w.y : w.y;
        const double xr = re[i] * w.x - im[i] * ws;
        const double xi = re[i] * ws + im[i] * w.x;
        re[i] = xr;
        im[i] = xi;
    }
    lds_transpose_f64<P>(re, xbuf, lane);
    lds_transpose_f64<P>(im, xbuf, lane);
    if (P == 32) {
        cross_lane_stage_f64<P, SIGN, 32, 64>(re, im, (lane & 32) != 0, false, lane);
    } else if (P == 16) {
        cross_lane_stage_f64<P, SIGN, 32, 64>(re, im, (lane & 32) != 0, (lane & 48) == 48, lane);
        cross_lane_stage_f64<P, SIGN, 16, 32>(re, im, (lane & 16) != 0, false, lane);
    } else {
        cross_lane_stage_f64<P, SIGN, 32, 64>(re, im, (lane & 32) != 0, false, lane);
        cross_lane_stage_f64<P, SIGN, 16, 32>(re, im, (lane & 16) != 0, (lane & 24) == 24, lane);
        cross_lane_stage_f64<P, SIGN, 8, 16>(re, im, (lane & 8) != 0, false, lane);
    }
    fft_inreg_f64<P, SIGN>(re, im);
}

template <int P, int SIGN>
__device__ __forceinline__ void wave_fft_dit_f64(double (&re)[P], double (&im)[P], const double* twn, float* xbuf, int lane) {
    constexpr int LB = ilog2(P);
    fft_inreg_dit_f64<P, SIGN>(re, im);
    const double2* trow = reinterpret_cast<const double2*>(twn + lane * tw64_stride<P>());
#pragma unroll
    for (int i = 0; i < P; ++i) {
        if ((i & 7) == 0) asm volatile("" ::: "memory");
        const double2 w = trow[i];
        const double ws = (SIGN < 0) ? -w.y : w.y;
        const double xr = re[i] * w.x - im[i] * ws;
        const double xi = re[i] * ws + im[i] * w.x;
        re[i] = xr;
        im[i] = xi;
    }
    lds_transpose_f64<P, true>(re, xbuf, lane);
    lds_transpose_f64<P, true>(im, xbuf, lane);
    if (P == 32) {
        cross_lane_stage_f64<P, SIGN, 32, 64>(re, im, (lane & 32) != 0, false, lane);
    } else if (P == 16) {
        cross_lane_stage_f64<P, SIGN, 32, 64>(re, im, (lane & 32) != 0, (lane & 48) == 48, lane);
        cross_lane_stage_f64<P, SIGN, 16, 32>(re, im, (lane & 16) != 0, false, lane);
    } else {
        cross_lane_stage_f64<P, SIGN, 32, 64>(re, im, (lane & 32) != 0, false, lane);
        cross_lane_stage_f64<P, SIGN, 16, 32>(re, im, (lane & 16) != 0, (lane & 24) == 24, lane);
        cross_lane_stage_f64<P, SIGN, 8, 16>(re, im, (lane & 8) != 0, false, lane);
    }
    double tr[P], ti[P];
#pragma unroll
    for (int r = 0; r < P; ++r) {
        tr[brev(r, LB)] = re[r];
        ti[brev(r, LB)] = im[r];
    }
    fft_inreg_dit_f64<P, SIGN>(tr, ti);
#pragma unroll
    for (int r = 0; r < P; ++r) {
        re[r] = tr[r];
        im[r] = ti[r];
    }
}

}
```

magphase_amd/engine.py:

```python
import ctypes
import os

import numpy as np

from . import _lib, hostmath as hm, hostplan


def _torch():
    import torch

    return torch


class HostTicket:

    def __init__(self, ring, slot, event, keep):
        self._ring, self._slot, self._event, self._keep = ring, slot, event, keep

    def wait(self):
        if self._event is not None:
            self._event.synchronize()
            self._event = self._keep = None

    def release(self):
        if self._ring is not None:
            self.wait()
            self._ring.release(self._slot)
            self._ring = None

    def __del__(self):
        try:
            self.release()
        except Exception:
            pass


class _PinnedRing:

    def __init__(self, slots=4):
        import queue
        import threading

        self._bufs = [None] * slots
        self._freeq = queue.SimpleQueue()
        for k in range(slots):
            self._freeq.put(k)
        self._lock = threading.Lock()

    def acquire(self, nbytes, timeout=None):
        import queue

        torch = _torch()
        if timeout is None:
            timeout = float(os.environ.get("MAGPHASE_RING_WAIT_S", "20"))
        try:
            slot = self._freeq.get(timeout=timeout)
        except queue.Empty:
            return None, None
        try:
            with self._lock:
                buf = self._bufs[slot]
                if buf is None or buf.numel() < nbytes:
                    size = max([int(nbytes * 1.25), 1 << 20] + [b.numel() for b in self._bufs if b is not None])
                    self._bufs[slot] = buf = torch.empty(size, dtype=torch.uint8).pin_memory()
                    idle = []
                    while True:
                        try:
                            idle.append(self._freeq.get_nowait())
                        except queue.Empty:
                            break
                    try:
                        for k in idle:
                            if self._bufs[k] is None or self._bufs[k].numel() < size:
                                self._bufs[k] = torch.empty(size, dtype=torch.uint8).pin_memory()
                    finally:
                        for k in idle:
                            self._freeq.put(k)
        except BaseException:
            self._freeq.put(slot)
            raise
        return slot, buf

    def release(self, slot):
        self._freeq.put(slot)


class Engine:
    def __init__(self, device=None):
        torch = _torch()
        self.lib = _lib.load()
        if not torch.cuda.is_available():
            raise _lib.MagphaseHipError("magphase_amd needs a ROCm GPU (torch.cuda.is_available() is False); "
                                        "there is no CPU fallback")
        if device is None:
            device = torch.device("cuda", torch.cuda.current_device())
        self.device = torch.device(device)
        self._tables = {}

    def stream_ptr(self):
        return _torch().cuda.current_stream(self.device).cuda_stream

    def launch(self, name, *args):
        tensor = _torch().Tensor
        with _torch().cuda.device(self.device):
            rc = getattr(self.lib, name)(self.stream_ptr(), *[a.data_ptr() if isinstance(a, tensor) else a for a in args])
        if rc != 0:
            _lib.check(rc, name)

    def background(self, fn, *args):
        import concurrent.futures as cf

        if os.environ.get("MAGPHASE_HOST_THREAD", "1") == "0":
            f = cf.Future()
            try:
                f.set_result(fn(*args))
            except BaseException as exc:
                f.set_exception(exc)
            return f
        ex = getattr(self, "_helper", None)
        if ex is None:
            ex = self._helper = cf.ThreadPoolExecutor(max_workers=1, thread_name_prefix="mpx-host")
        return ex.submit(fn, *args)

    def copy_stream(self, kind):
        if os.environ.get("MAGPHASE_COPY_STREAMS", "1") == "0":
            return None
        cs = getattr(self, "_copy_streams", None)
        if cs is None:
            torch = _torch()
            cs = self._copy_streams = {"up": torch.cuda.Stream(self.device), "down": torch.cuda.Stream(self.device)}
        if kind == "rng" and os.environ.get("MAGPHASE_RNG_STREAM", "1") == "0":
            return None
        if kind not in cs:
            cs[kind] = _torch().cuda.Stream(self.device)
        return cs[kind]

    def _download(self, pairs):
        torch = _torch()
        cur = torch.cuda.current_stream(self.device)
        down = self.copy_stream("down")
        if down is None:
            for dst, src in pairs:
                dst.copy_(src, non_blocking=True)
            ev = torch.cuda.Event()
            ev.record(cur)
            return ev
        ready = torch.cuda.Event()
        ready.record(cur)
        with torch.cuda.stream(down):
            down.wait_event(ready)
            for dst, src in pairs:
                dst.copy_(src, non_blocking=True)
                src.record_stream(down)
            ev = torch.cuda.Event()
            ev.record(down)
        return ev

    def empty(self, shape, dtype=None):
        torch = _torch()
        return torch.empty(shape, dtype=dtype or torch.float32, device=self.device)

    def empty_feats(self, n_frames, n_bins, ld=None):
        ld = int(ld or os.environ.get("MAGPHASE_FEAT_LD", 0) or self.lib.mpx_feat_ld(2 * (int(n_bins) - 1)) or n_bins)
        return self.empty((int(n_frames), ld))[:, :int(n_bins)]

    def feats_cat_to_device(self, parts, n_bins):
        H = int(n_bins)
        if int(os.environ.get("MAGPHASE_FEAT_LD", 0) or self.lib.mpx_feat_ld(2 * (H - 1)) or H) != H:
            return None
        rows = [int(np.shape(p)[0]) for p in parts]
        total = int(sum(rows)) * H
        if total == 0 or total > (128 << 20):
            return None
        stage = self.host_staging(total)
        n_thr = self.host_threads(4 * total, big=16)
        off = 0
        for p_, r in zip(parts, rows):
            a = np.asarray(p_)
            if a.ndim != 2 or a.shape[1] != H:
                raise ValueError("feature matrices must be [frames x %d]" % H)
            if a.dtype == np.float64 and a.flags.c_contiguous:
                if self.lib.mpx_host_narrow_f64(a.ctypes.data, stage[off:off + r * H].ctypes.data, r * H, n_thr) != 0:
                    raise _lib.MagphaseHipError("mpx_host_narrow_f64 failed")
            else:
                stage[off:off + r * H] = a.reshape(-1)
            off += r * H
        return self.upload_staged(total).view(int(sum(rows)), H)

    def feats_to_device(self, arr):
        torch = _torch()
        arr = np.ascontiguousarray(arr, dtype=np.float32)
        out = self.empty_feats(arr.shape[0], arr.shape[1])
        out.copy_(torch.from_numpy(arr))
        return out

    def _pinned_ring(self, n_floats, depth):
        torch = _torch()
        cur = getattr(self, "_pinned", None)
        if cur is None or len(cur) < depth or cur[0].numel() < n_floats:
            n_alloc = max(int(n_floats * 1.5), 1 << 20)
            self._pinned = tuple(torch.empty(n_alloc, dtype=torch.float32).pin_memory() for _ in range(depth))
        return self._pinned

    def to_host_f64_many(self, tensors, chunk_bytes=None, depth=3):
        torch = _torch()
        n_thr = self.host_threads(sum(int(t.numel()) * 4 for t in tensors), big=16)
        if chunk_bytes is None:
            chunk_bytes = int(os.environ.get("MAGPHASE_D2H_CHUNK_MB", "32")) << 20
        outs, views, work = [], [], []
        for k, t in enumerate(tensors):
            v = t.view(1, -1) if t.dim() == 1 else t
            rows, cols = int(v.shape[0]), int(v.shape[1])
            out = np.empty((rows, cols), dtype=np.float64)
            outs.append(out.reshape(-1) if t.dim() == 1 else out)
            views.append((v, out, cols))
            if rows and cols:
                rows_per = max(1, int(chunk_bytes) // (4 * cols))
                work.extend((k, r0, min(rows, r0 + rows_per)) for r0 in range(0, rows, rows_per))
        if not work:
            return outs
        biggest = max((r1 - r0) * views[k][2] for k, r0, r1 in work)
        bufs = self._pinned_ring(biggest, depth)
        events = [torch.cuda.Event() for _ in range(depth)]

        def drain(i):
            k, r0, r1 = work[i]
            _v, out, cols = views[k]
            events[i % depth].synchronize()
            if self.lib.mpx_host_widen_f32(bufs[i % depth].data_ptr(), out[r0:r1].ctypes.data, (r1 - r0) * cols, n_thr) != 0:
                raise _lib.MagphaseHipError("mpx_host_widen_f32 failed")

        with torch.cuda.device(self.device):
            for i, (k, r0, r1) in enumerate(work):
                if i >= depth:
                    drain(i - depth)
                v, _out, cols = views[k]
                bufs[i % depth][:(r1 - r0) * cols].view(r1 - r0, cols).copy_(v[r0:r1], non_blocking=True)
                events[i % depth].record()
            for i in range(max(0, len(work) - depth), len(work)):
                drain(i)
        return outs

    def to_host_f64(self, t, chunk_bytes=None):
        return self.to_host_f64_many([t], chunk_bytes=chunk_bytes)[0]

    def to_host_f32(self, t):
        torch = _torch()
        dst = torch.empty(tuple(int(x) for x in t.shape), dtype=torch.float32)
        if dst.numel():
            with torch.cuda.device(self.device):
# ... 1119 lines not shown
```

Measured before the change: 172.7 million.

## Add narrow-support pruned FFT arms for noise stats and f64 fused analysis

Extends the support-class pruning, where the first FFT stages skip butterflies on known-zero input rows for frames whose window is narrow, to the non-compact noise-stats kernel and to the f64 fused analysis kernels, using new pruned DIT stages for f64. Each kernel checks per frame whether its support is narrow and takes either the pruned gather and butterflies or the full path. Both arms are on by default and can be turned off at runtime through a global mask set by an environment variable. This adds more kernel instantiations and a divergent branch per frame, which may raise register pressure in kernels already held to two waves per EU.

Result: slower. 170.2 million (-1.4%).

```diff
diff --git a/include/magphase_hip.h b/include/magphase_hip.h
--- a/include/magphase_hip.h
+++ b/include/magphase_hip.h
@@ -17,6 +17,11 @@
 
 int mpx_version(void);
 const char* mpx_last_error(void);
+
+#define MPX_SUPPORT_ARM_NOISE 1u
+#define MPX_SUPPORT_ARM_F64 2u
+void mpx_support_arms_set(uint32_t mask);
+uint32_t mpx_support_arms_get(void);
 
 size_t mpx_tables_bytes(int fft_len);
 int mpx_tables_init(void* stream, int fft_len, void* tables);
diff --git a/magphase_amd/_lib.py b/magphase_amd/_lib.py
--- a/magphase_amd/_lib.py
+++ b/magphase_amd/_lib.py
@@ -11,6 +11,8 @@
 PROTOTYPES = {
     "mpx_version": (i32, []),
     "mpx_last_error": (ctypes.c_char_p, []),
+    "mpx_support_arms_set": (None, [u32]),
+    "mpx_support_arms_get": (u32, []),
     "mpx_tables_bytes": (sz, [i32]),
     "mpx_tables_init": (i32, [vp, i32, vp]),
     "mpx_feat_ld": (i64, [i32]),
@@ -118,6 +120,7 @@
 SYMBOLS = tuple(PROTOTYPES)
 RT_STORE_FLAGS = {"rows": 4, "lines": 0, "lines_nt": 8}
 RT_INVERSE_FLAGS = {"direct": 0, "transform": 32}
+SUPPORT_ARMS = {"off": 0, "noise": 1, "f64": 2, "on": 3}
 del vp, i32, i64, sz, f64
 
 _lib = None
diff --git a/magphase_amd/csrc/magphase_comp.hip b/magphase_amd/csrc/magphase_comp.hip
--- a/magphase_amd/csrc/magphase_comp.hip
+++ b/magphase_amd/csrc/magphase_comp.hip
@@ -82,7 +82,7 @@
 __device__ __forceinline__ void noise_fft(const FrameGeom& g, int wtype, const float* tw, float* xbuf,
                                           unsigned xbuf_byte, int lane, float (&re)[P], float (&im)[P], float lc = 1.0f,
                                           float ls = 0.0f, bool narrow = false, Hook hook = Hook()) {
-    static_assert(NW == 0 || (COMPACT && !MPX_COMP_DIT), "support classes: the compact DIF form only");
+    static_assert(NW == 0 || !(COMPACT && MPX_COMP_DIT), "support classes: the DIF forms only");
     if constexpr (NW > 0) {
         constexpr unsigned kZin = support_zero_rows<P>(NW);
         constexpr int S0 = zin_clear_stride<P>(kZin);
@@ -102,9 +102,14 @@
             fft_inreg_stages<P, -1, P / 2, 2 * S0>(re, im);
             MPX_ARM_END_FULL();
         }
-        const float4 pk = tw_half_pad<P>(tw, lane);
-        fft_inreg_stages<P, -1, S0>(re, im);
-        wave_fft_front_compact_rest<P, -1>(re, im, tw, xbuf, lane, pk.z, pk.w);
+        if constexpr (COMPACT) {
+            const float4 pk = tw_half_pad<P>(tw, lane);
+            fft_inreg_stages<P, -1, S0>(re, im);
+            wave_fft_front_compact_rest<P, -1>(re, im, tw, xbuf, lane, pk.z, pk.w);
+        } else {
+            fft_inreg_stages<P, -1, S0>(re, im);
+            wave_fft_front_rest<P, -1>(re, im, tw, xbuf, lane);
+        }
         hook.exchanged();
         fft_inreg<P, -1>(re, im);
         (void)lc;
@@ -277,6 +282,9 @@
 typedef float spec_f32x4 __attribute__((ext_vector_type(4)));
 
 template <int P>
+constexpr int noise_arm_class(bool arms) { return (arms && P == 32) ? kSupportNarrow : 0; }
+
+template <int P, bool ARMS = false>
 __global__ __launch_bounds__(kAnaThreads) void k_noise_stats(const float* __restrict__ noise,
                                                           const long long* __restrict__ npos,
                                                           const int* __restrict__ nleft,
@@ -306,7 +314,11 @@
         asm volatile("" : "+v"(lane), "+v"(wl_s), "+v"(wl_c));
         const FrameGeom g = frame_geom(noise, npos[f], nleft[f], nright[f], N);
         float no_r[P / 2], no_i[P / 2], nm_r[P / 2], nm_i[P / 2], nh_r, nh_i;
-        noise_spectrum_paired<P>(g, wtype[f], tw, xbuf, xbuf_byte, lane, wl_c, wl_s, no_r, no_i, nm_r, nm_i, nh_r, nh_i);
+        constexpr int NW = noise_arm_class<P>(ARMS);
+        bool narrow = false;
+        if constexpr (NW > 0) narrow = (frame_support_class(g.L, g.LR - g.L, N) == NW);
+        noise_spectrum_paired<P, false, false, NW>(g, wtype[f], tw, xbuf, xbuf_byte, lane, wl_c, wl_s, no_r, no_i, nm_r, nm_i,
+                                                   nh_r, nh_i, 1.0f, 0.0f, narrow);
         if constexpr (P == 32) {
             if (spec_out) {
                 spec_f32x4* d = reinterpret_cast<spec_f32x4*>(spec_out + f * (long long)kSpecFrameFloats) + lane_id;
@@ -1448,7 +1460,11 @@
         return fail(MPX_ERR_ARG, "mpx_noise_stats: null pointer%s");
     const dim3 grid(grid_for(n_frames, kAnaWaves)), block(kAnaThreads);
     hipStream_t s = (hipStream_t)stream;
-    if (P == 32) {
+    if (P == 32 && support_arm_on(MPX_SUPPORT_ARM_NOISE)) {
+        if (int rc = set_lds(k_noise_stats<32, true>, lds_bytes_ana<32>())) return rc;
+        hipLaunchKernelGGL((k_noise_stats<32, true>), grid, block, lds_bytes_ana<32>(), s, noise, (const long long*)frame_pos,
+                           frame_left, frame_right, frame_wtype, (long long)n_frames, (const float*)tables, out_sum, spectra);
+    } else if (P == 32) {
         if (int rc = set_lds(k_noise_stats<32>, lds_bytes_ana<32>())) return rc;
         hipLaunchKernelGGL(k_noise_stats<32>, grid, block, lds_bytes_ana<32>(), s, noise, (const long long*)frame_pos,
                            frame_left, frame_right, frame_wtype, (long long)n_frames, (const float*)tables, out_sum, spectra);
diff --git a/magphase_amd/csrc/magphase_f64.hip b/magphase_amd/csrc/magphase_f64.hip
--- a/magphase_amd/csrc/magphase_f64.hip
+++ b/magphase_amd/csrc/magphase_f64.hip
@@ -61,6 +61,94 @@
 __device__ __forceinline__ constexpr int f64_out_reg(int q) { return kF64Dit ? q : brev(q, ilog2(P)); }
 
 template <int P>
+constexpr int f64_arm_class(bool arms) { return (arms && P == 32 && kF64Dit) ? kSupportNarrow : 0; }
+constexpr bool fused_arm_built(int ntp, int magmode) { return ntp == 1 && magmode == 0; }
+constexpr bool fused_cr_arm_built(int ntp) { return ntp >= 2; }
+template <int P>
+constexpr unsigned f64_zero_regs(int W) {
+    unsigned z = 0u;
+    for (int j = 0; j < P; ++j)
+        if ((support_zero_rows<P>(W) >> j) & 1u) z |= 1u << f64_in_reg<P>(j);
+    return z;
+}
+
+template <int P, int W>
+__device__ __forceinline__ void f64_window_gather(const FrameGeom& g, bool tabw, const double* tl, const double* tr, double invL,
+                                                  double invR, float in_scale, float* xbuf, unsigned xbuf_byte, float* wbuf,
+                                                  unsigned wbuf_byte, int lane, double (&re)[P], double (&im)[P], double& s_abs) {
+    constexpr int N = 128 * P, kTile = 64 * P;
+#pragma unroll
+    for (int j = 0; j < P; ++j)
+        if (j < W || j >= P - W) re[f64_in_reg<P>(j)] = im[f64_in_reg<P>(j)] = 0.0;
+    constexpr int capD = f64_win_floats<P>() / 2;
+    double* wl = reinterpret_cast<double*>(wbuf);
+    const int nidx = g.LR + 2;
+    const int ntiles = (g.len + kTile - 1) / kTile;
+    for (int t = 0; t < ntiles; ++t) {
+        const int tile0 = t * kTile;
+        const int hi = min(g.len, tile0 + kTile);
+        stage_samples_async(g, tile0, kTile, xbuf_byte, lane);
+        for (int seg0 = 0; seg0 < nidx; seg0 += capD) {
+            const int seg1 = min(seg0 + capD, nidx);
+            if (tabw) {
+                const int a0 = seg0, a1 = min(g.L + 1, seg1), b0 = max(g.L + 1, seg0), b1 = seg1;
+                const float* srcl = reinterpret_cast<const float*>(tl + a0);
+                const float* srcr = reinterpret_cast<const float*>(tr + (b0 - (g.L + 1)));
+                const int nl = 2 * max(a1 - a0, 0), nr = 2 * max(b1 - b0, 0);
+                for (int c = 0; c < (nl + 63) >> 6; ++c) {
+                    const unsigned m0v = __builtin_amdgcn_readfirstlane(wbuf_byte + 256u * (unsigned)c);
+                    if (64 * c + lane < nl) {
+                        const float* src = srcl + 64 * c + lane;
+                        asm volatile("s_mov_b32 m0, %1\n\ts_nop 0\n\tglobal_load_lds_dword %0, off" ::"v"(src), "s"(m0v) : "m0", "memory");
+                    }
+                }
+                for (int c = 0; c < (nr + 63) >> 6; ++c) {
+                    const unsigned m0v = __builtin_amdgcn_readfirstlane(wbuf_byte + 8u * (unsigned)(b0 - seg0) + 256u * (unsigned)c);
+                    if (64 * c + lane < nr) {
+                        const float* src = srcr + 64 * c + lane;
+                        asm volatile("s_mov_b32 m0, %1\n\ts_nop 0\n\tglobal_load_lds_dword %0, off" ::"v"(src), "s"(m0v) : "m0", "memory");
+                    }
+                }
+            } else {
+                for (int i = seg0 + lane; i < seg1; i += 64) {
+                    const int k = (i <= g.L) ? i : g.LR - (i - (g.L + 1));
+                    wl[i - seg0] = hann_half_f64(k, g.L, g.LR, g.kadd, invL, invR);
+                }
+            }
+            staged_wait<0>();
+            wave_sync();
+            int lane_g = lane;
+            asm volatile("" : "+v"(lane_g));
+#pragma unroll
+            for (int j = 0; j < P; ++j) {
+                const int m0 = 128 * j;
+                const bool any = (j < W || j >= P - W) && ((m0 < g.len - g.rot) || (m0 + 127 >= N - g.rot));
+                if (any) {
+                    const int m = m0 + 2 * lane_g;
+                    int k0 = m + g.rot;
+                    k0 = (k0 >= N) ? k0 - N : k0;
+                    int k1 = m + 1 + g.rot;
+                    k1 = (k1 >= N) ? k1 - N : k1;
+                    const int i0 = ((k0 <= g.L) ? k0 : g.L + 1 + (g.LR - k0)) - seg0;
+                    const int i1 = ((k1 <= g.L) ? k1 : g.L + 1 + (g.LR - k1)) - seg0;
+                    if (k0 >= tile0 && k0 < hi && i0 >= 0 && i0 < capD) {
+                        const double v = (double)(xbuf[k0 - tile0] * in_scale) * wl[i0];
+                        re[f64_in_reg<P>(j)] = v;
+                        s_abs += fabs(v);
+                    }
+                    if (k1 >= tile0 && k1 < hi && i1 >= 0 && i1 < capD) {
+                        const double v = (double)(xbuf[k1 - tile0] * in_scale) * wl[i1];
+                        im[f64_in_reg<P>(j)] = v;
+                        s_abs += fabs(v);
+                    }
+                }
+            }
+            wave_sync();
+        }
+    }
+}
+
+template <int P, bool ARMS = false>
 __device__ __forceinline__ void f64_frame_transform(const float* __restrict__ sig, long long pos, int Lf, int Rf,
                                                     const double* __restrict__ win_tab, int win_cap, const double* tw,
                                                     float* xbuf, unsigned xbuf_byte, float* wbuf, unsigned wbuf_byte,
@@ -78,6 +166,38 @@
     const float mag_scale = tabw ? 9.313225746154785e-10f : 1.0f;
 
     double s_abs = 0.0;
+    if constexpr (f64_arm_class<P>(ARMS) > 0) {
+        constexpr int NW = f64_arm_class<P>(ARMS);
+        constexpr unsigned kZin = f64_zero_regs<P>(NW);
+        const bool narrow = rfl((int)(frame_support_class(g.L, gR, N) == NW)) != 0;
+        if (narrow) {
+            f64_window_gather<P, NW>(g, tabw, tl, tr, invL, invR, in_scale, xbuf, xbuf_byte, wbuf, wbuf_byte, lane, re, im, s_abs);
+            fft_inreg_dit_pruned2_f64<P, -1, 1, kZin>(re, im);
+            MPX_ARM_END_CLASS();
+        } else {
+            f64_window_gather<P, P / 2>(g, tabw, tl, tr, invL, invR, in_scale, xbuf, xbuf_byte, wbuf, wbuf_byte, lane, re, im, s_abs);
+            fft_inreg_dit_stages_f64<P, -1, 1, 2>(re, im);
+            MPX_ARM_END_FULL();
+        }
+        fft_inreg_dit_stages_f64<P, -1, 4>(re, im);
+        float s_all = (float)s_abs;
+#pragma unroll
+        for (int d = 32; d >= 1; d >>= 1) s_all += __shfl_xor(s_all, d);
+        const double zt = 2.842170943040401e-14 * (double)s_all;
+#ifdef MPX_F64_NOFLUSH
+        const double zero2 = 1.0e-36 + 0.0 * zt;
+#else
+        const double zero2 = tabw ? 1.0e-36 : fmax(zt * zt, 1.0e-36);
+#endif
+        wave_fft_dit_f64_rest<P, -1>(re, im, tw, xbuf, lane);
+#pragma unroll
+        for (int j = 0; j < P; j += 4)
+            asm volatile("" : "+v"(re[j]), "+v"(re[j + 1]), "+v"(re[j + 2]), "+v"(re[j + 3]), "+v"(im[j]), "+v"(im[j + 1]),
+                              "+v"(im[j + 2]), "+v"(im[j + 3]));
+        zero2_out = zero2;
+        mag_scale_out = mag_scale;
+        return;
+    }
 #pragma unroll
     for (int j = 0; j < P; ++j) re[j] = im[j] = 0.0;
     constexpr int capD = f64_win_floats<P>() / 2;
@@ -398,7 +518,7 @@
     return sizeof(double) * (size_t)tw64_doubles<P>() + work + sizeof(float) * 32;
 }
 
-template <int P, int NTM, int NTP, int MAGMODE>
+template <int P, int NTM, int NTP, int MAGMODE, bool ARMS = false>
 __attribute__((amdgpu_waves_per_eu(2, 2)))
 __global__ __launch_bounds__(kFusedWaves * 64) void k_analysis_warp_fused(
     const float* __restrict__ sig, const long long* __restrict__ fpos, const int* __restrict__ fleft,
@@ -446,8 +566,8 @@
         float mag_scale = 1.0f;
         bool voi = false;
         if (has) {
-            f64_frame_transform<P>(sig, fpos[f], fleft[f], fright[f], win_tab, win_cap, tw, xbuf, xbuf_byte, wbuf, wbuf_byte, lane,
-                                   re, im, zero2, mag_scale);
+            f64_frame_transform<P, ARMS>(sig, fpos[f], fleft[f], fright[f], win_tab, win_cap, tw, xbuf, xbuf_byte, wbuf, wbuf_byte, lane,
+                                         re, im, zero2, mag_scale);
             voi = rfl((int)(voiced[f] != 0.0f)) != 0;
         } else {
 #pragma unroll
@@ -689,7 +809,7 @@
     cstart[f] = lo;
 }
 
-template <int P, int NTP>
+template <int P, int NTP, bool ARMS = false>
 __attribute__((amdgpu_waves_per_eu(2, 2)))
 __global__ __launch_bounds__(kFusedWaves * 64) void k_analysis_warp_fused_cr(
     const float* __restrict__ sig, const long long* __restrict__ fpos, const int* __restrict__ fleft,
@@ -758,8 +878,8 @@
         float mag_scale = 1.0f;
         bool voi = false;
         if (has) {
-            f64_frame_transform<P>(sig, fpos[f], fleft[f], fright[f], win_tab, win_cap, tw, xbuf, xbuf_byte, wbuf, wbuf_byte, lane,
-                                   re, im, zero2, mag_scale);
+            f64_frame_transform<P, ARMS>(sig, fpos[f], fleft[f], fright[f], win_tab, win_cap, tw, xbuf, xbuf_byte, wbuf, wbuf_byte, lane,
+                                         re, im, zero2, mag_scale);
             voi = rfl((int)(rows_in_use[f] != 0.0f)) != 0;
         } else {
 #pragma unroll
@@ -1112,25 +1232,26 @@
     const dim3 grid((unsigned)(nrounds < slots ? nrounds : slots)), block(kFusedWaves * 64);
     hipStream_t s = (hipStream_t)stream;
     const int ntp = (phase_dim + 15) / 16;
-#define MPX_FUSED_GO(PP, NTP_, MM)                                                                                        \
+#define MPX_FUSED_GO(PP, NTP_, MM, AA)                                                                                    \
     do {                                                                                                                  \
-        if (int rc = set_lds(k_analysis_warp_fused<PP, 4, NTP_, MM>, (lds_bytes_fused<PP, 4, NTP_>()))) return rc;        \
-        hipLaunchKernelGGL((k_analysis_warp_fused<PP, 4, NTP_, MM>), grid, block, (lds_bytes_fused<PP, 4, NTP_>()), s, sig, \
+        if (int rc = set_lds(k_analysis_warp_fused<PP, 4, NTP_, MM, (AA) && fused_arm_built(NTP_, MM)>, (lds_bytes_fused<PP, 4, NTP_>()))) return rc;    \
+        hipLaunchKernelGGL((k_analysis_warp_fused<PP, 4, NTP_, MM, (AA) && fused_arm_built(NTP_, MM)>), grid, block, (lds_bytes_fused<PP, 4, NTP_>()), s, sig, \
                            (const long long*)frame_pos, frame_left, frame_right, (long long)n_frames,                     \
                            (const double*)tables_f64, win_tab, (int)win_cap, wpack, whalf, voiced, (int)mag_dim,          \
                            (int)phase_dim, out_mag, out_real, out_imag);                                                  \
     } while (0)
-#define MPX_FUSED_P(PP)                                                     \
+#define MPX_FUSED_P(PP, AA)                                                 \
     do {                                                                    \
-        if (ntp == 1 && !mag_fbank) MPX_FUSED_GO(PP, 1, 0);                 \
-        else if (ntp == 1) MPX_FUSED_GO(PP, 1, 2);                          \
-        else if (ntp == 2 && !mag_fbank) MPX_FUSED_GO(PP, 2, 0);            \
-        else if (ntp == 2) MPX_FUSED_GO(PP, 2, 2);                          \
-        else if (!mag_fbank) MPX_FUSED_GO(PP, 3, 0);                        \
-        else MPX_FUSED_GO(PP, 3, 2);                                        \
+        if (ntp == 1 && !mag_fbank) MPX_FUSED_GO(PP, 1, 0, AA);             \
+        else if (ntp == 1) MPX_FUSED_GO(PP, 1, 2, AA);                      \
+        else if (ntp == 2 && !mag_fbank) MPX_FUSED_GO(PP, 2, 0, AA);        \
+        else if (ntp == 2) MPX_FUSED_GO(PP, 2, 2, AA);                      \
+        else if (!mag_fbank) MPX_FUSED_GO(PP, 3, 0, AA);                    \
+        else MPX_FUSED_GO(PP, 3, 2, AA);                                    \
     } while (0)
-    if (P == 32) MPX_FUSED_P(32);
-    else MPX_FUSED_P(16);
+    if (P == 32 && f64_arm_class<32>(true) > 0 && support_arm_on(MPX_SUPPORT_ARM_F64)) MPX_FUSED_P(32, true);
+    else if (P == 32) MPX_FUSED_P(32, false);
+    else MPX_FUSED_P(16, false);
 #undef MPX_FUSED_P
 #undef MPX_FUSED_GO
     MPX_HIP_CHECK(hipGetLastError());
@@ -1173,23 +1294,24 @@
     const long long fw = 8 * ((per + 1 + 7) / 8) - 1;
     const dim3 grid((unsigned)((n_frames + fw - 1) / fw)), block(kFusedWaves * 64);
     const int ntp = (phase_dim + 15) / 16;
-#define MPX_FUSED_CR_GO(PP, NTP_)                                                                                       \
+#define MPX_FUSED_CR_GO(PP, NTP_, AA)                                                                                   \
     do {                                                                                                                \
-        if (int rc = set_lds(k_analysis_warp_fused_cr<PP, NTP_>, (lds_bytes_fused_cr<PP, NTP_>()))) return rc;          \
-        hipLaunchKernelGGL((k_analysis_warp_fused_cr<PP, NTP_>), grid, block, (lds_bytes_fused_cr<PP, NTP_>()), s, sig, \
+        if (int rc = set_lds(k_analysis_warp_fused_cr<PP, NTP_, (AA) && fused_cr_arm_built(NTP_)>, (lds_bytes_fused_cr<PP, NTP_>()))) return rc;      \
+        hipLaunchKernelGGL((k_analysis_warp_fused_cr<PP, NTP_, (AA) && fused_cr_arm_built(NTP_)>), grid, block, (lds_bytes_fused_cr<PP, NTP_>()), s, sig, \
                            (const long long*)frame_pos, frame_left, frame_right, (long long)n_frames,                   \
                            (const double*)tables_f64, win_tab, (int)win_cap, wpack, whalf, rows_in_use, row0, row1,     \
                            row_t, (const int*)cstart, (int)fw, (int)mag_dim, (int)phase_dim, out_mag, tmp_real,         \
                            tmp_imag, halo);                                                                             \
     } while (0)
-#define MPX_FUSED_CR_P(PP)                       \
-    do {                                         \
-        if (ntp == 1) MPX_FUSED_CR_GO(PP, 1);    \
-        else if (ntp == 2) MPX_FUSED_CR_GO(PP, 2); \
-        else MPX_FUSED_CR_GO(PP, 3);             \
+#define MPX_FUSED_CR_P(PP, AA)                       \
+    do {                                             \
+        if (ntp == 1) MPX_FUSED_CR_GO(PP, 1, AA);    \
+        else if (ntp == 2) MPX_FUSED_CR_GO(PP, 2, AA); \
+        else MPX_FUSED_CR_GO(PP, 3, AA);             \
     } while (0)
-    if (P == 32) MPX_FUSED_CR_P(32);
-    else MPX_FUSED_CR_P(16);
+    if (P == 32 && f64_arm_class<32>(true) > 0 && support_arm_on(MPX_SUPPORT_ARM_F64)) MPX_FUSED_CR_P(32, true);
+    else if (P == 32) MPX_FUSED_CR_P(32, false);
+    else MPX_FUSED_CR_P(16, false);
 #undef MPX_FUSED_CR_P
 #undef MPX_FUSED_CR_GO
     MPX_HIP_CHECK(hipGetLastError());
diff --git a/magphase_amd/csrc/magphase_hip.hip b/magphase_amd/csrc/magphase_hip.hip
--- a/magphase_amd/csrc/magphase_hip.hip
+++ b/magphase_amd/csrc/magphase_hip.hip
@@ -746,6 +746,10 @@
 int mpx_version(void) { return MPX_ABI_VERSION; }
 
 const char* mpx_last_error(void) { return g_err; }
+
+void mpx_support_arms_set(uint32_t mask) { g_support_arms.store(mask & (MPX_SUPPORT_ARM_NOISE | MPX_SUPPORT_ARM_F64), std::memory_order_relaxed); }
+
+uint32_t mpx_support_arms_get(void) { return g_support_arms.load(std::memory_order_relaxed); }
 
 size_t mpx_tables_bytes(int fft_len) {
     const int P = p_of(fft_len);
diff --git a/magphase_amd/csrc/mpx_common.hpp b/magphase_amd/csrc/mpx_common.hpp
--- a/magphase_amd/csrc/mpx_common.hpp
+++ b/magphase_amd/csrc/mpx_common.hpp
@@ -1,5 +1,6 @@
 #pragma once
 #include <hip/hip_runtime.h>
+#include <atomic>
 #include <cmath>
 #include <cstdint>
 #include <cstdio>
@@ -18,6 +19,9 @@
     snprintf(g_err, sizeof(g_err), fmt, detail);
     return code;
 }
+
+inline std::atomic<uint32_t> g_support_arms{MPX_SUPPORT_ARM_NOISE | MPX_SUPPORT_ARM_F64};
+inline bool support_arm_on(uint32_t bit) { return (g_support_arms.load(std::memory_order_relaxed) & bit) != 0u; }
 
 #define MPX_HIP_CHECK(expr)                                                       \
     do {                                                                          \
diff --git a/magphase_amd/csrc/wave_fft.hpp b/magphase_amd/csrc/wave_fft.hpp
--- a/magphase_amd/csrc/wave_fft.hpp
+++ b/magphase_amd/csrc/wave_fft.hpp
@@ -338,8 +338,14 @@
 }
 
 template <int P, int SIGN>
+__device__ __forceinline__ void wave_fft_front_rest(float (&re)[P], float (&im)[P], const float* tw, float* xbuf, int lane);
+template <int P, int SIGN>
 __device__ __forceinline__ void wave_fft_front(float (&re)[P], float (&im)[P], const float* tw, float* xbuf, int lane) {
     fft_inreg<P, SIGN>(re, im);
+    wave_fft_front_rest<P, SIGN>(re, im, tw, xbuf, lane);
+}
+template <int P, int SIGN>
+__device__ __forceinline__ void wave_fft_front_rest(float (&re)[P], float (&im)[P], const float* tw, float* xbuf, int lane) {
     const float4* trow = reinterpret_cast<const float4*>(tw + lane * tw_stride<P>());
 #pragma unroll
     for (int q = 0; q < P / 2; ++q) {
diff --git a/magphase_amd/csrc/wave_fft_f64.hpp b/magphase_amd/csrc/wave_fft_f64.hpp
--- a/magphase_amd/csrc/wave_fft_f64.hpp
+++ b/magphase_amd/csrc/wave_fft_f64.hpp
@@ -91,6 +91,79 @@
     }
 }
 
+template <int P, int SIGN, int S_LO, int S_HI = P / 2>
+__device__ __forceinline__ void fft_inreg_dit_stages_f64(double (&re)[P], double (&im)[P]) {
+#pragma unroll
+    for (int s = S_LO; s <= S_HI; s <<= 1) {
+#pragma unroll
+        for (int g = 0; g < P; g += 2 * s) {
+#pragma unroll
+            for (int k = 0; k < s; ++k) {
+                const int i0 = g + k, i1 = g + k + s;
+                const int t = k * (16 / s);
+                const double ar = re[i0], ai = im[i0], br = re[i1], bi = im[i1];
+                if (t == 0) {
+                    re[i0] = ar + br;
+                    im[i0] = ai + bi;
+                    re[i1] = ar - br;
+                    im[i1] = ai - bi;
+                } else if (t == 8) {
+                    re[i0] = (SIGN < 0) ? ar + bi : ar - bi;
+                    im[i0] = (SIGN < 0) ? ai - br : ai + br;
+                    re[i1] = (SIGN < 0) ? ar - bi : ar + bi;
+                    im[i1] = (SIGN < 0) ? ai + br : ai - br;
+                } else {
+                    const double c = dc64(2 * t), sn = (SIGN < 0) ? -ds64(2 * t) : ds64(2 * t);
+                    const double o0r = fma(br, c, fma(-bi, sn, ar));
+                    const double o0i = fma(br, sn, fma(bi, c, ai));
+                    re[i0] = o0r;
+                    im[i0] = o0i;
+                    re[i1] = fma(2.0, ar, -o0r);
+                    im[i1] = fma(2.0, ai, -o0i);
+                }
+            }
+        }
+    }
+}
+
+template <int P>
+__host__ __device__ constexpr bool dit_pruned2_ok(unsigned zin) {
+    for (int s = 1; s <= 2; s <<= 1) {
+        for (int g = 0; g < P; g += 2 * s)
+            for (int k = 0; k < s; ++k)
+                if (!((zin >> (g + k)) & 1u) && !((zin >> (g + k + s)) & 1u)) return false;
+        zin = dif_zero_after<P>(s, zin);
+    }
+    return (zin & (P >= 32 ? ~0u : ((1u << (P & 31)) - 1u))) == 0u;
+}
+template <int P, int SIGN, int S, unsigned ZIN>
+__device__ __forceinline__ void fft_inreg_dit_pruned2_f64(double (&re)[P], double (&im)[P]) {
+    static_assert(S == 1 || S == 2, "the stages whose twiddles are 1 and SIGN i");
+    static_assert(S == 2 || dit_pruned2_ok<P>(ZIN), "every butterfly of the two stages meets a zero, none is left behind them");
+#pragma unroll
+    for (int g = 0; g < P; g += 2 * S) {
+#pragma unroll
+        for (int k = 0; k < S; ++k) {
+            const int i0 = g + k, i1 = g + k + S;
+            const bool za = (ZIN >> i0) & 1u, zb = (ZIN >> i1) & 1u;
+            if (za && zb) continue;
+            if (zb) {
+                re[i1] = re[i0];
+                im[i1] = im[i0];
+            } else if (za) {
+                const double br = re[i1], bi = im[i1];
+                const double wr = (k == 0) ? br : ((SIGN < 0) ? bi : -bi);
+                const double wi = (k == 0) ? bi : ((SIGN < 0) ? -br : br);
+                re[i0] = wr;
+                im[i0] = wi;
+                re[i1] = -wr;
+                im[i1] = -wi;
+            }
+        }
+    }
+    if constexpr (S == 1) fft_inreg_dit_pruned2_f64<P, SIGN, 2, dif_zero_after<P>(1, ZIN)>(re, im);
+}
+
 template <int P, bool NAT = false>
 __device__ __forceinline__ void lds_transpose_f64(double (&x)[P], float* xbuf, int lane) {
     float lo[P], hi[P];
@@ -231,9 +304,15 @@
 }
 
 template <int P, int SIGN>
+__device__ __forceinline__ void wave_fft_dit_f64_rest(double (&re)[P], double (&im)[P], const double* twn, float* xbuf, int lane);
+template <int P, int SIGN>
 __device__ __forceinline__ void wave_fft_dit_f64(double (&re)[P], double (&im)[P], const double* twn, float* xbuf, int lane) {
+    fft_inreg_dit_f64<P, SIGN>(re, im);
+    wave_fft_dit_f64_rest<P, SIGN>(re, im, twn, xbuf, lane);
+}
+template <int P, int SIGN>
+__device__ __forceinline__ void wave_fft_dit_f64_rest(double (&re)[P], double (&im)[P], const double* twn, float* xbuf, int lane) {
     constexpr int LB = ilog2(P);
-    fft_inreg_dit_f64<P, SIGN>(re, im);
     const double2* trow = reinterpret_cast<const double2*>(twn + lane * tw64_stride<P>());
 #pragma unroll
     for (int i = 0; i < P; ++i) {
diff --git a/magphase_amd/engine.py b/magphase_amd/engine.py
--- a/magphase_amd/engine.py
+++ b/magphase_amd/engine.py
@@ -96,6 +96,11 @@
             device = torch.device("cuda", torch.cuda.current_device())
         self.device = torch.device(device)
         self._tables = {}
+        arms = os.environ.get("MAGPHASE_SUPPORT_ARMS", "")
+        if arms:
+            if arms not in _lib.SUPPORT_ARMS:
+                raise ValueError("MAGPHASE_SUPPORT_ARMS must be off, noise, f64 or on, not %r" % arms)
+            self.lib.mpx_support_arms_set(_lib.SUPPORT_ARMS[arms])
 
     def stream_ptr(self):
         return _torch().cuda.current_stream(self.device).cuda_stream
```
